# griffithlab/regtools

Measured on AMD Instinct MI355X. Metric: alignments/sec + junctions/sec, junctions extract, 1/2/4/8 MI355X, higher is better.
Workload: dtype u8/u32 integer; 1 GPU; configs[1]: synthetic 50000000-read 101 bp BAM per GPU, ~15% reads with one N-op, junctions extract -s XS; reads_per_gpu=50000000, seed=1, bgzf_members=169426, compressed_bytes_per_gpu=533101619, inflated_bytes_per_gpu=11060000978

## Files before the change

### include/regtools_amd.h

```cpp
#ifndef REGTOOLS_AMD_H
#define REGTOOLS_AMD_H
#include <stddef.h>
#include <stdint.h>

#ifdef __cplusplus
extern "C" {
#endif

#define RGX_OK             0
#define RGX_ERR_OPEN       1
#define RGX_ERR_INDEX      2
#define RGX_ERR_REGION     3
#define RGX_ERR_NO_DEVICE  4
#define RGX_ERR_DEVICE     5
#define RGX_ERR_FORMAT     6
#define RGX_ERR_ARG        7
#define RGX_ERR_FASTA      8
#define RGX_ERR_ABORT      9
#define RGX_ERR_EXIT      10

typedef struct rgx_ctx rgx_ctx;

typedef struct {
    const char *region;
    int32_t     strandness;
    char        strand_tag[2];
    uint32_t    min_anchor;
    uint32_t    min_intron;
    uint32_t    max_intron;
    const char *fasta_path;
    int32_t     shard;
    int32_t     n_shards;
    int32_t     barcodes;
    char        barcode_tag[2];
} rgx_extract_params;

void rgx_extract_params_default(rgx_extract_params *p);

typedef struct {
    int32_t    n_ref;
    char     **ref_name;
    uint32_t  *ref_len;
    uint64_t   n;
    int32_t   *tid;
    uint32_t  *start, *end;
    uint32_t  *thick_start, *thick_end;
    uint32_t  *read_count;
    uint64_t  *name_index;
    char      *strand;
    uint8_t   *left_ok, *right_ok;
    uint64_t   n_records;
    uint64_t   n_events;
    uint64_t   inflated_bytes, compressed_bytes, n_members;
    double     ms_total, ms_inflate, ms_records, ms_scan, ms_reduce;
    uint64_t  *first_seen;
    uint64_t  *last_seen;
    uint64_t   framing_sweeps;
    uint64_t  *bc_row_begin;
    uint32_t  *bc_count;
    uint64_t  *bc_str_begin;
    char      *bc_text;
    uint32_t  *bc_insert_rank;
    double     ms_barcodes;
    uint64_t   stream_ended;
    double     ms_inflate_launch;
} rgx_junction_table;

int  rgx_ctx_create(int device, rgx_ctx **out, char *err, size_t errlen);
void rgx_ctx_destroy(rgx_ctx *ctx);
int  rgx_ctx_arena_trials(const rgx_ctx *ctx, float *ms, int cap);

int  rgx_extract(rgx_ctx *ctx, const char *bam_path, const rgx_extract_params *p,
                 rgx_junction_table **out, char *err, size_t errlen);

void *rgx_host_alloc(size_t bytes);
void  rgx_host_free(void *p);
int  rgx_extract_mem(rgx_ctx *ctx, const void *bam, size_t bam_len, const void *bai, size_t bai_len,
                     const rgx_extract_params *p, rgx_junction_table **out, char *err, size_t errlen);

typedef struct rgx_pipeline rgx_pipeline;
int  rgx_pipeline_create(int device, int depth , rgx_pipeline **out, char *err, size_t errlen);
int  rgx_pipeline_depth(const rgx_pipeline *pl);
rgx_ctx *rgx_pipeline_ctx(const rgx_pipeline *pl, uint64_t ticket);
int  rgx_extract_submit(rgx_pipeline *pl, const void *bam, size_t bam_len, const void *bai, size_t bai_len, const rgx_extract_params *p,
                        uint64_t *ticket, char *err, size_t errlen);
int  rgx_extract_wait(rgx_pipeline *pl, uint64_t ticket, rgx_junction_table **out, char *err, size_t errlen);
void rgx_pipeline_destroy(rgx_pipeline *pl);

int  rgx_extract_device(rgx_ctx *ctx, const void *d_bam, size_t bam_len,
                        const void *bai, size_t bai_len, const rgx_extract_params *p,
                        rgx_junction_table **out, char *err, size_t errlen);

int  rgx_extract_multi(const int *devices, int n_devices, const char *bam_path, const rgx_extract_params *p,
                       rgx_junction_table **out, char *err, size_t errlen);
int  rgx_extract_multi_mem(const int *devices, int n_devices, const void *bam, size_t bam_len, const void *bai, size_t bai_len,
                           const rgx_extract_params *p, rgx_junction_table **out, char *err, size_t errlen);
const char *rgx_multi_exchange_kind(void);

void rgx_table_free(rgx_junction_table *t);

int  rgx_table_merge(const rgx_junction_table *const *parts, int n_parts, uint32_t min_anchor,
                     rgx_junction_table **out, char *err, size_t errlen);

#define RGX_PACKED_ROW_BYTES 48
size_t rgx_table_pack(const rgx_junction_table *t, void *dst, size_t dst_cap);
int    rgx_table_unpack(const void *src, size_t n_rows, const rgx_junction_table *names_from,
                        rgx_junction_table **out);
size_t rgx_table_pack_barcodes(const rgx_junction_table *t, void *dst, size_t dst_cap);
int    rgx_table_unpack_barcodes(rgx_junction_table *t, const void *src, size_t len);
int    rgx_table_merge_barcodes(const rgx_junction_table *const *parts, int n_parts, rgx_junction_table *merged, char *err, size_t errlen);
int    rgx_last_table_pack_device(rgx_ctx *ctx, const rgx_junction_table *t, void *d_dst, uint64_t cap_rows, char *err, size_t errlen);
int    rgx_table_merge_device(rgx_ctx *ctx, const void *d_rows, uint64_t stride_rows, const uint64_t *part_rows, int n_parts,
                              uint32_t min_anchor, const rgx_junction_table *names_from, rgx_junction_table **out,
                              char *err, size_t errlen);

size_t rgx_table_format_bed12(const rgx_junction_table *t, int only_anchored, char *buf, size_t cap);

size_t rgx_table_format_barcodes(const rgx_junction_table *t, int only_anchored, char *buf, size_t cap);

const char *rgx_version(void);

typedef struct { uint64_t cpos, upos; uint32_t clen, isize; } rgx_member;
int  rgx_k_inflate(const void *d_comp, const rgx_member *d_members, uint32_t n_members,
                   void *d_arena, uint32_t *d_status, void *stream);
int  rgx_k_inflate_form(int form, const void *d_comp, const rgx_member *d_members, uint32_t n_members,
                        void *d_arena, uint32_t *d_status, void *stream);

typedef struct {
    const char *vcf_path, *bam_path, *fasta_path, *gtf_path;
    const char *out_tsv;
    const char *out_vcf;
    const char *out_bed;
    uint32_t    window;
    uint32_t    intronic_min;
    uint32_t    exonic_min;
    int32_t     all_intronic;
    int32_t     all_exonic;
    int32_t     skip_single;
    int32_t     strandness;
    char        strand_tag[2];
    uint32_t    min_anchor;
    uint32_t    min_intron;
    uint32_t    max_intron;
    int32_t     override_motif;
    const char *bed_path;
    int32_t     echo;
} rgx_identify_params;

typedef struct {
    uint64_t n_variants, n_relevant, n_windows, n_pairs, n_window_rows, n_junctions;
    uint64_t n_records, n_events;
    uint64_t exon_visits_variants;
    uint64_t exon_visits_junctions;
    double   ms_total, ms_gtf, ms_variants, ms_extract, ms_join, ms_annotate, ms_output;
    double   ms_k_variant_scan, ms_k_junction_scan, ms_k_window_pairs;
} rgx_identify_stats;

void rgx_identify_params_default(rgx_identify_params *p);

int  rgx_identify(rgx_ctx *ctx, const rgx_identify_params *p, rgx_identify_stats *stats, char *err, size_t errlen);
int  rgx_identify_multi(const int *devices, int n_devices, const rgx_identify_params *p, rgx_identify_stats *stats, char *err, size_t errlen);

int  rgx_associate(rgx_ctx *ctx, const rgx_identify_params *p, rgx_identify_stats *stats, char *err, size_t errlen);
int  rgx_variants_annotate(rgx_ctx *ctx, const rgx_identify_params *p, rgx_identify_stats *stats, char *err, size_t errlen);
int  rgx_junctions_annotate(rgx_ctx *ctx, const char *bed_path, const char *fasta_path, const char *gtf_path, const char *out_path,
                            uint64_t *n_rows, char *err, size_t errlen);
#define RGX_ANNOTATE_SINGLE_EXON 1
#define RGX_ANNOTATE_ECHO        2
int  rgx_junctions_annotate_opts(rgx_ctx *ctx, const char *bed_path, const char *fasta_path, const char *gtf_path, const char *out_path,
                                 int options, uint64_t *n_rows, char *err, size_t errlen);

typedef struct rgx_gtf rgx_gtf;
int  rgx_gtf_load(rgx_ctx *ctx, const char *gtf_path, rgx_gtf **out, char *err, size_t errlen);
void rgx_gtf_free(rgx_gtf *g);
int  rgx_gtf_info(const rgx_gtf *g, uint32_t *n_transcripts, uint32_t *n_exons, uint32_t *n_chroms);
int  rgx_gtf_transcript_bin(const rgx_gtf *g, const char *transcript_id, uint32_t *bin);

typedef struct {
    uint64_t n; uint32_t *cis_start, *cis_end; uint32_t *hit_off; uint32_t *hit_transcript, *hit_annotation, *hit_distance;
} rgx_variant_hits;
int  rgx_variant_windows(rgx_ctx *ctx, const rgx_gtf *g, uint64_t n, const char *const *chrom, const uint32_t *pos0, uint32_t intronic_min,
                         uint32_t exonic_min, int all_intronic, int all_exonic, int skip_single, rgx_variant_hits **out, char *err, size_t errlen);
void rgx_variant_hits_free(rgx_variant_hits *h);
const char *rgx_gtf_transcript_id(const rgx_gtf *g, uint32_t t);

typedef struct {
    uint64_t n; uint32_t *flags, *n_acceptors_skipped, *n_exons_skipped, *n_donors_skipped; uint32_t *tx_off, *tx;
} rgx_junction_annot;
int  rgx_annotate_junctions(rgx_ctx *ctx, const rgx_gtf *g, uint64_t n, const char *const *chrom, const uint32_t *start, const uint32_t *end1,
                            const char *strand, rgx_junction_annot **out, char *err, size_t errlen);
void rgx_junction_annot_free(rgx_junction_annot *a);

typedef struct {
    uint64_t n;
    uint32_t *window, *start, *end, *thick_start, *thick_end, *read_count, *name_index;
    char *strand;
} rgx_window_rows;
int  rgx_window_join(rgx_ctx *ctx, const char *bam_path, const rgx_extract_params *p, uint64_t n_windows, const char *const *chrom,
                     const int32_t *beg, const int32_t *end, rgx_window_rows **out, char *err, size_t errlen);
void rgx_window_rows_free(rgx_window_rows *r);

#ifdef __cplusplus
}
#endif
#endif
```

### regtools_amd/_ffi.py

```python
import ctypes as C
import os

_HERE = os.path.dirname(os.path.abspath(__file__))
LIB_PATH = os.path.join(_HERE, "libregtools_amd.so")
SYNTH_PATH = os.path.join(_HERE, "libregtools_synth.so")


class ExtractParams(C.Structure):
    _fields_ = [("region", C.c_char_p), ("strandness", C.c_int32), ("strand_tag", C.c_char * 2),
                ("min_anchor", C.c_uint32), ("min_intron", C.c_uint32), ("max_intron", C.c_uint32),
                ("fasta_path", C.c_char_p), ("shard", C.c_int32), ("n_shards", C.c_int32),
                ("barcodes", C.c_int32), ("barcode_tag", C.c_char * 2)]


class JunctionTable(C.Structure):
    _fields_ = [("n_ref", C.c_int32), ("ref_name", C.POINTER(C.c_char_p)), ("ref_len", C.POINTER(C.c_uint32)),
                ("n", C.c_uint64), ("tid", C.POINTER(C.c_int32)), ("start", C.POINTER(C.c_uint32)),
                ("end", C.POINTER(C.c_uint32)), ("thick_start", C.POINTER(C.c_uint32)),
                ("thick_end", C.POINTER(C.c_uint32)), ("read_count", C.POINTER(C.c_uint32)),
                ("name_index", C.POINTER(C.c_uint64)), ("strand", C.POINTER(C.c_char)),
                ("left_ok", C.POINTER(C.c_uint8)), ("right_ok", C.POINTER(C.c_uint8)),
                ("n_records", C.c_uint64), ("n_events", C.c_uint64), ("inflated_bytes", C.c_uint64),
                ("compressed_bytes", C.c_uint64), ("n_members", C.c_uint64),
                ("ms_total", C.c_double), ("ms_inflate", C.c_double), ("ms_records", C.c_double),
                ("ms_scan", C.c_double), ("ms_reduce", C.c_double),
                ("first_seen", C.POINTER(C.c_uint64)), ("last_seen", C.POINTER(C.c_uint64)), ("framing_sweeps", C.c_uint64),
                ("bc_row_begin", C.POINTER(C.c_uint64)), ("bc_count", C.POINTER(C.c_uint32)), ("bc_str_begin", C.POINTER(C.c_uint64)),
                ("bc_text", C.POINTER(C.c_char)), ("bc_insert_rank", C.POINTER(C.c_uint32)), ("ms_barcodes", C.c_double), ("stream_ended", C.c_uint64),
                ("ms_inflate_launch", C.c_double)]


class Member(C.Structure):
    _fields_ = [("cpos", C.c_uint64), ("upos", C.c_uint64), ("clen", C.c_uint32), ("isize", C.c_uint32)]


EXPORTS = ["rgx_extract_params_default", "rgx_ctx_create", "rgx_ctx_destroy", "rgx_extract", "rgx_extract_mem",
           "rgx_extract_device", "rgx_table_free", "rgx_table_merge", "rgx_table_pack", "rgx_table_unpack",
           "rgx_table_format_bed12", "rgx_table_format_barcodes", "rgx_version", "rgx_k_inflate",
           "rgx_identify_params_default", "rgx_identify", "rgx_gtf_load", "rgx_gtf_free", "rgx_gtf_info", "rgx_gtf_transcript_bin",
           "rgx_gtf_transcript_id", "rgx_variant_windows", "rgx_variant_hits_free", "rgx_annotate_junctions", "rgx_junction_annot_free",
           "rgx_associate", "rgx_variants_annotate", "rgx_junctions_annotate", "rgx_junctions_annotate_opts", "rgx_table_merge_device", "rgx_window_join", "rgx_window_rows_free", "rgx_last_table_pack_device",
           "rgx_host_alloc", "rgx_host_free", "rgx_extract_multi", "rgx_extract_multi_mem", "rgx_multi_exchange_kind", "rgx_k_inflate_form", "rgx_table_merge_barcodes",
           "rgx_table_pack_barcodes", "rgx_table_unpack_barcodes", "rgx_identify_multi", "rgx_ctx_arena_trials",
           "rgx_pipeline_create", "rgx_pipeline_depth", "rgx_pipeline_ctx", "rgx_extract_submit", "rgx_extract_wait", "rgx_pipeline_destroy"]


class IdentifyParams(C.Structure):
    _fields_ = [("vcf_path", C.c_char_p), ("bam_path", C.c_char_p), ("fasta_path", C.c_char_p), ("gtf_path", C.c_char_p),
                ("out_tsv", C.c_char_p), ("out_vcf", C.c_char_p), ("out_bed", C.c_char_p), ("window", C.c_uint32),
                ("intronic_min", C.c_uint32), ("exonic_min", C.c_uint32), ("all_intronic", C.c_int32), ("all_exonic", C.c_int32),
                ("skip_single", C.c_int32), ("strandness", C.c_int32), ("strand_tag", C.c_char * 2), ("min_anchor", C.c_uint32),
                ("min_intron", C.c_uint32), ("max_intron", C.c_uint32), ("override_motif", C.c_int32), ("bed_path", C.c_char_p), ("echo", C.c_int32)]


class IdentifyStats(C.Structure):
    _fields_ = [(n, C.c_uint64) for n in ("n_variants", "n_relevant", "n_windows", "n_pairs", "n_window_rows", "n_junctions", "n_records", "n_events",
                                          "exon_visits_variants", "exon_visits_junctions")] + \
               [(n, C.c_double) for n in ("ms_total", "ms_gtf", "ms_variants", "ms_extract", "ms_join", "ms_annotate", "ms_output",
                                          "ms_k_variant_scan", "ms_k_junction_scan", "ms_k_window_pairs")]


class VariantHits(C.Structure):
    _fields_ = [("n", C.c_uint64), ("cis_start", C.POINTER(C.c_uint32)), ("cis_end", C.POINTER(C.c_uint32)), ("hit_off", C.POINTER(C.c_uint32)),
                ("hit_transcript", C.POINTER(C.c_uint32)), ("hit_annotation", C.POINTER(C.c_uint32)), ("hit_distance", C.POINTER(C.c_uint32))]


class WindowRows(C.Structure):
    _fields_ = [("n", C.c_uint64)] + [(k, C.POINTER(C.c_uint32)) for k in ("window", "start", "end", "thick_start", "thick_end", "read_count", "name_index")] + \
               [("strand", C.POINTER(C.c_char))]


class JunctionAnnot(C.Structure):
    _fields_ = [("n", C.c_uint64), ("flags", C.POINTER(C.c_uint32)), ("n_acceptors_skipped", C.POINTER(C.c_uint32)),
                ("n_exons_skipped", C.POINTER(C.c_uint32)), ("n_donors_skipped", C.POINTER(C.c_uint32)), ("tx_off", C.POINTER(C.c_uint32)),
                ("tx", C.POINTER(C.c_uint32))]

_lib = None


def _preload_torch_hip_runtime():
    try:
        import importlib.util
        spec = importlib.util.find_spec("torch")
        if spec and spec.submodule_search_locations:
            cand = os.path.join(list(spec.submodule_search_locations)[0], "lib", "libamdhip64.so")
            if os.path.exists(cand):
                C.CDLL(cand, mode=C.RTLD_GLOBAL)
    except Exception:
        pass


def lib():
    global _lib
    if _lib is None:
        if not os.path.exists(LIB_PATH):
            raise RuntimeError("regtools_amd: %s is missing -- run `python -c 'import __graft_entry__ as g; g.build()'` "
                               "(hipcc --offload-arch=gfx950). There is no CPU fallback." % LIB_PATH)
        _preload_torch_hip_runtime()
        L = C.CDLL(LIB_PATH)
        P = C.POINTER
        L.rgx_version.restype = C.c_char_p
        L.rgx_extract_params_default.argtypes = [P(ExtractParams)]
        L.rgx_ctx_create.argtypes = [C.c_int, P(C.c_void_p), C.c_char_p, C.c_size_t]
        L.rgx_ctx_destroy.argtypes = [C.c_void_p]
        L.rgx_ctx_arena_trials.argtypes = [C.c_void_p, P(C.c_float), C.c_int]
        L.rgx_extract.argtypes = [C.c_void_p, C.c_char_p, P(ExtractParams), P(P(JunctionTable)), C.c_char_p, C.c_size_t]
        L.rgx_extract_mem.argtypes = [C.c_void_p, C.c_void_p, C.c_size_t, C.c_void_p, C.c_size_t, P(ExtractParams),
                                      P(P(JunctionTable)), C.c_char_p, C.c_size_t]
        L.rgx_extract_device.argtypes = [C.c_void_p, C.c_void_p, C.c_size_t, C.c_void_p, C.c_size_t,
                                         P(ExtractParams), P(P(JunctionTable)), C.c_char_p, C.c_size_t]
        L.rgx_table_free.argtypes = [P(JunctionTable)]
        L.rgx_pipeline_create.argtypes = [C.c_int, C.c_int, P(C.c_void_p), C.c_char_p, C.c_size_t]
        L.rgx_pipeline_depth.argtypes = [C.c_void_p]
        L.rgx_pipeline_ctx.argtypes = [C.c_void_p, C.c_uint64]
        L.rgx_pipeline_ctx.restype = C.c_void_p
        L.rgx_extract_submit.argtypes = [C.c_void_p, C.c_void_p, C.c_size_t, C.c_void_p, C.c_size_t, P(ExtractParams), P(C.c_uint64), C.c_char_p, C.c_size_t]
        L.rgx_extract_wait.argtypes = [C.c_void_p, C.c_uint64, P(P(JunctionTable)), C.c_char_p, C.c_size_t]
        L.rgx_pipeline_destroy.argtypes = [C.c_void_p]
        L.rgx_extract_multi.argtypes = [P(C.c_int), C.c_int, C.c_char_p, P(ExtractParams), P(P(JunctionTable)), C.c_char_p, C.c_size_t]
        L.rgx_multi_exchange_kind.restype = C.c_char_p
        L.rgx_multi_exchange_kind.argtypes = []
        L.rgx_extract_multi_mem.argtypes = [P(C.c_int), C.c_int, C.c_void_p, C.c_size_t, C.c_void_p, C.c_size_t, P(ExtractParams), P(P(JunctionTable)), C.c_char_p, C.c_size_t]
        L.rgx_host_alloc.argtypes = [C.c_size_t]
        L.rgx_host_alloc.restype = C.c_void_p
        L.rgx_host_free.argtypes = [C.c_void_p]
        L.rgx_table_merge.argtypes = [P(P(JunctionTable)), C.c_int, C.c_uint32, P(P(JunctionTable)), C.c_char_p, C.c_size_t]
        L.rgx_table_merge_barcodes.argtypes = [P(P(JunctionTable)), C.c_int, P(JunctionTable), C.c_char_p, C.c_size_t]
        L.rgx_table_pack_barcodes.argtypes = [P(JunctionTable), C.c_void_p, C.c_size_t]
        L.rgx_table_pack_barcodes.restype = C.c_size_t
        L.rgx_table_unpack_barcodes.argtypes = [P(JunctionTable), C.c_void_p, C.c_size_t]
        L.rgx_table_pack.argtypes = [P(JunctionTable), C.c_void_p, C.c_size_t]
        L.rgx_table_pack.restype = C.c_size_t
        L.rgx_table_unpack.argtypes = [C.c_void_p, C.c_size_t, P(JunctionTable), P(P(JunctionTable))]
        L.rgx_last_table_pack_device.argtypes = [C.c_void_p, P(JunctionTable), C.c_void_p, C.c_uint64, C.c_char_p, C.c_size_t]
        L.rgx_table_merge_device.argtypes = [C.c_void_p, C.c_void_p, C.c_uint64, P(C.c_uint64), C.c_int, C.c_uint32, P(JunctionTable), P(P(JunctionTable)), C.c_char_p, C.c_size_t]
        L.rgx_table_format_bed12.argtypes = [P(JunctionTable), C.c_int, C.c_char_p, C.c_size_t]
        L.rgx_table_format_bed12.restype = C.c_size_t
        L.rgx_table_format_barcodes.argtypes = [P(JunctionTable), C.c_int, C.c_char_p, C.c_size_t]
        L.rgx_table_format_barcodes.restype = C.c_size_t
        L.rgx_k_inflate.argtypes = [C.c_void_p, C.c_void_p, C.c_uint32, C.c_void_p, C.c_void_p, C.c_void_p]
        L.rgx_k_inflate_form.argtypes = [C.c_int, C.c_void_p, C.c_void_p, C.c_uint32, C.c_void_p, C.c_void_p, C.c_void_p]
        L.rgx_identify_params_default.argtypes = [P(IdentifyParams)]
        L.rgx_identify.argtypes = [C.c_void_p, P(IdentifyParams), P(IdentifyStats), C.c_char_p, C.c_size_t]
        L.rgx_associate.argtypes = L.rgx_identify.argtypes
        L.rgx_identify_multi.argtypes = [P(C.c_int), C.c_int, P(IdentifyParams), P(IdentifyStats), C.c_char_p, C.c_size_t]
        L.rgx_variants_annotate.argtypes = L.rgx_identify.argtypes
        L.rgx_junctions_annotate_opts.argtypes = [C.c_void_p, C.c_char_p, C.c_char_p, C.c_char_p, C.c_char_p, C.c_int, P(C.c_uint64), C.c_char_p, C.c_size_t]
        L.rgx_junctions_annotate.argtypes = [C.c_void_p, C.c_char_p, C.c_char_p, C.c_char_p, C.c_char_p, P(C.c_uint64), C.c_char_p, C.c_size_t]
        L.rgx_gtf_load.argtypes = [C.c_void_p, C.c_char_p, P(C.c_void_p), C.c_char_p, C.c_size_t]
        L.rgx_gtf_free.argtypes = [C.c_void_p]
        L.rgx_gtf_info.argtypes = [C.c_void_p, P(C.c_uint32), P(C.c_uint32), P(C.c_uint32)]
        L.rgx_gtf_transcript_bin.argtypes = [C.c_void_p, C.c_char_p, P(C.c_uint32)]
        L.rgx_gtf_transcript_id.argtypes = [C.c_void_p, C.c_uint32]
        L.rgx_gtf_transcript_id.restype = C.c_char_p
        L.rgx_variant_windows.argtypes = [C.c_void_p, C.c_void_p, C.c_uint64, P(C.c_char_p), P(C.c_uint32), C.c_uint32, C.c_uint32, C.c_int, C.c_int, C.c_int,
                                          P(P(VariantHits)), C.c_char_p, C.c_size_t]
        L.rgx_variant_hits_free.argtypes = [P(VariantHits)]
        L.rgx_annotate_junctions.argtypes = [C.c_void_p, C.c_void_p, C.c_uint64, P(C.c_char_p), P(C.c_uint32), P(C.c_uint32), C.c_char_p,
                                             P(P(JunctionAnnot)), C.c_char_p, C.c_size_t]
        L.rgx_junction_annot_free.argtypes = [P(JunctionAnnot)]
        L.rgx_window_join.argtypes = [C.c_void_p, C.c_char_p, P(ExtractParams), C.c_uint64, P(C.c_char_p), P(C.c_int32), P(C.c_int32), P(P(WindowRows)), C.c_char_p, C.c_size_t]
        L.rgx_window_rows_free.argtypes = [P(WindowRows)]
        _lib = L
    return _lib


class SynthParams(C.Structure):
    _fields_ = [("shape", C.c_int), ("n_reads", C.c_uint64), ("seed", C.c_uint64), ("level", C.c_int),
                ("threads", C.c_int), ("n_introns", C.c_uint32), ("spliced_frac", C.c_double),
                ("realistic_payload", C.c_int), ("slice_index", C.c_int), ("n_slices", C.c_int), ("n_genes", C.c_uint32)]


class SynthResult(C.Structure):
    _fields_ = [("bam", C.c_void_p), ("bam_len", C.c_size_t), ("bai", C.c_void_p), ("bai_len", C.c_size_t),
                ("n_reads", C.c_uint64), ("n_spliced", C.c_uint64), ("n_blocks", C.c_uint64),
                ("inflated_bytes", C.c_uint64), ("cigar_ops", C.c_uint64)]


_synth = None


def synth():
    global _synth
    if _synth is None:
        if not os.path.exists(SYNTH_PATH):
            raise RuntimeError("regtools_amd: %s is missing -- run __graft_entry__.build()" % SYNTH_PATH)
        L = C.CDLL(SYNTH_PATH)
        P = C.POINTER
        L.rgx_synth_generate.argtypes = [P(SynthParams), P(SynthResult)]
        L.rgx_synth_free.argtypes = [P(SynthResult)]
        L.rgx_synth_write.argtypes = [P(SynthParams), C.c_char_p, P(SynthResult)]
        L.rgx_synth_index.argtypes = [C.c_char_p]
        L.rgx_synth_annotation.argtypes = [P(SynthParams), C.c_uint32, C.c_char_p, C.c_char_p, C.c_char_p]
        _synth = L
    return _synth


def format_bed12(table_ptr, only_anchored=True):
    L = lib()
    t = table_ptr.contents
    longest = max([len(t.ref_name[i]) for i in range(t.n_ref)] or [0])
    cap = int(t.n) * (longest + 160) + 1
    buf = C.create_string_buffer(cap)
    n = L.rgx_table_format_bed12(table_ptr, 1 if only_anchored else 0, buf, cap)
    if n > cap:
        buf = C.create_string_buffer(n + 1)
        L.rgx_table_format_bed12(table_ptr, 1 if only_anchored else 0, buf, n)
    return buf.raw[:n]
```

### regtools_amd/csrc/api_ctx.cpp

```cpp
#include "api_internal.h"

AllocStats g_alloc_stats;

rgx::Fasta *host_fasta(rgx_ctx *c, const char *path) {
    struct stat st;
    if (!path || stat(path, &st) != 0) return nullptr;
    const uint64_t key[4] = {(uint64_t)st.st_dev, (uint64_t)st.st_ino, (uint64_t)st.st_size,
        (uint64_t)st.st_mtim.tv_sec * 1000000000ull + (uint64_t)st.st_mtim.tv_nsec};
    if (c->host_fasta && c->host_fasta_path == path && !memcmp(key, c->host_fasta_key, sizeof key)) return c->host_fasta;
    delete c->host_fasta; c->host_fasta = nullptr;
    rgx::Fasta *f = new rgx::Fasta();
    if (!f->load(path)) { delete f; return nullptr; }
    c->host_fasta = f; c->host_fasta_path = path; memcpy(c->host_fasta_key, key, sizeof key);
    return f;
}

void ktime_begin(rgx_ctx *c, int slot) {
    hipEvent_t e[2];
    for (auto &x : e) { if (!c->kfree.empty()) { x = c->kfree.back(); c->kfree.pop_back(); } else if (hipEventCreate(&x) != hipSuccess) return; }
    (void)hipEventRecord(e[0], c->stream);
    c->kpend.push_back({e[0], e[1], slot});
}
void ktime_end(rgx_ctx *c) { if (!c->kpend.empty()) (void)hipEventRecord(c->kpend.back().b, c->stream); }
void ktime_collect(rgx_ctx *c) {
    for (auto &k : c->kpend) {
        float ms = 0;
        if (hipEventSynchronize(k.b) == hipSuccess && hipEventElapsedTime(&ms, k.a, k.b) == hipSuccess) c->kms[k.slot] += ms;
        c->kfree.push_back(k.a); c->kfree.push_back(k.b);
    }
    c->kpend.clear();
}

extern "C" const char *rgx_version(void) { return "regtools_amd 0.1 gfx950"; }

extern "C" void rgx_extract_params_default(rgx_extract_params *p) {
    memset(p, 0, sizeof *p);
    p->region = "."; p->strandness = -1; p->strand_tag[0] = 'X'; p->strand_tag[1] = 'S';
    p->min_anchor = 8; p->min_intron = 70; p->max_intron = 500000; p->fasta_path = nullptr; p->shard = 0; p->n_shards = 1;
    p->barcodes = 0; p->barcode_tag[0] = 'C'; p->barcode_tag[1] = 'B';
}

extern "C" int rgx_ctx_create(int device, rgx_ctx **out, char *err, size_t errlen) {
    *out = nullptr;
    int n = 0;
    if (hipGetDeviceCount(&n) != hipSuccess || n <= 0)
        return fail(err, errlen, RGX_ERR_NO_DEVICE, "regtools_amd: no HIP device visible; this library has no CPU fallback\n");
    if (device < 0 || device >= n) return fail(err, errlen, RGX_ERR_NO_DEVICE, "regtools_amd: device %d out of range (%d visible)\n", device, n);
    HIP_TRY(hipSetDevice(device));
    hipDeviceProp_t prop;
    HIP_TRY(hipGetDeviceProperties(&prop, device));
    if (!strstr(prop.gcnArchName, "gfx950"))
        return fail(err, errlen, RGX_ERR_NO_DEVICE, "regtools_amd: device %d is %s; the kernels are built for gfx950 only\n", device, prop.gcnArchName);
    rgx_ctx *c = new rgx_ctx();
    c->device = device;
    HIP_TRY(hipStreamCreateWithFlags(&c->stream, hipStreamNonBlocking));
    { const char *e = getenv("REGTOOLS_AMD_ONE_SHOT"); c->one_shot = e && strcmp(e, "0") != 0; }
    c->buf("arena").piece = arena_knobs().piece;
    for (auto &e : c->ev) HIP_TRY(hipEventCreate(&e));
    for (auto &e : c->ev_launch) HIP_TRY(hipEventCreate(&e));
    for (auto &e : c->ev_trial) HIP_TRY(hipEventCreate(&e));
    HIP_TRY(hipHostMalloc(&c->pinned, 4096, hipHostMallocDefault));
    c->pinned_cap = 4096;
    *out = c;
    return RGX_OK;
}

hipError_t ensure_upload_streams(rgx_ctx *c) {
    if (c->copy_stream || c->ev_ready) return hipSuccess;
    if (c->one_shot) return hipEventCreateWithFlags(&c->ev_ready, hipEventDisableTiming);
    hipError_t e = hipStreamCreateWithFlags(&c->copy_stream, hipStreamNonBlocking);
    if (e != hipSuccess) return e;
    for (int k = 0; k < kSideStreams; ++k) {
        if ((e = hipStreamCreateWithPriority(&c->side[k], hipStreamNonBlocking, 0)) != hipSuccess) return e;
        if ((e = hipEventCreateWithFlags(&c->ev_side[k], hipEventDisableTiming)) != hipSuccess) return e;
    }
    return hipEventCreateWithFlags(&c->ev_ready, hipEventDisableTiming);
}

void rgx_ctx_no_arena_trials(rgx_ctx *c) { if (c) c->arena_calibrated_bytes = UINT64_MAX; }
void *rgx_link_turn_create(int depth) {
    LinkTurn *l = new LinkTurn;
    const char *q = getenv("GPU_MAX_HW_QUEUES");
    l->chip.width = q && atoi(q) >= 8 * std::max(2, depth) ? 2 : 1;
    return l;
}
void rgx_link_turn_destroy(void *l) { delete (LinkTurn *)l; }
void rgx_ctx_set_link(rgx_ctx *c, void *l) { if (c) c->link = (LinkTurn *)l; }

extern "C" int rgx_ctx_arena_trials(const rgx_ctx *c, float *ms, int cap) {
    if (!c) return 0;
    for (int k = 0; k < c->arena_trials && k < cap; ++k) ms[k] = c->arena_trial_ms[k];
    return c->arena_trials;
}

extern "C" void rgx_ctx_destroy(rgx_ctx *c) {
    if (!c) return;
    Reaper::get().drain();
    (void)hipSetDevice(c->device);
    for (auto &kv : c->bufs) kv.second.release();
    if (c->arena_retired) { c->arena_retired->release(); delete c->arena_retired; }
    for (auto &e : c->ev) if (e) (void)hipEventDestroy(e);
    for (auto &e : c->ev_launch) if (e) (void)hipEventDestroy(e);
    for (auto &e : c->ev_trial) if (e) (void)hipEventDestroy(e);
    for (auto &e : c->chunk_ev) if (e) (void)hipEventDestroy(e);
    ktime_collect(c);
    for (auto &e : c->kfree) (void)hipEventDestroy(e);
    for (auto &e : c->ev_side) if (e) (void)hipEventDestroy(e);
    if (c->ev_ready) (void)hipEventDestroy(c->ev_ready);
    if (c->ev_packed) (void)hipEventDestroy(c->ev_packed);
    for (auto &q : c->side) if (q) (void)hipStreamDestroy(q);
    if (c->copy_stream) (void)hipStreamDestroy(c->copy_stream);
    delete c->fasta;
    delete c->host_fasta;
    if (c->pinned) (void)hipHostFree(c->pinned);
    if (c->pinned_rows) (void)hipHostFree(c->pinned_rows);
    if (c->pinned_members) (void)hipHostFree(c->pinned_members);
    if (c->stream) (void)hipStreamDestroy(c->stream);
    delete c;
}

static std::mutex g_block_mu;
static std::vector<CachedBlock> g_blocks;
static const size_t kBlockCacheEntries = 6, kBlockCacheBytes = (size_t)1 << 30;

void *block_take(size_t need, size_t &cap, bool pinned) {
    {
        std::lock_guard<std::mutex> lk(g_block_mu);
        size_t best = g_blocks.size();
        for (size_t i = 0; i < g_blocks.size(); ++i)
            if (g_blocks[i].pinned == pinned && g_blocks[i].cap >= need && g_blocks[i].cap <= need * 2 + (1 << 20) &&
                (best == g_blocks.size() || g_blocks[i].cap < g_blocks[best].cap)) best = i;
        if (best != g_blocks.size()) { void *p = g_blocks[best].p; cap = g_blocks[best].cap; g_blocks.erase(g_blocks.begin() + (long)best); return p; }
    }
    cap = need;
    if (!pinned) return malloc(need);
    void *p = nullptr;
    if (hipHostMalloc(&p, need, hipHostMallocDefault) != hipSuccess) return nullptr;
    return p;
}
void block_give(void *p, size_t cap, bool pinned) {
    if (!p) return;
    {
        std::lock_guard<std::mutex> lk(g_block_mu);
        size_t held = 0;
        for (auto &b : g_blocks) held += b.cap;
        if (cap >= (1 << 16) && g_blocks.size() < kBlockCacheEntries && held + cap <= kBlockCacheBytes) { g_blocks.push_back(CachedBlock{p, cap, pinned});
            return; }
    }
    if (pinned) (void)hipHostFree(p); else free(p);
}

rgx_junction_table *table_alloc(const BamHeader &h, uint64_t n, bool zero, bool pinned) {
    TableBox *box = (TableBox *)calloc(1, sizeof *box);
    rgx_junction_table *t = &box->t;
    t->n_ref = (int32_t)h.names.size();
    t->ref_name = (char **)calloc(h.names.size() + 1, sizeof(char *));
    t->ref_len = (uint32_t *)calloc(h.names.size() + 1, sizeof(uint32_t));
    for (size_t i = 0; i < h.names.size(); ++i) { t->ref_name[i] = strdup(h.names[i].c_str()); t->ref_len[i] = h.lens[i]; }
    t->n = n;
    const size_t m = table_block_rows(n);
    const size_t need = table_block_bytes(n);
    box->pinned = pinned;
    box->block = block_take(need, box->block_cap, pinned);
    if (!box->block && pinned) { box->pinned = false; box->block = block_take(need, box->block_cap, false); }
    if (!box->block) {
        for (int32_t i = 0; i < t->n_ref; ++i) free(t->ref_name[i]);
        free(t->ref_name); free(t->ref_len); free(box);
        return nullptr;
    }
    if (zero) memset(box->block, 0, need);
    uint8_t *q = (uint8_t *)box->block;
    t->name_index = (uint64_t *)q; q += m * 8; t->first_seen = (uint64_t *)q; q += m * 8; t->last_seen = (uint64_t *)q; q += m * 8;
    t->tid = (int32_t *)q; q += m * 4; t->start = (uint32_t *)q; q += m * 4; t->end = (uint32_t *)q; q += m * 4;
    t->thick_start = (uint32_t *)q; q += m * 4; t->thick_end = (uint32_t *)q; q += m * 4; t->read_count = (uint32_t *)q; q += m * 4;
    t->strand = (char *)q; q += m; t->left_ok = q; q += m; t->right_ok = q;
    return t;
}

extern "C" void rgx_table_free(rgx_junction_table *t) {
    if (!t) return;
    TableBox *box = (TableBox *)t;
    if (t->ref_name) for (int32_t i = 0; i < t->n_ref; ++i) free(t->ref_name[i]);
    free(t->ref_name); free(t->ref_len);
    block_give(box->block, box->block_cap, box->pinned);
    free(t->bc_row_begin); free(t->bc_count); free(t->bc_str_begin); free(t->bc_text); free(t->bc_insert_rank);
    free(box);
}

void host_sort_rows(rgx_junction_table *t) {
    std::vector<uint32_t> crank((size_t)std::max(t->n_ref, 1), 0);
    {
        std::vector<int32_t> order((size_t)t->n_ref);
        for (int32_t i = 0; i < t->n_ref; ++i) order[(size_t)i] = i;
        std::sort(order.begin(), order.end(), [&](int32_t a, int32_t b) { return strcmp(t->ref_name[a], t->ref_name[b]) < 0; });
        uint32_t rk = 0;
        for (int32_t i = 0; i < t->n_ref; ++i) { if (i > 0 && strcmp(t->ref_name[order[(size_t)i]], t->ref_name[order[(size_t)i - 1]]) != 0) ++rk;
            crank[(size_t)order[(size_t)i]] = rk; }
    }
    auto name_less = [](uint64_t a, uint64_t b) {
        if (a < 100000000ull && b < 100000000ull) return a < b;
        char na[32], nb[32];
        snprintf(na, sizeof na, "%08llu", (unsigned long long)a); snprintf(nb, sizeof nb, "%08llu", (unsigned long long)b);
        return strcmp(na, nb) < 0;
    };
    std::vector<uint64_t> idx(t->n);
    for (uint64_t i = 0; i < t->n; ++i) idx[i] = i;
    std::sort(idx.begin(), idx.end(), [&](uint64_t a, uint64_t b) {
        const uint32_t ca = crank[(size_t)t->tid[a]], cb = crank[(size_t)t->tid[b]];
        if (ca != cb) return ca < cb;
        if (t->thick_start[a] != t->thick_start[b]) return t->thick_start[a] < t->thick_start[b];
        if (t->thick_end[a] != t->thick_end[b]) return t->thick_end[a] < t->thick_end[b];
        return name_less(t->name_index[a], t->name_index[b]);
    });
    auto permute = [&](auto *col) {
        typedef typename std::remove_reference<decltype(col[0])>::type T;
        std::vector<T> tmp(t->n);
        for (uint64_t i = 0; i < t->n; ++i) tmp[i] = col[idx[i]];
        memcpy(col, tmp.data(), sizeof(T) * t->n);
    };
    permute(t->tid); permute(t->start); permute(t->end); permute(t->thick_start); permute(t->thick_end); permute(t->read_count);
    permute(t->name_index); permute(t->strand); permute(t->left_ok); permute(t->right_ok); permute(t->first_seen); permute(t->last_seen);
}

void format_bed12_rows(const rgx_junction_table *t, int only_anchored, uint64_t r0, uint64_t r1, std::string &out) {
    char tail[256];
    for (uint64_t i = r0; i < r1; ++i) {
        if (only_anchored && !(t->left_ok[i] && t->right_ok[i])) continue;
        const char *name = t->ref_name[t->tid[i]];
        const int n = snprintf(tail, sizeof tail, "\t%u\t%u\tJUNC%08llu\t%u\t%c\t%u\t%u\t255,0,0\t2\t%u,%u\t0,%u\n",
                               t->thick_start[i], t->thick_end[i], (unsigned long long)t->name_index[i], t->read_count[i], t->strand[i],
                               t->thick_start[i], t->thick_end[i], (uint32_t)(t->start[i] - t->thick_start[i]),
                               (uint32_t)(t->thick_end[i] - t->end[i]), (uint32_t)(t->end[i] - t->thick_start[i]));
        out.append(name); out.append(tail, (size_t)n);
    }
}

extern "C" size_t rgx_table_format_bed12(const rgx_junction_table *t, int only_anchored, char *buf, size_t cap) {
    const unsigned n_thr = t->n >= 20000 ? std::max(1u, std::min<unsigned>(usable_threads(16), (unsigned)(t->n / 8192))) : 1u;
    std::vector<std::string> part(n_thr);
    if (n_thr == 1) format_bed12_rows(t, only_anchored, 0, t->n, part[0]);
    else {
        std::vector<std::thread> pool;
        for (unsigned w = 0; w < n_thr; ++w)
            pool.emplace_back([&, w] { part[w].reserve((size_t)(t->n / n_thr + 1) * 96); format_bed12_rows(t, only_anchored, t->n * w / n_thr,
                t->n * (w + 1) / n_thr, part[w]); });
        for (auto &th : pool) th.join();
    }
    size_t need = 0;
    for (const std::string &q : part) need += q.size();
    if (buf && need <= cap) { size_t o = 0; for (const std::string &q : part) { memcpy(buf + o, q.data(), q.size()); o += q.size(); } }
    return need;
}

extern "C" size_t rgx_table_format_barcodes(const rgx_junction_table *t, int only_anchored, char *buf, size_t cap) {
    size_t need = 0;
    auto put = [&](const char *s, size_t n) { if (buf && need + n <= cap) memcpy(buf + need, s, n); need += n; };
    char num[32];
    for (uint64_t i = 0; i < t->n; ++i) {
        if (only_anchored && !(t->left_ok[i] && t->right_ok[i])) continue;
        const uint64_t b = t->bc_row_begin ? t->bc_row_begin[i] : 0, e = t->bc_row_begin ? t->bc_row_begin[i + 1] : 0;
// ... 12 lines not shown
```

### regtools_amd/csrc/api_entry.cpp

```cpp
#include "api_internal.h"

extern "C" int rgx_extract_device(rgx_ctx *ctx, const void *d_bam, size_t bam_len, const void *bai, size_t bai_len,
                                  const rgx_extract_params *p, rgx_junction_table **out, char *err, size_t errlen) {
    if (!ctx || !d_bam || !out) return fail(err, errlen, RGX_ERR_ARG, "regtools_amd: bad arguments\n");
    return run_pipeline(ctx, (const uint8_t *)d_bam, nullptr, bam_len, (const uint8_t *)bai, bai_len, p, out, err, errlen);
}

extern "C" int rgx_extract_mem(rgx_ctx *ctx, const void *bam, size_t bam_len, const void *bai, size_t bai_len, const rgx_extract_params *p,
                               rgx_junction_table **out, char *err, size_t errlen) {
    if (!ctx || !bam || !out) return fail(err, errlen, RGX_ERR_ARG, "regtools_amd: bad arguments\n");
    fputs(bam_open_notes((const uint8_t *)bam, bam_len, nullptr, nullptr).c_str(), stderr);
    return run_pipeline(ctx, nullptr, (const uint8_t *)bam, bam_len, (const uint8_t *)bai, bai_len, p, out, err, errlen);
}

int rgx_extract_mem_scanned(rgx_ctx *ctx, const void *bam, size_t bam_len, const void *bai, size_t bai_len, const rgx_extract_params *p,
                            const std::vector<rgx::Member> *members, uint64_t total_inflated, rgx_junction_table **out, char *err, size_t errlen) {
    if (!ctx || !bam || !out) return fail(err, errlen, RGX_ERR_ARG, "regtools_amd: bad arguments\n");
    SharedMembers sm{members, total_inflated};
    return run_pipeline(ctx, nullptr, (const uint8_t *)bam, bam_len, (const uint8_t *)bai, bai_len, p, out, err, errlen, members && !members->empty() ? &sm :
        nullptr);
}

extern "C" void *rgx_host_alloc(size_t bytes) {
    void *p = nullptr;
    return hipHostMalloc(&p, bytes ? bytes : 1, hipHostMallocDefault) == hipSuccess ? p : nullptr;
}
extern "C" void rgx_host_free(void *p) { if (p) (void)hipHostFree(p); }

extern "C" int rgx_extract(rgx_ctx *ctx, const char *bam_path, const rgx_extract_params *p, rgx_junction_table **out, char *err, size_t errlen) {
    if (!ctx || !bam_path || !out) return fail(err, errlen, RGX_ERR_ARG, "regtools_amd: bad arguments\n");
    FileBytes bam; std::vector<uint8_t> bai;
    if (!bam.open(bam_path)) return fail(err, errlen, RGX_ERR_OPEN, "[E::hts_open_format] fail to open file '%s'\n%s", bam_path, kMsgOpen);
    std::string idx;
    int r = find_index(bam_path, idx);
    fputs(bam_open_notes(bam.data(), bam.size(), r == 0 ? bam_path : nullptr, r == 0 ? idx.c_str() : nullptr).c_str(), stderr);
    if (r != 0 || !read_index(idx, bai)) return fail(err, errlen, RGX_ERR_INDEX, "%s", kMsgIndex);
    return run_pipeline(ctx, nullptr, bam.data(), bam.size(), bai.data(), bai.size(), p, out, err, errlen);
}

extern "C" int rgx_k_inflate(const void *d_comp, const rgx_member *d_members, uint32_t n_members, void *d_arena, uint32_t *d_status, void *stream) {
    return rgx_k_inflate_form(0, d_comp, d_members, n_members, d_arena, d_status, stream);
}

extern "C" int rgx_k_inflate_form(int form, const void *d_comp, const rgx_member *d_members, uint32_t n_members, void *d_arena, uint32_t *d_status,
    void *stream) {
    if (form < 0 || form > 5) return RGX_ERR_ARG;
    static_assert(sizeof(rgx_member) == sizeof(Member), "rgx_member layout");
    static void *scratch = nullptr; static size_t scratch_cap = 0;
    const size_t need = inflate_scratch_bytes(n_members);
    if (need > scratch_cap) {
        if (scratch) (void)hipFree(scratch);
        if (hipMalloc(&scratch, need) != hipSuccess) { scratch = nullptr; scratch_cap = 0; return RGX_ERR_DEVICE; }
        scratch_cap = need;
    }
    launch_inflate((const uint8_t *)d_comp, (const Member *)d_members, n_members, (uint8_t *)d_arena, 0, (uint32_t *)scratch, d_status, (hipStream_t)stream,
        0, 0, false, form, nullptr, 1, true);
    return hipGetLastError() == hipSuccess ? RGX_OK : RGX_ERR_DEVICE;
}

extern "C" size_t rgx_table_pack(const rgx_junction_table *t, void *dst, size_t dst_cap) {
    const size_t need = (size_t)t->n * RGX_PACKED_ROW_BYTES;
    if (!dst || dst_cap < need) return need;
    uint8_t *q = (uint8_t *)dst;
    for (uint64_t i = 0; i < t->n; ++i, q += RGX_PACKED_ROW_BYTES) {
        uint32_t w[12] = {(uint32_t)t->tid[i], t->start[i], t->end[i], t->thick_start[i], t->thick_end[i], t->read_count[i],
                          (uint32_t)t->first_seen[i], (uint32_t)(t->first_seen[i] >> 32), (uint32_t)t->last_seen[i], (uint32_t)(t->last_seen[i] >> 32),
                          (uint32_t)(uint8_t)t->strand[i], (uint32_t)t->name_index[i]};
        memcpy(q, w, sizeof w);
    }
    return need;
}

extern "C" int rgx_table_unpack(const void *src, size_t n_rows, const rgx_junction_table *names_from, rgx_junction_table **out) {
    BamHeader h;
    for (int32_t i = 0; i < names_from->n_ref; ++i) { h.names.push_back(names_from->ref_name[i]); h.lens.push_back(names_from->ref_len[i]); }
    rgx_junction_table *t = table_alloc(h, n_rows);
    if (!t) return RGX_ERR_ARG;
    const uint8_t *q = (const uint8_t *)src;
    for (size_t i = 0; i < n_rows; ++i, q += RGX_PACKED_ROW_BYTES) {
        uint32_t w[12]; memcpy(w, q, sizeof w);
        t->tid[i] = (int32_t)w[0]; t->start[i] = w[1]; t->end[i] = w[2]; t->thick_start[i] = w[3]; t->thick_end[i] = w[4]; t->read_count[i] = w[5];
        t->first_seen[i] = (uint64_t)w[6] | (uint64_t)w[7] << 32; t->last_seen[i] = (uint64_t)w[8] | (uint64_t)w[9] << 32; t->strand[i] = (char)w[10];
        t->name_index[i] = w[11];
    }
    *out = t;
    return RGX_OK;
}

extern "C" size_t rgx_table_pack_barcodes(const rgx_junction_table *t, void *dst, size_t dst_cap) {
    if (!t || !t->bc_row_begin) return 0;
    const uint64_t n = t->n, E = t->bc_row_begin[n], T = t->bc_str_begin ? t->bc_str_begin[E] : 0;
    const size_t need = 24 + (size_t)(n + 1) * 8 + (size_t)(E + 1) * 8 + (size_t)E * 8 + (size_t)T;
    if (!dst || dst_cap < need) return need;
    uint8_t *q = (uint8_t *)dst;
    const uint64_t head[3] = {n, E, T};
    memcpy(q, head, 24); q += 24;
    memcpy(q, t->bc_row_begin, (size_t)(n + 1) * 8); q += (size_t)(n + 1) * 8;
    memcpy(q, t->bc_str_begin, (size_t)(E + 1) * 8); q += (size_t)(E + 1) * 8;
    memcpy(q, t->bc_count, (size_t)E * 4); q += (size_t)E * 4;
    memcpy(q, t->bc_insert_rank, (size_t)E * 4); q += (size_t)E * 4;
    memcpy(q, t->bc_text, (size_t)T);
    return need;
}

extern "C" int rgx_table_unpack_barcodes(rgx_junction_table *t, const void *src, size_t len) {
    if (!t || !src || len < 24) return RGX_ERR_ARG;
    const uint8_t *q = (const uint8_t *)src;
    uint64_t head[3]; memcpy(head, q, 24); q += 24;
    const uint64_t n = head[0], E = head[1], T = head[2];
    if (n != t->n || E > (len >> 3) || T > len) return RGX_ERR_ARG;
    const size_t need = 24 + (size_t)(n + 1) * 8 + (size_t)(E + 1) * 8 + (size_t)E * 8 + (size_t)T;
    if (len < need) return RGX_ERR_ARG;
    uint64_t *row_begin = (uint64_t *)calloc((size_t)n + 1, 8), *str_begin = (uint64_t *)calloc((size_t)E + 1, 8);
    uint32_t *count = (uint32_t *)calloc((size_t)E + 1, 4), *rank = (uint32_t *)calloc((size_t)E + 1, 4);
    char *text = (char *)malloc((size_t)T + 1);
    bool ok = row_begin && str_begin && count && rank && text;
    if (ok) {
        memcpy(row_begin, q, (size_t)(n + 1) * 8); q += (size_t)(n + 1) * 8;
        memcpy(str_begin, q, (size_t)(E + 1) * 8); q += (size_t)(E + 1) * 8;
        memcpy(count, q, (size_t)E * 4); q += (size_t)E * 4;
        memcpy(rank, q, (size_t)E * 4); q += (size_t)E * 4;
        memcpy(text, q, (size_t)T);
        ok = row_begin[0] == 0 && row_begin[n] == E && str_begin[0] == 0 && str_begin[E] == T;
        for (uint64_t i = 0; ok && i < n; ++i) ok = row_begin[i] <= row_begin[i + 1];
        for (uint64_t k = 0; ok && k < E; ++k) ok = str_begin[k] <= str_begin[k + 1];
        for (uint64_t i = 0; ok && i < n; ++i) {
            const uint64_t b = row_begin[i], e = row_begin[i + 1];
            std::vector<uint8_t> seen((size_t)(e - b), 0);
            for (uint64_t k = b; ok && k < e; ++k) { ok = rank[k] < e - b && !seen[rank[k]]; if (ok) seen[rank[k]] = 1; }
        }
    }
    if (!ok) { free(row_begin); free(str_begin); free(count); free(rank); free(text); return RGX_ERR_ARG; }
    free(t->bc_row_begin); free(t->bc_count); free(t->bc_str_begin); free(t->bc_text); free(t->bc_insert_rank);
    t->bc_row_begin = row_begin; t->bc_str_begin = str_begin; t->bc_count = count; t->bc_insert_rank = rank; t->bc_text = text;
    return RGX_OK;
}

extern "C" int rgx_table_merge_barcodes(const rgx_junction_table *const *parts, int n_parts, rgx_junction_table *t, char *err, size_t errlen) {
    if (!parts || n_parts <= 0 || !t) return fail(err, errlen, RGX_ERR_ARG, "regtools_amd: nothing to merge\n");
    for (int g = 0; g < n_parts; ++g) if (!parts[g] || !parts[g]->bc_row_begin) return fail(err, errlen, RGX_ERR_ARG,
        "regtools_amd: shard %d carries no barcode counts\n", g);
    auto cls = [](char c) { return c == '+' ? 0u : c == '-' ? 1u : 2u; };
    struct Key { int32_t tid; uint32_t start, end, cls; bool operator==(const Key &o) const { return tid == o.tid && start == o.start && end == o.end &&
        cls == o.cls; } };
    struct KeyHash {
        size_t operator()(const Key &k) const {
            const uint64_t h = (uint64_t)(uint32_t)k.tid * 0x9e3779b97f4a7c15ull ^ ((uint64_t)k.start << 32 | k.end) * 0xc2b2ae3d27d4eb4full ^ k.cls;
            return (size_t)(h ^ h >> 29);
        }
    };
    std::unordered_map<Key, uint64_t, KeyHash> row_of;
    row_of.reserve((size_t)t->n * 2 + 16);
    for (uint64_t i = 0; i < t->n; ++i) row_of[Key{t->tid[i], t->start[i], t->end[i], cls(t->strand[i])}] = i;
    struct Ent { const char *s; uint32_t len; uint32_t count; };
    std::vector<std::vector<Ent>> per_row((size_t)t->n);
    typedef std::pair<const char *, uint32_t> Sv;
    struct SvHash {
        size_t operator()(const Sv &k) const {
            uint64_t h = 1469598103934665603ull;
            for (uint32_t i = 0; i < k.second; ++i) h = (h ^ (uint8_t)k.first[i]) * 1099511628211ull;
            return (size_t)h;
        }
    };
    struct SvEq { bool operator()(const Sv &a, const Sv &b) const { return a.second == b.second && !memcmp(a.first, b.first, a.second); } };
    typedef std::unordered_map<std::pair<const char *, uint32_t>, uint32_t, SvHash, SvEq> RowIndex;
    std::unordered_map<uint64_t, RowIndex> row_index;
    constexpr size_t kScanRows = 16;
    std::vector<uint64_t> order;
    for (int g = 0; g < n_parts; ++g) {
        const rgx_junction_table *p = parts[g];
        for (uint64_t i = 0; i < p->n; ++i) {
            auto it = row_of.find(Key{p->tid[i], p->start[i], p->end[i], cls(p->strand[i])});
            if (it == row_of.end()) return fail(err, errlen, RGX_ERR_ARG,
                "regtools_amd: a shard row is missing from the merged table (shard %d row %llu: tid %d %u-%u '%c'; merged rows %llu)\n", g,
                (unsigned long long)i, p->tid[i], p->start[i], p->end[i], p->strand[i], (unsigned long long)t->n);
            std::vector<Ent> &dst = per_row[(size_t)it->second];
            const uint64_t b = p->bc_row_begin[i], e = p->bc_row_begin[i + 1];
            order.assign(e - b, 0);
            for (uint64_t k = b; k < e; ++k) order[p->bc_insert_rank[k]] = k;
            for (uint64_t k : order) {
                const char *str = p->bc_text + p->bc_str_begin[k];
                const uint32_t len = (uint32_t)(p->bc_str_begin[k + 1] - p->bc_str_begin[k]);
                bool found = false;
                if (dst.size() > kScanRows) {
                    RowIndex &ix = row_index[it->second];
                    if (ix.empty()) for (uint32_t q = 0; q < dst.size(); ++q) ix.emplace(std::make_pair(dst[q].s, dst[q].len), q);
                    auto f = ix.find(std::make_pair(str, len));
                    if (f != ix.end()) { dst[f->second].count += p->bc_count[k]; found = true; }
                    else ix.emplace(std::make_pair(str, len), (uint32_t)dst.size());
                } else for (Ent &x : dst) if (x.len == len && !memcmp(x.s, str, len)) { x.count += p->bc_count[k]; found = true; break; }
                if (!found) dst.push_back(Ent{str, len, p->bc_count[k]});
            }
        }
        if (p->stream_ended) break;
    }
    size_t n_pairs = 0, text_len = 0;
    for (auto &v : per_row) { n_pairs += v.size(); for (auto &x : v) text_len += x.len; }
    free(t->bc_row_begin); free(t->bc_count); free(t->bc_str_begin); free(t->bc_text); free(t->bc_insert_rank);
    t->bc_row_begin = (uint64_t *)calloc((size_t)t->n + 1, 8);
    t->bc_count = (uint32_t *)calloc(n_pairs + 1, 4);
    t->bc_str_begin = (uint64_t *)calloc(n_pairs + 1, 8);
    t->bc_text = (char *)malloc(text_len + 1);
    t->bc_insert_rank = (uint32_t *)calloc(n_pairs + 1, 4);
    uint64_t o = 0, pos = 0;
    for (uint64_t r = 0; r < t->n; ++r) {
        t->bc_row_begin[r] = o;
        const std::vector<Ent> &v = per_row[(size_t)r];
        std::unordered_map<std::string, int> m;
        for (size_t k = 0; k < v.size(); ++k) m.insert(std::pair<std::string, int>(std::string(v[k].s, v[k].len), (int)k));
// ... 216 lines not shown
```

### regtools_amd/csrc/api_front.cpp

```cpp
#include "api_internal.h"

int EventsRun::run() {
    if (!p || p->strandness < 0 || p->strandness > 3) return fail(err, errlen, RGX_ERR_ARG, "Please supply strandness mode with '-s' option!\n\n");
    if (p->strandness == 3 && !p->fasta_path) return fail(err, errlen, RGX_ERR_ARG, "Strandness mode 'intron-motif' requires a fasta file!\n\n");
    HIP_ENTER(c->device);
    st = c->stream;
    copy_q = c->copy_stream ? c->copy_stream : c->stream;
    t_begin = now_ms();
    trace = getenv("REGTOOLS_AMD_TRACE") != nullptr;
    t_last = t_begin;

    if (bam_len < 28) return fail(err, errlen, RGX_ERR_OPEN, "%s", kMsgOpen);
    if (c->arena_retired) { c->arena_retired->release(); delete c->arena_retired; c->arena_retired = nullptr; }
    { const int rc = stage_upload(); if (rc != kGoOn) return rc; }
    { const int rc = stage_members(); if (rc != kGoOn) return rc; }
    { const int rc = stage_range_and_inflate(); if (rc != kGoOn) return rc; }
    { const int rc = stage_footers_and_header(); if (rc != kGoOn) return rc; }
    { const int rc = stage_bounds_and_chains(); if (rc != kGoOn) return rc; }
    { const int rc = stage_framing(); if (rc != kGoOn) return rc; }
    { const int rc = stage_decode(); if (rc != kGoOn) return rc; }
    const int rc_emit = stage_emit();
    if (rc_emit == RGX_OK) { const int rc = calibrate_arena(); if (rc != RGX_OK) return rc; }
    P.d_file = rc_emit == RGX_OK && p->n_shards <= 1 && (!p->region || !strcmp(p->region, ".")) ? d_bam : nullptr;
    return rc_emit;
}

static int arena_challengers() { return arena_knobs().trials; }
int EventsRun::calibrate_arena() {
    if (!arena_challengers() || c->one_shot || d_true_sizes || chunked || split_B || P.stream_ended || !n_range || n_range <= 2048 ||
        total < ((uint64_t)2 << 30)) return RGX_OK;
    if (c->arena_calibrated_bytes == UINT64_MAX || (c->arena_calibrated_bytes &&
        total + 256 <= c->arena_calibrated_bytes + c->arena_calibrated_bytes / 4)) return RGX_OK;
    static std::mutex trial_mu[16];
    std::lock_guard<std::mutex> trial_lock(trial_mu[(unsigned)c->device % 16u]);
    if (!inflate_takes_coop(n_range) || h_sc[0] != 0xffffffffu) return RGX_OK;
    DevBuf &b_arena = c->buf("arena"), &b_lens = c->buf("inflate_scratch");
    if (!b_arena.p || b_arena.cap < total + 256) return RGX_OK;
    auto room_for_one = [&] {
        size_t free_b = 0, total_b = 0;
        return hipMemGetInfo(&free_b, &total_b) == hipSuccess && free_b >= b_arena.cap + b_arena.cap / 8 + ((size_t)16 << 30);
    };
    const int plan = inflate_plan_for(bam_len, total_all);
    uint32_t *d_dummy = d_sc + 100;
    auto time_into = [&](uint8_t *arena_p, float &ms) -> hipError_t {
        float t[3] = {0, 0, 0};
        for (int k = 0; k < 4; ++k) {
            hipError_t e = hipMemsetAsync(d_dummy, 0xff, 8, st);
            if (e != hipSuccess) return e;
            if ((e = hipEventRecord(c->ev_trial[0], st)) != hipSuccess) return e;
            launch_inflate(d_bam, d_members + m_lo, n_range, arena_p, upos_lo, b_lens.as<uint32_t>(), d_dummy, st, 0, 0, false, 0, nullptr, plan);
            if ((e = hipEventRecord(c->ev_trial[1], st)) != hipSuccess) return e;
            if ((e = hipEventSynchronize(c->ev_trial[1])) != hipSuccess) return e;
            if (k && (e = hipEventElapsedTime(&t[k - 1], c->ev_trial[0], c->ev_trial[1])) != hipSuccess) return e;
        }
        std::sort(t, t + 3);
        ms = t[1];
        return hipSuccess;
    };
    c->arena_trials = 0;
    float best_ms = 0;
    if (time_into(b_arena.as<uint8_t>(), best_ms) != hipSuccess) { (void)hipGetLastError(); return RGX_OK; }
    c->arena_trial_ms[c->arena_trials++] = best_ms;
    DevBuf best;
    for (int k = 0; k < arena_challengers(); ++k) {
        if (best.p) break;
        if (!room_for_one()) break;
        static const size_t kLadder[] = {(size_t)1 << 30, (size_t)256 << 20, (size_t)512 << 20, (size_t)128 << 20, (size_t)1 << 30, (size_t)64 << 20,
            (size_t)512 << 20};
        DevBuf cand; cand.piece = b_arena.piece ? kLadder[k % 7] : 0;
        if (cand.ensure(b_arena.cap) != hipSuccess) { (void)hipGetLastError(); break; }
        float ms = 0;
        if (time_into(cand.as<uint8_t>(), ms) != hipSuccess) { (void)hipGetLastError(); cand.release(); break; }
        if (c->arena_trials < 8) c->arena_trial_ms[c->arena_trials++] = ms;
        if (ms < best_ms * 0.985f) { best = cand; best_ms = ms; } else cand.release();
    }
    if (best.p) {
        if (c->arena_retired) { c->arena_retired->release(); delete c->arena_retired; }
        c->arena_retired = new DevBuf(b_arena);
        b_arena = best;
        b_arena.piece = arena_knobs().piece;
    }
    c->arena_calibrated_bytes = b_arena.cap;
    if (trace) {
        fprintf(stderr, "[rgx trace] arena placement: call's arena %.3f ms", c->arena_trial_ms[0]);
        for (int k = 1; k < c->arena_trials; ++k) fprintf(stderr, ", %.3f", c->arena_trial_ms[k]);
        fprintf(stderr, " -> %s\n", best.p ? "a challenger kept" : "kept");
    }
    mark("arena placement trial");
    return RGX_OK;
}

int EventsRun::stage_upload() {
    bai_thread = std::thread([this] {
        bai_ok = bai && normalize_index(bai, bai_len, index_image, bai, bai_len) && parse_bai(bai, bai_len, bi, false);
    });
    d_bam = d_bam_in;
    std::vector<Member> &hm = c->hm_scratch;
    hm.clear();
    if (!d_bam) {
        DevBuf &b = c->buf("bam");
        HIP_TRY(b.ensure(bam_len + 64));
        d_bam = b.as<uint8_t>();
        mark("file buffer in HBM");
        if (c->link) { c->wire_hold.take(&c->link->wire); mark("the link is ours"); }
        const size_t overlap_min = overlap_knobs().min_bytes;
        if (allow_overlap && !d_true_sizes && bam_len >= overlap_min) {
            HIP_TRY(ensure_upload_streams(c));
            if (c->copy_stream) copy_q = c->copy_stream;
            mark("upload streams");
            size_t up_lo = 0, up_hi = bam_len, hdr_hi = 0;
            if (shared && p->n_shards > 1 && p->shard >= 0 && p->shard < p->n_shards) {
                if (bai_thread.joinable()) bai_thread.join();
                BamHeader hh; size_t hb = 0;
                if (bai_ok && host_bam_header(h_bam, std::min<size_t>(bam_len, (size_t)8 << 20), hh, &hb)) {
                    const bool rest0 = p->region && !strcmp(p->region, "*"), whole0 = rest0 || !strcmp(p->region ? p->region : ".", ".");
                    uint64_t sv = 0;
                    if (rest0 && bi.have_nocoor) sv = bi.nocoor_voff; else if (whole0 && !rest0 && bi.have_start) sv = bi.start_voff;
                    uint64_t tgt[2], got[2];
                    for (int k = 0; k < 2; ++k) tgt[k] = std::max<uint64_t>((uint64_t)((double)bam_len * (p->shard + k) / p->n_shards) << 16, sv ? sv : 1);
                    bai_first_anchor_ge(bai, bai_len, tgt, 2, got);
                    if (p->shard > 0 && got[0] != UINT64_MAX) up_lo = std::min<size_t>(bam_len, (size_t)(got[0] >> 16));
                    else if (p->shard > 0) up_lo = bam_len;
                    if (p->shard + 1 < p->n_shards && got[1] != UINT64_MAX) up_hi = std::min<size_t>(bam_len, (size_t)(got[1] >> 16) + 2 * kBgzfMaxBlock + 64);
                    if (up_hi < up_lo) up_hi = up_lo;
                    const std::vector<Member> &sm = *shared->members;
                    if (!sm.empty()) { const Member &m4 = sm[std::min<size_t>(sm.size(), 4) - 1]; hb = std::max<size_t>(hb, (size_t)m4.cpos + m4.clen + 8); }
                    hdr_hi = std::min(up_lo, hb + 64);
                    up_lo &= ~(size_t)4095;
                    if (up_lo < hdr_hi) { up_lo = 0; hdr_hi = 0; }
                }
            }
            const unsigned gate_chunks = overlap_knobs().chunks;
            gated = !c->gate_distrust && !c->one_shot && up_hi - up_lo >= std::min(overlap_min, (size_t)8 << 20) &&
                up_hi - up_lo >= 2 * 4096 * (size_t)gate_chunks;
            if (gated) {
                uint64_t cb = 0, ub = 0; size_t o = 0;
                for (int k = 0; k < 64 && o + 28 <= bam_len; ++k) {
                    if (!(h_bam[o] == 0x1f && h_bam[o + 1] == 0x8b && h_bam[o + 12] == 'B' && h_bam[o + 13] == 'C')) break;
                    const size_t bl = (size_t)(h_bam[o + 16] | h_bam[o + 17] << 8) + 1;
                    if (bl < 26 || o + bl > bam_len) break;
                    uint32_t isz; memcpy(&isz, h_bam + o + bl - 4, 4);
                    cb += bl; ub += isz; o += bl;
                }
                if (cb && !(inflate_plan_for(cb, ub) & 1)) gated = false;
            }
            std::vector<unsigned> cuts = {33, 67};
            if (c->one_shot) cuts.clear();
            if (gated) {
                gate_chunk = (((up_hi - up_lo) + gate_chunks - 1) / gate_chunks + 4095) & ~(size_t)4095;
                for (size_t e = up_lo + gate_chunk; e < up_hi; e += gate_chunk) up.end.push_back(e);
                DevBuf &bg = c->buf("gate_flags");
                if (!bg.p) { HIP_TRY(bg.ensure(4 * 64)); HIP_TRY(hipMemset(bg.p, 0, 4 * 64)); c->gate_epoch = 0; }
                ++c->gate_epoch;
            } else
            for (unsigned pc : cuts) {
                const size_t e = (up_lo + (size_t)((double)(up_hi - up_lo) * pc / 100.0) + 4095) & ~(size_t)4095;
                if (e < up_hi && e > up_lo && (up.end.empty() || e > up.end.back())) up.end.push_back(e);
            }
            up.end.push_back(up_hi);
// ... 354 lines not shown
```

### regtools_amd/csrc/api_internal.h

```cpp
#pragma once
#include "../../include/regtools_amd.h"

#include <hip/hip_runtime.h>
#include <stdarg.h>
#include <stdio.h>
#include <stdlib.h>
#include <string.h>

#include <algorithm>
#include <atomic>
#include <condition_variable>
#include <charconv>
#include <chrono>
#include <map>
#include <memory>
#include <mutex>
#include <string>
#include <thread>
#include <unordered_map>
#include <vector>

#include "cse_host.h"
#include "host_io.h"
#include "worker_pool.h"
// ... 35 lines not shown
inline const ArenaKnobs &arena_knobs() {
    static const ArenaKnobs k = [] {
        ArenaKnobs v;
        if (const char *e = getenv("REGTOOLS_AMD_ARENA")) {
            long long a = -1, b = -1;
            const int n = sscanf(e, "%lld,%lld", &a, &b);
            if (n >= 1 && a >= 0) v.trials = (int)std::min<long long>(a, 7);
            if (n >= 2 && b >= 0) v.piece = b == 0 ? 0 : (size_t)std::min<long long>(std::max<long long>(b, 2), 16384) << 20;
        }
        return v;
    }();
    return k;
}
struct DevBuf {
    static constexpr size_t kFront = 256;
    void *p = nullptr; size_t cap = 0;
    size_t piece = 0;
    size_t mapped = 0;
    std::vector<size_t> piece_len;
    int range_dev = -1;
    struct KeptRange { void *base; size_t len; int dev; };
    struct KeptRanges { std::mutex mu; std::vector<KeptRange> v; };
    static KeptRanges &kept_ranges() { static KeptRanges *k = new KeptRanges(); return *k; }
    static void *take_range(int dev, size_t total, size_t *reserved) {
        KeptRanges &k = kept_ranges();
        std::lock_guard<std::mutex> lock(k.mu);
        size_t best = SIZE_MAX;
        for (size_t i = 0; i < k.v.size(); ++i) if (k.v[i].dev == dev && k.v[i].len >= total && (best == SIZE_MAX || k.v[i].len < k.v[best].len)) best = i;
        if (best == SIZE_MAX) return nullptr;
        void *base = k.v[best].base; *reserved = k.v[best].len;
        k.v.erase(k.v.begin() + (long)best);
        return base;
    }
    static void unmap_range(void *base, const std::vector<size_t> &lens, size_t reserved, int dev) {
        static const bool trace = getenv("REGTOOLS_AMD_TRACE") != nullptr;
        size_t at = 0;
        for (size_t n : lens) {
            const hipError_t e = hipMemUnmap((uint8_t *)base + at, n);
            if (e != hipSuccess && trace) fprintf(stderr, "[rgx trace] hipMemUnmap of %zu bytes at +%zu: %s\n", n, at, hipGetErrorString(e));
            if (e != hipSuccess) (void)hipGetLastError();
            at += n;
        }
        KeptRanges &k = kept_ranges();
        std::lock_guard<std::mutex> lock(k.mu);
        k.v.push_back(KeptRange{base, reserved, dev});
    }
    hipError_t map_pieces(size_t bytes, void **out) {
        int dev = 0;
        hipError_t e = hipGetDevice(&dev);
        if (e != hipSuccess) return e;
        hipMemAllocationProp prop = {}; prop.type = hipMemAllocationTypePinned; prop.location.type = hipMemLocationTypeDevice; prop.location.id = dev;
        size_t gran = 0;
        if (hipMemGetAllocationGranularity(&gran, &prop, hipMemAllocationGranularityRecommended) != hipSuccess || !gran) { (void)hipGetLastError();
            gran = (size_t)2 << 20; }
        const size_t total = (bytes + gran - 1) / gran * gran, each = std::max(gran, piece / gran * gran);
        size_t reserved = total;
        void *base = take_range(dev, total, &reserved);
        if (!base) { reserved = total; if ((e = hipMemAddressReserve(&base, total, 0, nullptr, 0)) != hipSuccess) return e; }
        std::vector<size_t> lens;
        size_t done = 0;
        while (done < total) {
            const size_t n = std::min(each, total - done);
            hipMemGenericAllocationHandle_t h;
            if ((e = hipMemCreate(&h, n, &prop, 0)) != hipSuccess) break;
            e = hipMemMap((uint8_t *)base + done, n, 0, h, 0);
            (void)hipMemRelease(h);
            if (e != hipSuccess) break;
            lens.push_back(n);
            done += n;
        }
        if (e == hipSuccess) {
            hipMemAccessDesc ad = {}; ad.location.type = hipMemLocationTypeDevice; ad.location.id = dev; ad.flags = hipMemAccessFlagsProtReadWrite;
            e = hipMemSetAccess(base, total, &ad, 1);
        }
        if (e != hipSuccess) { unmap_range(base, lens, reserved, dev); return e; }
        *out = base; mapped = reserved; range_dev = dev; piece_len.swap(lens);
        return hipSuccess;
    }
    hipError_t ensure(size_t bytes) {
        if (bytes <= cap) return hipSuccess;
        static const bool trace = getenv("REGTOOLS_AMD_TRACE") != nullptr;
        const auto t0 = std::chrono::steady_clock::now();
        release();
        static const bool no_slack = [] { const char *e = getenv("REGTOOLS_AMD_ONE_SHOT"); return e && strcmp(e, "0") != 0; }();
        size_t want = bytes + (no_slack ? 0 : bytes / 8) + 256;
        void *raw = nullptr;
        hipError_t e = hipErrorNotSupported;
        if (piece && want + kFront >= piece) { e = map_pieces(want + kFront, &raw); if (e != hipSuccess) { (void)hipGetLastError(); raw = nullptr;
            mapped = 0; piece_len.clear(); } }
        if (e != hipSuccess) e = hipMalloc(&raw, want + kFront);
        if (e == hipSuccess) { p = (uint8_t *)raw + kFront; cap = want; }
        if (trace) {
            static std::mutex mu; std::lock_guard<std::mutex> lock(mu);
            g_alloc_stats.ms += std::chrono::duration<double, std::milli>(std::chrono::steady_clock::now() - t0).count(); ++g_alloc_stats.calls;
                g_alloc_stats.bytes += want;
        }
        return e;
    }
    void release() {
        if (p && mapped) { (void)hipDeviceSynchronize();
                           unmap_range((uint8_t *)p - kFront, piece_len, mapped, range_dev); }
        else if (p) (void)hipFree((uint8_t *)p - kFront);
        p = nullptr; cap = 0; mapped = 0; piece_len.clear();
    }
    template <class T> T *as() const { return (T *)p; }
};

constexpr int kSideStreams = 2;
struct OverlapKnobs { size_t min_bytes = (size_t)8 << 20; unsigned chunks = 16; uint32_t early_min = 4096; bool early_small = false; };
inline const OverlapKnobs &overlap_knobs() {
    static const OverlapKnobs k = [] {
        OverlapKnobs v;
        if (const char *e = getenv("REGTOOLS_AMD_OVERLAP")) {
            long long a = -1, b = -1, c2 = -1;
            const int n = sscanf(e, "%lld,%lld,%lld", &a, &b, &c2);
            if (n >= 1 && a >= 0) v.min_bytes = (size_t)a;
            if (n >= 2 && b >= 2) v.chunks = (unsigned)std::min<long long>(b, 64);
            if (n >= 3 && c2 >= 1) { v.early_min = (uint32_t)c2; v.early_small = true; }
        }
        return v;
    }();
    return k;
}
struct Turn {
    std::mutex mu; std::condition_variable cv; uint64_t next = 0, serving = 0;
    uint64_t width = 1;
};
struct LinkTurn { Turn wire, chip; };
struct TurnHold {
    Turn *t = nullptr; std::atomic<bool> held{false};
    void take(Turn *x) {
        if (!x || held.load()) return;
        std::unique_lock<std::mutex> lk(x->mu);
        const uint64_t mine = x->next++;
        x->cv.wait(lk, [&] { return mine < x->serving + x->width; });
        t = x; held.store(true);
    }
    void give() { if (held.exchange(false)) { { std::lock_guard<std::mutex> lk(t->mu); ++t->serving; } t->cv.notify_all(); } }
};

struct rgx_ctx {
    int device = 0;
    LinkTurn *link = nullptr;
    TurnHold wire_hold, chip_hold;
    hipStream_t stream = nullptr;
    hipStream_t copy_stream = nullptr, side[kSideStreams] = {};
    bool gate_distrust = false, early_distrust = false;
    bool walk_strict = false;
    bool one_shot = false;
    std::vector<hipEvent_t> chunk_ev;
    uint32_t gate_epoch = 0;
    hipEvent_t ev_ready = nullptr, ev_side[kSideStreams] = {}, ev_packed = nullptr;
    hipEvent_t ev[8] = {};
    uint64_t arena_calibrated_bytes = 0;
    DevBuf *arena_retired = nullptr;
    hipEvent_t ev_trial[2] = {};
    float arena_trial_ms[8] = {}; int arena_trials = 0;
    hipEvent_t ev_launch[2] = {}; bool launch_timed = false;
    std::map<std::string, DevBuf> bufs;
    void *pinned = nullptr; size_t pinned_cap = 0;
    std::vector<Member> hm_scratch;
    void *pinned_members = nullptr; size_t pinned_members_cap = 0;
    void *pinned_rows = nullptr; size_t pinned_rows_cap = 0;
    uint64_t last_rows = 0, last_records = 0, last_events = 0, last_bytes = 0; bool last_rows_valid = false;
    struct KPend { hipEvent_t a, b; int slot; };
    std::vector<KPend> kpend; std::vector<hipEvent_t> kfree; double kms[3] = {0, 0, 0};
    uint64_t tables_made = 0;
    std::vector<uint32_t> rank_stage;
    std::string fasta_path;
    rgx::Fasta *fasta = nullptr;
    rgx::Fasta *host_fasta = nullptr; std::string host_fasta_path; uint64_t host_fasta_key[4] = {0, 0, 0, 0};
    DevBuf &buf(const char *name) { return bufs[name]; }
};


rgx::Fasta *host_fasta(rgx_ctx *c, const char *path);
void ktime_begin(rgx_ctx *c, int slot);
void ktime_end(rgx_ctx *c);
void ktime_collect(rgx_ctx *c);
hipError_t ensure_upload_streams(rgx_ctx *c);
rgx_junction_table *table_alloc(const BamHeader &h, uint64_t n, bool zero = true, bool pinned = false);
void host_sort_rows(rgx_junction_table *t);
void format_bed12_rows(const rgx_junction_table *t, int only_anchored, uint64_t r0, uint64_t r1, std::string &out);
void *block_take(size_t need, size_t &cap, bool pinned);
void block_give(void *p, size_t cap, bool pinned);
struct TableBox { rgx_junction_table t; void *block; size_t block_cap; bool pinned; };
struct CachedBlock { void *p; size_t cap; bool pinned; };
struct SharedMembers { const std::vector<Member> *members; uint64_t total_inflated; };

struct Prep {
    BamHeader hdr;
    const uint8_t *arena = nullptr;
    ReadSoA soa{};
    EventSoA ev{};
    uint32_t n_rec = 0, n_events = 0, n_range = 0;
    uint64_t n_iterated = 0, total = 0;
    uint32_t framing_sweeps = 0;
    bool stream_ended = false;
    double t_begin = 0;
    struct OddAux { int32_t tid, pos, end; };
    std::vector<OddAux> odd_aux;
    const uint8_t *d_file = nullptr;
};

int prepare_events(rgx_ctx *c, const uint8_t *d_bam_in, const uint8_t *h_bam, size_t bam_len, const uint8_t *bai, size_t bai_len,
                          const rgx_extract_params *p, bool want_read_span, Prep &P, char *err, size_t errlen, const uint32_t *d_true_sizes = nullptr,
                          bool allow_overlap = true, bool region_to_file_end = false, const SharedMembers *shared = nullptr);

constexpr int kGoOn = -1;

struct EventsRun {
    rgx_ctx *c; const uint8_t *d_bam_in; const uint8_t *h_bam; size_t bam_len; const uint8_t *bai; size_t bai_len;
    const rgx_extract_params *p; bool want_read_span; Prep &P; char *err; size_t errlen; const uint32_t *d_true_sizes;
    bool allow_overlap, region_to_file_end; const SharedMembers *shared;
    hipStream_t st = nullptr, copy_q = nullptr;
    double t_begin = 0, t_last = 0; bool trace = false;
    void mark(const char *what) { if (trace) { double t = now_ms(); fprintf(stderr, "[rgx trace] %-28s +%8.3f ms  (at %8.3f)%s\n", what, t - t_last,
        t - t_begin, c->link ? (" clock " + std::to_string(fmod(t, 1e5))).c_str() : ""); t_last = t; } }
    BaiInfo bi; bool bai_ok = false;
    std::vector<uint8_t> index_image;
    std::thread bai_thread;
    const uint8_t *d_bam = nullptr;
    struct Upload {
        std::thread th; std::atomic<uint32_t> recorded{0}; std::atomic<int> err{0};
        std::vector<size_t> end;
        size_t lo = 0, hi = 0, hdr_hi = 0;
        hipStream_t copy_stream = nullptr;
        ~Upload() { if (th.joinable()) th.join(); if (copy_stream) (void)hipStreamSynchronize(copy_stream); }
    } up;
    bool overlap = false, gated = false;
    size_t gate_chunk = 0;
    uint64_t hm_total = 0;
    uint32_t *d_sc = nullptr, *h_sc = nullptr;
    hipError_t complete_upload() {
        if (!h_bam || !(up.lo || (up.hi && up.hi < bam_len))) return hipSuccess;
        if (up.th.joinable()) up.th.join();
        hipError_t e = hipStreamSynchronize(copy_q);
        uint8_t *dst = c->buf("bam").as<uint8_t>();
        if (e == hipSuccess && up.lo > up.hdr_hi) e = hipMemcpy(dst + up.hdr_hi, h_bam + up.hdr_hi, up.lo - up.hdr_hi, hipMemcpyHostToDevice);
        if (e == hipSuccess && up.hi < bam_len) e = hipMemcpy(dst + up.hi, h_bam + up.hi, bam_len - up.hi, hipMemcpyHostToDevice);
        up.lo = 0; up.hi = bam_len; up.hdr_hi = 0;
        return e;
    }
    uint32_t n_cand = 0;
    uint64_t *cand = nullptr;
    uint32_t *nx[2] = {nullptr, nullptr}, *c_isize = nullptr, *c_reach = nullptr, *c_rank = nullptr, *c_isz2 = nullptr, *c_tmp = nullptr;
    Member *d_members = nullptr; hipMemcpyKind from_members = hipMemcpyDeviceToHost;
    void chain(uint64_t root2) {
        launch_member_link(d_bam, bam_len, cand, n_cand, nx[0], c_isize, c_reach, root2, st);
        int cur = 0;
        for (uint32_t span = 1; span < n_cand; span <<= 1) { launch_member_jump(n_cand, nx[cur], nx[cur ^ 1], c_reach, st); cur ^= 1; }
        launch_member_jump(n_cand, nx[cur], nx[cur ^ 1], c_reach, st);
        launch_scan_u32(c_reach, c_rank, n_cand, d_sc + 17, c_tmp, st);
        launch_member_compact(d_bam, bam_len, cand, c_isize, c_reach, c_rank, n_cand, d_members, c_isz2, st);
        if (d_true_sizes) launch_member_fix(d_members, c_isz2, n_cand, d_sc + 17, d_true_sizes, st);
        launch_member_upos(d_members, c_isz2, d_sc + 17, (uint64_t *)(d_sc + 20), st);
    }
    bool whole = false, seek = false, chunked = false, geom_chunked_hint = false, empty_stream = false;
    uint64_t seek_voff = 0, cut_lo = 0, cut_hi = UINT64_MAX, total_all = 0, q_upos[3] = {0, 0, 0};
    std::vector<VChunk> chunks;
    uint32_t n_members_all = 0, first_member = 0, stop = 0;
    uint32_t m_lo = 0, m_hi = 0, n_range = 0;
    uint64_t upos_lo = 0, total = 0;
    uint8_t *d_bad = nullptr;
    hipError_t member_at(uint32_t k, Member &m) {
        if (from_members == hipMemcpyHostToHost) { memcpy(&m, d_members + k, sizeof m); return hipSuccess; }
        hipError_t e = hipMemcpyAsync(&m, d_members + k, sizeof m, from_members, st);
        return e == hipSuccess ? hipStreamSynchronize(st) : e;
    }
    hipError_t upos_of(uint32_t k, uint64_t &out_v) {
        if (k >= n_members_all) { out_v = total_all; return hipSuccess; }
        Member m;
        hipError_t e = member_at(k, m);
        out_v = m.upos;
        return e;
    }
    struct EarlyPart { uint32_t members, waves; uint64_t upos; };
    std::vector<EarlyPart> early_parts;
    bool split_B = false; hipEvent_t split_ev = nullptr;
    hipError_t join_B() {
        if (!split_B) return hipSuccess;
        split_B = false;
        return hipStreamWaitEvent(st, split_ev, 0);
    }
    bool spec = false; uint32_t mean_rec = 0;
    BamHeader hdr; int32_t n_ref = 0;
    uint64_t lim = 0, pos0 = 0; bool chain_ended = false;
    ExtractCfg cfg; SegGeom geom; uint32_t seg_bytes = 0;
    std::vector<SegChunk> seg_chunks;
    const uint8_t *arena = nullptr; uint64_t span = 0; uint32_t n_seg = 0, n_rec = 0; bool lite_walk = false;
    uint64_t *seg_start[2] = {nullptr, nullptr}, *seg_exit[2] = {nullptr, nullptr};
    uint32_t *seg_cnt[2] = {nullptr, nullptr}, *seg_base = nullptr;
    uint32_t *seg_iter_e = nullptr, *seg_long_e = nullptr, *seg_long_base_e = nullptr;
    uint16_t *seg_cp = nullptr;
    int cur = 0;
    int frame(uint32_t n_s, uint32_t walk_from, bool &ended) {
        DevBuf &b_tmp = c->buf("tmp");
        launch_seg_walk(arena, geom, n_s, n_ref, seg_start[cur], seg_exit[cur], seg_cnt[cur], seg_cp, st, walk_from);
        for (int iter = 0;; ++iter) {
            HIP_TRY(hipMemsetAsync(d_sc + 10, 0xff, 8, st));
            launch_seg_verify(arena, geom, n_s, seg_start[cur], seg_exit[cur], seg_cnt[cur], seg_start[cur ^ 1], seg_exit[cur ^ 1],
                              seg_cnt[cur ^ 1], d_sc + 10, seg_cp, st);
            cur ^= 1;
            launch_scan_u32(seg_cnt[cur], seg_base, n_s, d_sc + 3, b_tmp.as<uint32_t>(), st);
            HIP_TRY(hipMemcpyAsync(h_sc + 3, d_sc + 3, 4, hipMemcpyDeviceToHost, st));
            HIP_TRY(hipMemcpyAsync(h_sc + 10, d_sc + 10, 8, hipMemcpyDeviceToHost, st));
            if (spec && iter == 0) {
                HIP_TRY(hipMemcpyAsync(h_sc, d_sc, 8, hipMemcpyDeviceToHost, st));
                HIP_TRY(hipMemcpyAsync(h_sc + kStatusEarly, d_sc + kStatusEarly, 8, hipMemcpyDeviceToHost, st));
            }
            HIP_TRY(hipStreamSynchronize(st));
            if (spec && iter == 0 && (h_sc[0] != 0xffffffffu || h_sc[kStatusEarly] != 0xffffffffu)) {
                mark("inflate verdict: not clean, starting over device-resident");
                if (gated) { c->gate_distrust = true; if (trace) fprintf(stderr,
                    "[rgx trace] arrival gate: verdict not clean, this context no longer uses it\n"); }
                HIP_TRY(join_B());
                HIP_TRY(complete_upload());
                HIP_TRY(hipStreamSynchronize(copy_q));
                HIP_TRY(hipStreamSynchronize(st));
                const int rc2 = prepare_events(c, d_bam, nullptr, bam_len, bai, bai_len, p, want_read_span, P, err, errlen, nullptr, false, region_to_file_end);
                P.t_begin = t_begin;
                return rc2;
            }
            ++P.framing_sweeps;
            if (h_sc[11] != 0xffffffffu) ended = true;
            if (h_sc[11] != 0xffffffffu && (h_sc[11] < h_sc[10] || (h_sc[10] == 0xffffffffu && geom.chunks))) {
                launch_seg_truncate(geom, n_s, h_sc[11], seg_start[cur], seg_exit[cur], seg_cnt[cur], st);
                launch_scan_u32(seg_cnt[cur], seg_base, n_s, d_sc + 3, b_tmp.as<uint32_t>(), st);
                HIP_TRY(hipMemcpyAsync(h_sc + 3, d_sc + 3, 4, hipMemcpyDeviceToHost, st));
                HIP_TRY(hipStreamSynchronize(st));
                break;
            }
            if (h_sc[10] == 0xffffffffu) break;
            if (iter > 1 << 20) return fail(err, errlen, RGX_ERR_FORMAT, "regtools_amd: record framing did not converge\n");
        }
        return -1;
    }
    uint32_t sA = 0;
    bool emit_parts_ok = false; uint32_t emit_parts = 0, emit_rows = 0; size_t ev_lay = 0;
    EventSoA ev_e;
    EventSoA ev_layout(uint8_t *q, size_t E) {
        EventSoA v; memset(&v, 0, sizeof v);
        v.tid = (uint32_t *)q; q += E * 4; v.start = (uint32_t *)q; q += E * 4; v.ilen_cls = (uint32_t *)q; q += E * 4;
        v.ts = (uint32_t *)q; q += E * 4; v.te = (uint32_t *)q; q += E * 4;
        if (want_read_span) { v.rpos = (uint32_t *)q; q += E * 4; v.rend = (uint32_t *)q; q += E * 4; }
        if (p->barcodes) { v.read = (uint32_t *)q; q += E * 4; }
        v.strand = q;
        return v;
    }
    size_t soa_cap = 0;
    ReadSoA soa;
    uint32_t *ev_base = nullptr, *long_list = nullptr;
    hipError_t soa_layout(size_t R) {
        DevBuf &b_soa = c->buf("soa");
        hipError_t e_ = b_soa.ensure(R * (4 + 4 + 4 + 8 + 1 + 4 + 4 + 4 + (p->barcodes ? 8 : 0)) + 256);
        if (e_ != hipSuccess) return e_;
        uint8_t *q = b_soa.as<uint8_t>();
        soa.cig_off = (uint64_t *)q; q += R * 8;
        if (p->barcodes) { soa.rec_off = (uint64_t *)q; q += R * 8; }
        soa.tid = (int32_t *)q; q += R * 4; soa.pos = (int32_t *)q; q += R * 4; soa.flag_nc = (uint32_t *)q; q += R * 4;
        soa.n_ev = (uint32_t *)q; q += R * 4; ev_base = (uint32_t *)q; q += R * 4; long_list = (uint32_t *)q; q += R * 4;
        soa.strand = q;
        soa_cap = R;
        return hipSuccess;
    }
    uint32_t n_events = 0, n_long = 0; uint64_t n_iterated = 0;
    ~EventsRun() {
        if (split_B && split_ev) (void)hipEventSynchronize(split_ev);
        if (bai_thread.joinable()) bai_thread.join();
        if (c->link && !d_bam_in) { c->wire_hold.give(); c->chip_hold.give(); }
    }
    int run();
    int calibrate_arena();
    int stage_upload();
    int stage_members();
    int stage_range_and_inflate();
    int stage_footers_and_header();
    int stage_bounds_and_chains();
    int stage_framing();
    int stage_decode();
    int stage_emit();
};
struct HostRows {
    std::vector<uint32_t> group, start, end, ts, te, count, name_rank, first_seen, last_seen;
    std::vector<uint8_t> strand;
    size_t n = 0;
    const uint32_t *cols = nullptr;
};

struct RowMap { uint32_t *ev_urow = nullptr, *urow_pos = nullptr; };
struct TableSink { const BamHeader *hdr = nullptr; uint32_t min_anchor = 0; rgx_junction_table *table = nullptr; };

int reduce_events(rgx_ctx *c, EventSoA ev, uint32_t n_events, uint32_t group_bits, uint32_t ilen_bits, const uint32_t *rank_of_group_host,
                  uint32_t n_groups, HostRows &R, char *err, size_t errlen, bool view_only = false, RowMap *row_map = nullptr, TableSink *sink = nullptr,
                  bool allow_preagg = true );
int barcode_rows(rgx_ctx *c, const Prep &P, const RowMap &rm, const rgx_extract_params *p, rgx_junction_table *t, char *err, size_t errlen);
void chrom_string_ranks(const BamHeader &hdr, std::vector<uint32_t> &rank_of_tid);
int run_pipeline(rgx_ctx *c, const uint8_t *d_bam_in, const uint8_t *h_bam, size_t bam_len, const uint8_t *bai, size_t bai_len,
                 const rgx_extract_params *p, rgx_junction_table **out, char *err, size_t errlen, const SharedMembers *shared = nullptr);
bool rgx_enable_peer(int a, int b);
int rgx_last_table_pack_async(rgx_ctx *c, const rgx_junction_table *t, void **d_packed, hipEvent_t *done, char *err, size_t errlen);
```

### regtools_amd/csrc/api_records.cpp

```cpp
#include "api_internal.h"

int EventsRun::stage_footers_and_header() {
    DevBuf &b_arena = c->buf("arena"), &b_hdr = c->buf("hdr_arena"), &b_lens = c->buf("inflate_scratch");
    BamHeader hdr_host;
    mean_rec = 0;
    spec = overlap && !d_true_sizes && !geom_chunked_hint && host_bam_header(h_bam, std::min<size_t>(bam_len, (size_t)8 << 20), hdr_host, nullptr, &mean_rec);
    if (spec) { h_sc[0] = h_sc[1] = 0xffffffffu; h_sc[kStatusEarly] = h_sc[kStatusEarly + 1] = 0xffffffffu; }
    else {
        HIP_TRY(join_B());
        HIP_TRY(hipMemcpyAsync(h_sc, d_sc, 8, hipMemcpyDeviceToHost, st));
        HIP_TRY(hipMemcpyAsync(h_sc + kStatusEarly, d_sc + kStatusEarly, 8, hipMemcpyDeviceToHost, st));
        HIP_TRY(hipStreamSynchronize(st));
    }
    if (!d_true_sizes) {
        auto size_trouble = [&](uint32_t k) { return h_sc[k] != 0xffffffffu &&
            (h_sc[k + 1] == 12u  || h_sc[k + 1] == 10u ); };
        bool lies = size_trouble(0) || size_trouble(kStatusEarly);
        if (!lies && stop < n_members_all) {
            Member ms; uint8_t two[2] = {0, 0};
            HIP_TRY(member_at(stop, ms));
            if (ms.isize == 0 && ms.clen >= 2) {
                if (h_bam && ms.cpos + 2 <= bam_len) memcpy(two, h_bam + ms.cpos, 2);
                else { HIP_TRY(hipMemcpyAsync(two, d_bam + ms.cpos, 2, hipMemcpyDeviceToHost, st)); HIP_TRY(hipStreamSynchronize(st)); }
            }
// ... 58 lines not shown
                return fail(err, errlen, RGX_ERR_REGION, "%s", kMsgRegion);
            n_h = std::min(n_members_all, n_h * 4);
        }
    }
    n_ref = (int32_t)hdr.names.size();
    mark("header (sync: inflate done)");

    return kGoOn;
}

int EventsRun::stage_bounds_and_chains() {
    lim = total;
    if (h_sc[0] != 0xffffffffu) {
        uint64_t u = 0;
        HIP_TRY(upos_of(m_lo + h_sc[0], u));
        lim = u - upos_lo;
    }
    auto arena_of = [&](uint64_t voff, uint32_t idx, uint64_t upos) -> uint64_t {
        if (idx >= n_members_all || idx < m_lo || idx >= m_hi) return total;
        return std::min<uint64_t>(total, upos - upos_lo + (voff & 0xffff));
    };
    if (cut_lo) pos0 = arena_of(cut_lo, h_sc[25], q_upos[1]);
    else pos0 = hdr.end;
    chain_ended = false;
    P.stream_ended = empty_stream;
    if (cut_hi != UINT64_MAX) {
        const uint64_t cut_lim = arena_of(cut_hi, h_sc[26], q_upos[2]);
        const uint32_t mh = h_sc[26];
        const uint32_t hi_wanted = (mh < n_members_all && (cut_hi & 0xffff)) ? mh + 1 : mh;
        if (!chunked && h_sc[0] != 0xffffffffu && lim < cut_lim) P.stream_ended = true;
        if (!chunked && stop < std::min(hi_wanted, n_members_all)) P.stream_ended = true;
        lim = std::min(lim, cut_lim);
    } else if (h_sc[0] != 0xffffffffu) P.stream_ended = true;
    if (pos0 > lim) pos0 = lim;
    if (empty_stream) lim = pos0;

    memset(&cfg, 0, sizeof cfg);
    cfg.n_ref = n_ref; cfg.strandness = p->strandness; cfg.tag0 = (uint8_t)p->strand_tag[0]; cfg.tag1 = (uint8_t)p->strand_tag[1];
    if ((p->strandness == 0 || p->barcodes) && !want_read_span) { cfg.abort_out = d_sc + 96; HIP_TRY(hipMemsetAsync(d_sc + 96, 0xff, 4, st)); }
    if (p->barcodes && !want_read_span) { cfg.bc0 = (uint8_t)p->barcode_tag[0]; cfg.bc1 = (uint8_t)p->barcode_tag[1]; }
    if (p->strandness == 0 && want_read_span) { cfg.odd_count = d_sc + 97; HIP_TRY(hipMemsetAsync(d_sc + 97, 0, 4, st)); }
    P.odd_aux.clear();
    cfg.min_anchor = p->min_anchor; cfg.min_intron = p->min_intron; cfg.max_intron = p->max_intron;
    cfg.region_tid = -2; cfg.long_threshold = 16;
    if (!whole) {
        int32_t tid, beg, end;
        if (!parse_region(hdr, p->region, tid, beg, end) || tid >= bi.n_ref || end < beg)
            return fail(err, errlen, RGX_ERR_REGION, "%s", kMsgRegion);
        cfg.region_tid = tid; cfg.region_beg = beg; cfg.region_end = end;
    }

    if (p->fasta_path) {
        if (!c->fasta || c->fasta_path != p->fasta_path) {
            delete c->fasta; c->fasta = new Fasta(); c->fasta_path.clear();
            if (!c->fasta->load(p->fasta_path)) { delete c->fasta; c->fasta = nullptr; return fail(err, errlen, RGX_ERR_FASTA,
                "Unable to open FASTA file.\n\n"); }
            DevBuf &bf = c->buf("fasta");
            HIP_TRY(bf.ensure(c->fasta->size + 256));
            HIP_TRY(hipMemcpy(bf.p, c->fasta->data, c->fasta->size, hipMemcpyHostToDevice));
            c->fasta_path = p->fasta_path;
        }
        std::vector<FaContig> tab((size_t)std::max(n_ref, 1));
        memset(tab.data(), 0, tab.size() * sizeof(FaContig));
        for (int32_t t = 0; t < n_ref; ++t)
            for (const Fasta::Seq &s : c->fasta->seqs)
                if (s.name == hdr.names[(size_t)t]) {
                    const bool sane = s.offset >= 0 && s.len >= 0 && s.line_blen > 0 && s.line_len >= s.line_blen &&
                                      (s.len == 0 ||
                                          (uint64_t)s.offset + (uint64_t)((s.len - 1) / s.line_blen) * (uint64_t)s.line_len +
                                                  (uint64_t)((s.len - 1) % s.line_blen) < (uint64_t)c->fasta->size);
                    if (!sane) continue;
                    tab[(size_t)t].offset = s.offset; tab[(size_t)t].len = s.len; tab[(size_t)t].line_blen = s.line_blen;
                        tab[(size_t)t].line_len = s.line_len; tab[(size_t)t].present = 1;
                }
        DevBuf &bt = c->buf("fasta_tab");
        HIP_TRY(bt.ensure(tab.size() * sizeof(FaContig) + 64));
        HIP_TRY(hipMemcpy(bt.p, tab.data(), tab.size() * sizeof(FaContig), hipMemcpyHostToDevice));
        cfg.fa_data = c->buf("fasta").as<uint8_t>(); cfg.fa_tab = bt.as<FaContig>(); cfg.fa_missing = d_sc + 64;
    }

    memset(&geom, 0, sizeof geom);
    const int env_seg = decode_knobs().seg_bytes;
    seg_bytes = env_seg == (int)kSegBytes || env_seg == (int)kSegBytesLong ? (uint32_t)env_seg : (mean_rec >= kLongRecordBytes ? kSegBytesLong : kSegBytes);
    geom.seg_bytes = seg_bytes;
    if (chunked && chunks.empty()) lim = pos0;
    if (chunked && !chunks.empty() && !empty_stream) {
        std::vector<Member> rm(n_range);
        std::vector<uint8_t> bad(n_range, 0);
        if (n_range) {
            HIP_TRY(hipMemcpyAsync(rm.data(), d_members + m_lo, (size_t)n_range * sizeof(Member), from_members, st));
            HIP_TRY(hipMemcpyAsync(bad.data(), d_bad, n_range, hipMemcpyDeviceToHost, st));
            HIP_TRY(hipStreamSynchronize(st));
        }
        for (uint32_t k = 0; k < n_range; ++k) if (rm[k].isize == 0 || rm[k].isize > kBgzfMaxBlock) bad[k] = 1;
        std::vector<uint32_t> next_bad((size_t)n_range + 1, n_range);
        for (uint32_t k = n_range; k-- > 0;) next_bad[k] = bad[k] ? k : next_bad[k + 1];
        auto usize = [&](uint32_t k) { return rm[k].isize <= kBgzfMaxBlock ? rm[k].isize : 0u; };
        auto lower = [&](uint64_t cfile) {
            uint32_t lo_ = 0, hi_ = n_range;
            while (lo_ < hi_) { const uint32_t mid = lo_ + (hi_ - lo_) / 2; if (rm[mid].cpos - 18 < cfile) lo_ = mid + 1; else hi_ = mid; }
            return lo_;
        };
        uint32_t seg_total = 0;
        for (const VChunk &ch : chunks) {
            const uint32_t k = lower(ch.u >> 16);
            if (k >= n_range || rm[k].cpos - 18 != (ch.u >> 16)) break;
            SegChunk sc; memset(&sc, 0, sizeof sc);
            sc.a = rm[k].upos - upos_lo + std::min<uint64_t>(ch.u & 0xffff, usize(k));
            const uint32_t kv = lower(ch.v >> 16);
            if (kv >= n_range) sc.b = total;
            else sc.b = rm[kv].upos - upos_lo + (rm[kv].cpos - 18 == (ch.v >> 16) ? std::min<uint64_t>(ch.v & 0xffff, usize(kv)) : 0);
            if (sc.b <= sc.a) sc.b = sc.a + 1;
            const uint32_t nb = next_bad[k];
            sc.dlim = nb < n_range ? rm[nb].upos - upos_lo : total;
            sc.seg_base = seg_total;
            const uint64_t ns = (sc.b - sc.a + seg_bytes - 1) / seg_bytes;
            if (seg_total + ns > 0x7fffffffull) return fail(err, errlen, RGX_ERR_FORMAT, "regtools_amd: region too large\n");
            seg_total += (uint32_t)ns;
            seg_chunks.push_back(sc);
        }
        if (seg_chunks.empty()) lim = pos0;
        else {
            DevBuf &b_ch = c->buf("seg_chunks");
            HIP_TRY(b_ch.ensure(seg_chunks.size() * sizeof(SegChunk) + 64));
            HIP_TRY(hipMemcpyAsync(b_ch.p, seg_chunks.data(), seg_chunks.size() * sizeof(SegChunk), hipMemcpyHostToDevice, st));
            geom.chunks = b_ch.as<SegChunk>(); geom.n_chunks = (uint32_t)seg_chunks.size();
        }
        mark("chunk table");
    }

    return kGoOn;
}

int EventsRun::stage_framing() {
    arena = c->buf("arena").as<uint8_t>();
    span = lim - pos0;
    n_seg = (uint32_t)((span + seg_bytes - 1) / seg_bytes);
    geom.pos0 = pos0; geom.lim = lim; geom.data_end = lim; geom.seg_bytes = seg_bytes;
    const int env_lite = 1;
    lite_walk = env_lite && !c->walk_strict;
    geom.lite_walk = lite_walk ? 1u : 0u;
    if (geom.chunks) {
        span = 0;
        for (const SegChunk &sc : seg_chunks) span += sc.b - sc.a;
        const SegChunk &lastc = seg_chunks.back();
        n_seg = lastc.seg_base + (uint32_t)((lastc.b - lastc.a + seg_bytes - 1) / seg_bytes);
        geom.data_end = total;
    }
    n_rec = 0;
    DevBuf &b_seg = c->buf("seg"), &b_tmp = c->buf("tmp");
    HIP_TRY(hipEventRecord(c->ev[2], st));
    sA = 0;
    emit_parts_ok = false; emit_parts = 0; emit_rows = 0; ev_lay = 0;
    memset(&ev_e, 0, sizeof ev_e);
    soa_cap = 0;
    memset(&soa, 0, sizeof soa);
    ev_base = nullptr; long_list = nullptr;
    if (n_seg) {
        const size_t per = (size_t)n_seg;
        HIP_TRY(b_seg.ensure(per * (8 + 8 + 4) * 2 + per * 4 + per * 12 + 64));
        HIP_TRY(c->buf("seg_cp").ensure(per * kSegCpSlots * 2 + 64));
        seg_cp = c->buf("seg_cp").as<uint16_t>();
        uint8_t *q = b_seg.as<uint8_t>();
        for (int k = 0; k < 2; ++k) { seg_start[k] = (uint64_t *)q; q += per * 8; seg_exit[k] = (uint64_t *)q; q += per * 8; }
        for (int k = 0; k < 2; ++k) { seg_cnt[k] = (uint32_t *)q; q += per * 4; }
        seg_base = (uint32_t *)q; q += per * 4;
        seg_iter_e = (uint32_t *)q; q += per * 4; seg_long_e = (uint32_t *)q; q += per * 4; seg_long_base_e = (uint32_t *)q;
        HIP_TRY(b_tmp.ensure(scan_tmp_words(n_seg) * 4 + 64));
        bool early = split_B && spec && !geom.chunks && seg_bytes == kSegBytes && cut_hi == UINT64_MAX && !empty_stream && lim == total;
        const bool env_early_emit = true;
        const bool small_ok = overlap_knobs().early_small;
        uint32_t waves_done = 0;
        for (size_t j = 0; early && j < early_parts.size(); ++j) {
            const EarlyPart &ep = early_parts[j];
            if (ep.upos <= pos0 + 2 * (uint64_t)kBgzfMaxBlock) continue;
            uint32_t sJ = (uint32_t)std::min<uint64_t>(n_seg, (ep.upos - kBgzfMaxBlock - pos0) / seg_bytes);
            if (small_ok ? (sJ < sA + 2 || n_seg - sJ < 1) : (sJ < sA + 1024 || n_seg - sJ < 64)) continue;
            HIP_TRY(hipMemsetAsync(d_sc + 83, 0, 4, st));
            for (size_t i = 0; i <= j; ++i) {
                const uint32_t w_end = early_parts[i].waves, w_beg = i ? early_parts[i - 1].waves : 0u;
                if (w_end > waves_done) { launch_wait_done(c->buf("gate_done").as<uint32_t>() + i, w_end - w_beg, d_sc + 83, st); waves_done = w_end; }
            }
            HIP_TRY(hipMemcpyAsync(h_sc + 83, d_sc + 83, 4, hipMemcpyDeviceToHost, st));
            if (trace) fprintf(stderr, "[rgx trace] early tail: part %zu: members < %u, segments [%u, %u) of %u\n", j, ep.members, sA, sJ, n_seg);
            bool ended_J = false;
            const uint32_t sweeps0 = P.framing_sweeps;
            const int rcJ = frame(sJ, sA, ended_J);
            if (rcJ != -1) return rcJ;
            const uint32_t n_rec_J = h_sc[3];
            uint64_t exit_J = 0;
            HIP_TRY(hipMemcpyAsync(h_sc + 92, seg_exit[cur] + (sJ - 1), 8, hipMemcpyDeviceToHost, st));
            HIP_TRY(hipStreamSynchronize(st));
            memcpy(&exit_J, h_sc + 92, 8);
            const bool reaches_J = exit_J > ep.upos;
            if (reaches_J && trace) fprintf(stderr,
                "[rgx trace] early tail: a record of the prefix ends at %llu, behind the inflated part (%llu): one pass\n", (unsigned long long)exit_J,
                (unsigned long long)ep.upos);
            const bool slow_J = P.framing_sweeps - sweeps0 > 2;
            P.framing_sweeps = sweeps0;
            const uint64_t span_J = (uint64_t)sJ * seg_bytes;
            if (h_sc[83]) { c->early_distrust = true; if (trace) fprintf(stderr,
                "[rgx trace] early tail: a wait for a part's waves timed out, this context no longer uses it\n"); }
            if (h_sc[83] || ended_J || slow_J || reaches_J || !n_rec_J || span_J / n_rec_J > kSparseRecordBytes ||
                (sA && n_rec_J > soa_cap)) { early = false; sA = 0; emit_parts_ok = false; emit_parts = 0; emit_rows = 0; break; }
            if (!sA) {
                HIP_TRY(soa_layout((size_t)((double)n_rec_J * ((double)n_seg / sJ) * 1.125) + 65536));
                cfg.insane_out = nullptr;
                if (lite_walk) { cfg.insane_out = d_sc + 82; HIP_TRY(hipMemsetAsync(d_sc + 82, 0, 4, st)); h_sc[82] = 0; }
            }
            launch_decode_seg(arena, geom, sJ, seg_start[cur], seg_base, seg_cnt[cur], cfg, soa, seg_iter_e, seg_long_e, seg_cp, true, st, sA);
            if (!sA) {
                DevBuf &b_ev0 = c->buf("events");
                ev_lay = b_ev0.cap > 256 ? (b_ev0.cap - 256) / 33 : 0;
                emit_parts_ok = env_early_emit && ev_lay >= 4096;
                if (emit_parts_ok) { HIP_TRY(b_tmp.ensure(scan_tmp_words((uint32_t)std::min<size_t>(soa_cap, 0xffffffffu)) * 4 + 64));
                    ev_e = ev_layout(b_ev0.as<uint8_t>(), ev_lay); }
            }
            if (emit_parts_ok && emit_parts < kGateParts - 1) {
                launch_scan_u32(soa.n_ev + emit_rows, ev_base + emit_rows, n_rec_J - emit_rows, d_sc + 84 + emit_parts, b_tmp.as<uint32_t>(), st);
                launch_emit_short(arena, n_rec_J, cfg, soa, ev_base, ev_e, st, emit_rows, d_sc + 84, emit_parts, (uint32_t)std::min<size_t>(ev_lay,
                    0xffffffffu));
                emit_rows = n_rec_J; ++emit_parts;
            }
            sA = sJ;
            mark("early tail: part framed and decoded");
        }
        HIP_TRY(join_B());
        const int rcF = frame(n_seg, sA, chain_ended);
        if (rcF != -1) return rcF;
        n_rec = h_sc[3];
    } else HIP_TRY(join_B());
    if (spec && !n_seg) {
        HIP_TRY(hipMemcpyAsync(h_sc, d_sc, 8, hipMemcpyDeviceToHost, st));
        HIP_TRY(hipMemcpyAsync(h_sc + kStatusEarly, d_sc + kStatusEarly, 8, hipMemcpyDeviceToHost, st));
        HIP_TRY(hipStreamSynchronize(st));
        if (h_sc[0] != 0xffffffffu || h_sc[kStatusEarly] != 0xffffffffu) {
            HIP_TRY(complete_upload());
            HIP_TRY(hipStreamSynchronize(copy_q));
            const int rc2 = prepare_events(c, d_bam, nullptr, bam_len, bai, bai_len, p, want_read_span, P, err, errlen, nullptr, false, region_to_file_end);
            P.t_begin = t_begin;
            return rc2;
        }
    }
    if (chain_ended) P.stream_ended = true;
    if (chain_ended && geom.chunks && m_hi < n_members_all && !region_to_file_end) {
        mark("region: chain ended, re-reading to the end of the file");
        if (overlap) { HIP_TRY(complete_upload()); HIP_TRY(hipStreamSynchronize(copy_q)); }
        const int rc2 = prepare_events(c, d_bam, nullptr, bam_len, bai, bai_len, p, want_read_span, P, err, errlen, d_true_sizes, false, true);
        P.t_begin = t_begin;
        return rc2;
    }
    HIP_TRY(hipEventRecord(c->ev[3], st));
    mark("framing (sync)");

    return kGoOn;
}

int EventsRun::stage_decode() {
    DevBuf &b_tmp = c->buf("tmp");
    n_events = 0; n_long = 0;
    n_iterated = 0;
    if (n_rec) {
        const size_t R = n_rec;
        uint32_t s_from = sA;
        if (sA && (R > soa_cap || chain_ended)) s_from = 0;
        if (!s_from) { HIP_TRY(soa_layout(R)); emit_parts_ok = false; }
        HIP_TRY(b_tmp.ensure(scan_tmp_words(n_rec) * 4 + 64));
        uint32_t *seg_iter = sA ? seg_iter_e : seg_cnt[cur ^ 1], *seg_long = sA ? seg_long_e : (uint32_t *)seg_start[cur ^ 1], *seg_long_base = sA ?
            seg_long_base_e : (uint32_t *)seg_exit[cur ^ 1];
        if (geom.chunks) {
            cfg.stop_out = d_sc + 80; cfg.stop_index = 0xffffffffu;
            HIP_TRY(hipMemsetAsync(d_sc + 80, 0xff, 4, st));
            HIP_TRY(hipMemsetAsync(d_sc + 81, 0, 4, st));
        }
        if (!s_from) {
            cfg.insane_out = nullptr;
            if (lite_walk) { cfg.insane_out = d_sc + 82; HIP_TRY(hipMemsetAsync(d_sc + 82, 0, 4, st)); h_sc[82] = 0; }
        }
        for (int pass = 0; pass < 2; ++pass) {
            launch_decode_seg(arena, geom, n_seg, seg_start[cur], seg_base, seg_cnt[cur], cfg, soa, seg_iter, seg_long, seg_cp,
                              span / n_rec <= kSparseRecordBytes, st, s_from);
            if (emit_parts_ok && s_from) {
                launch_scan_u32(soa.n_ev + emit_rows, ev_base + emit_rows, n_rec - emit_rows, d_sc + 84 + emit_parts, b_tmp.as<uint32_t>(), st);
                launch_emit_short(arena, n_rec, cfg, soa, ev_base, ev_e, st, emit_rows, d_sc + 84, emit_parts, (uint32_t)std::min<size_t>(ev_lay, 0xffffffffu));
                HIP_TRY(hipMemcpyAsync(h_sc + 84, d_sc + 84, 4 * kGateParts, hipMemcpyDeviceToHost, st));
            } else launch_scan_u32(soa.n_ev, ev_base, n_rec, d_sc + 4, b_tmp.as<uint32_t>(), st);
            launch_scan_u32(seg_iter, seg_iter, n_seg, d_sc + 8, b_tmp.as<uint32_t>(), st);
            launch_scan_u32(seg_long, seg_long_base, n_seg, d_sc + 5, b_tmp.as<uint32_t>(), st);
            HIP_TRY(hipMemcpyAsync(h_sc + 4, d_sc + 4, 24, hipMemcpyDeviceToHost, st));
            if (cfg.stop_out) HIP_TRY(hipMemcpyAsync(h_sc + 80, d_sc + 80, 8, hipMemcpyDeviceToHost, st));
            if (cfg.insane_out) HIP_TRY(hipMemcpyAsync(h_sc + 82, d_sc + 82, 4, hipMemcpyDeviceToHost, st));
            if (cfg.abort_out) HIP_TRY(hipMemcpyAsync(h_sc + 96, d_sc + 96, 4, hipMemcpyDeviceToHost, st));
            if (cfg.odd_count) HIP_TRY(hipMemcpyAsync(h_sc + 97, d_sc + 97, 4, hipMemcpyDeviceToHost, st));
            HIP_TRY(hipStreamSynchronize(st));
            if (cfg.insane_out && h_sc[82]) {
                mark("decode: a record fails bam_read1's test, starting over with the full walk");
                if (overlap) { HIP_TRY(complete_upload()); HIP_TRY(hipStreamSynchronize(copy_q)); }
                c->walk_strict = true;
                const int rc2 = prepare_events(c, d_bam, nullptr, bam_len, bai, bai_len, p, want_read_span, P, err, errlen, d_true_sizes, false,
                    region_to_file_end);
                c->walk_strict = false;
                P.t_begin = t_begin;
                return rc2;
            }
            if (pass || !cfg.stop_out || h_sc[80] == 0xffffffffu || h_sc[81] <= h_sc[80] + 1) break;
            cfg.stop_index = h_sc[80];
        }
        if (cfg.abort_out && h_sc[96] != 0xffffffffu && h_sc[96] < (cfg.stop_out ? cfg.stop_index : 0xffffffffu))
            return fail(err, errlen, RGX_ERR_ABORT,
                "regtools_amd: record %u has an auxiliary field of unknown type in front of its strand or barcode tag: the reference abort()s here\n",
                h_sc[96]);
        n_events = h_sc[4]; n_long = h_sc[5];
        if (emit_parts_ok && s_from) {
            uint64_t tot = 0;
            for (uint32_t k = 0; k <= emit_parts && k < kGateParts; ++k) tot += h_sc[84 + k];
            if (tot > ev_lay || tot > 0xffffffffull || n_long) {
                emit_parts_ok = false;
                launch_scan_u32(soa.n_ev, ev_base, n_rec, d_sc + 4, b_tmp.as<uint32_t>(), st);
                HIP_TRY(hipMemcpyAsync(h_sc + 4, d_sc + 4, 4, hipMemcpyDeviceToHost, st));
                HIP_TRY(hipStreamSynchronize(st));
                n_events = h_sc[4];
            } else n_events = (uint32_t)tot;
        }
        n_iterated = h_sc[8];
        if (cfg.odd_count && h_sc[97]) {
            const uint32_t cap = h_sc[97];
            DevBuf &b_odd = c->buf("odd_aux");
            HIP_TRY(b_odd.ensure((size_t)cap * 12 + 16));
            HIP_TRY(hipMemsetAsync(d_sc + 97, 0, 4, st));
            launch_collect_odd_aux(arena, soa, n_rec, cap, d_sc + 97, b_odd.as<int32_t>(), st);
            HIP_TRY(hipMemcpyAsync(h_sc + 97, d_sc + 97, 4, hipMemcpyDeviceToHost, st));
            HIP_TRY(hipStreamSynchronize(st));
            const uint32_t n_odd = std::min(h_sc[97], cap);
            std::vector<int32_t> rows((size_t)n_odd * 3);
            if (n_odd) { HIP_TRY(hipMemcpyAsync(rows.data(), b_odd.p, (size_t)n_odd * 12, hipMemcpyDeviceToHost, st)); HIP_TRY(hipStreamSynchronize(st)); }
            for (uint32_t k = 0; k < n_odd; ++k) P.odd_aux.push_back(Prep::OddAux{rows[3 * (size_t)k], rows[3 * (size_t)k + 1], rows[3 * (size_t)k + 2]});
        }
        if (geom.chunks && p->n_shards > 1 && h_sc[80] != 0xffffffffu) P.stream_ended = true;
        if (n_long) launch_long_fill(n_seg, seg_base, seg_cnt[cur], seg_long_base, cfg, soa, long_list, st);
    }
    HIP_TRY(hipEventRecord(c->ev[4], st));
    mark("decode+count (sync)");

    return kGoOn;
}

int EventsRun::stage_emit() {
    DevBuf &b_ev = c->buf("events");
    EventSoA ev; memset(&ev, 0, sizeof ev);
    if (n_events) {
        const size_t E = n_events;
        if (emit_parts_ok && n_rec) ev = ev_e;
        else {
            HIP_TRY(b_ev.ensure(E * (4 * 8 + 1) + 256));
            ev = ev_layout(b_ev.as<uint8_t>(), E);
            launch_emit_short(arena, n_rec, cfg, soa, ev_base, ev, st);
            launch_emit_long(arena, long_list, n_long, cfg, soa, ev_base, ev, st);
        }
        if (cfg.fa_data) {
            HIP_TRY(hipMemcpyAsync(h_sc + 64, d_sc + 64, 4, hipMemcpyDeviceToHost, st));
            HIP_TRY(hipStreamSynchronize(st));
            if (h_sc[64]) return fail(err, errlen, RGX_ERR_FASTA, "Unable to extract FASTA sequence for position %s\n\n",
                hdr.names[(size_t)(h_sc[64] - 1)].c_str());
        }
    }
    HIP_TRY(hipEventRecord(c->ev[5], st));

    P.hdr = hdr; P.arena = arena; P.soa = soa; P.ev = ev; P.n_rec = n_rec; P.n_events = n_events; P.n_range = n_range;
    P.n_iterated = n_iterated; P.total = total; P.t_begin = t_begin;
    return RGX_OK;
}

int prepare_events(rgx_ctx *c, const uint8_t *d_bam_in, const uint8_t *h_bam, size_t bam_len, const uint8_t *bai, size_t bai_len,
                          const rgx_extract_params *p, bool want_read_span, Prep &P, char *err, size_t errlen, const uint32_t *d_true_sizes,
                          bool allow_overlap, bool region_to_file_end, const SharedMembers *shared) {
    EventsRun r{c, d_bam_in, h_bam, bam_len, bai, bai_len, p, want_read_span, P, err, errlen, d_true_sizes, allow_overlap, region_to_file_end, shared};
    return r.run();
}
```

### regtools_amd/csrc/api_reduce.cpp

```cpp
#include "api_internal.h"

int reduce_events(rgx_ctx *c, EventSoA ev, uint32_t n_events, uint32_t group_bits, uint32_t ilen_bits, const uint32_t *rank_of_group_host,
                         uint32_t n_groups, HostRows &R, char *err, size_t errlen, bool view_only, RowMap *row_map, TableSink *sink, bool allow_preagg) {
    hipStream_t st = c->stream;
    uint32_t *d_sc = c->buf("scalars").as<uint32_t>();
    uint32_t *h_sc = (uint32_t *)c->pinned;
    DevBuf &b_sort = c->buf("sort"), &b_uni = c->buf("unique");
    c->last_rows_valid = false;
    uint32_t n_unique = 0;
    UniqueSoA u; memset(&u, 0, sizeof u);
    uint32_t *perm[2] = {nullptr, nullptr};
    uint32_t *final_perm = nullptr;
    uint32_t *chrom_rank_rows = nullptr;
    R = HostRows();
    if (n_events) {
        const bool preagg = !row_map && allow_preagg;
        PartialSoA pr; memset(&pr, 0, sizeof pr);
        uint32_t *ev_flag = nullptr;
        EventSoA sev = ev;
        uint32_t n_s = n_events;
        if (preagg) {
            DevBuf &b_par = c->buf("partials");
            const size_t Ev = n_events;
            HIP_TRY(b_par.ensure(Ev * 4 * 9 + scan_tmp_words(n_events) * 4 + 512));
            uint32_t *q = b_par.as<uint32_t>();
            pr.tid = q; q += Ev; pr.start = q; q += Ev; pr.ilen_cls = q; q += Ev; pr.ts = q; q += Ev; pr.te = q; q += Ev;
            pr.count = q; q += Ev; pr.first = q; q += Ev; pr.last = q; q += Ev; ev_flag = q;
            HIP_TRY(hipMemsetAsync(d_sc + 7, 0, 4, st));
            launch_preagg(ev, n_events, pr, d_sc + 7, st);
            HIP_TRY(hipMemcpyAsync(h_sc + 7, d_sc + 7, 4, hipMemcpyDeviceToHost, st));
            HIP_TRY(hipStreamSynchronize(st));
            n_s = h_sc[7];
            memset(&sev, 0, sizeof sev);
            sev.tid = pr.tid; sev.start = pr.start; sev.ilen_cls = pr.ilen_cls; sev.ts = pr.ts; sev.te = pr.te;
        }
        const size_t E = n_s;
        const size_t rtmp = radix_tmp_words(n_s) + scan_tmp_words(n_s) + 64;
        HIP_TRY(b_sort.ensure(E * 4 * 6 + rtmp * 4 + 256));
        uint32_t *q = b_sort.as<uint32_t>();
        perm[0] = q; q += E; perm[1] = q; q += E;
        uint32_t *key[2]; key[0] = q; q += E; key[1] = q; q += E;
        uint32_t *head = q; q += E; uint32_t *seg_excl = q; q += E;
        uint32_t *tmp = q;
        int pc = -1;
        auto sort_word = [&](const uint32_t *word, uint32_t nbits) {
            const uint32_t *kin = word;
            int kc = 0;
            if (pc >= 0) { launch_gather_u32(n_s, word, perm[pc], key[0], st); kin = key[0]; kc = 1; }
            for (uint32_t sh = 0; sh < nbits; sh += 8) {
                const uint32_t bits = std::min<uint32_t>(8, nbits - sh);
                const int nxt = pc < 0 ? 0 : pc ^ 1;
                launch_radix_pass_keyed(kin, key[kc], sh, bits, pc < 0 ? nullptr : perm[pc], perm[nxt], n_s, tmp, st);
                kin = key[kc]; kc ^= 1;
                pc = nxt;
            }
        };
        sort_word(sev.ilen_cls, ilen_bits);
        sort_word(sev.start, 32);
        sort_word(sev.tid, group_bits);
        const uint32_t *sorted = perm[pc];
        launch_heads(sev, sorted, n_s, head, st);
        launch_scan_u32(head, seg_excl, n_s, d_sc + 6, tmp, st);
        HIP_TRY(hipMemcpyAsync(h_sc + 6, d_sc + 6, 4, hipMemcpyDeviceToHost, st));
        HIP_TRY(hipStreamSynchronize(st));
        n_unique = h_sc[6];

        const size_t U = n_unique;
        const size_t utmp = radix_tmp_words(n_unique) + 64;
        HIP_TRY(b_uni.ensure(U * 4 * 13 + U + utmp * 4 + 256));
        uint32_t *w = b_uni.as<uint32_t>();
        u.tid = w; w += U; u.start = w; w += U; u.end = w; w += U; u.ts_min = w; w += U; u.te_max = w; w += U; u.count = w; w += U;
        u.first_seen = w; w += U; u.last_seen = w; w += U; u.name_rank = w; w += U;
        uint32_t *head_pos = w; w += U; chrom_rank_rows = w; w += U;
        uint32_t *uperm[2]; uperm[0] = w; w += U; uperm[1] = w; w += U;
        uint32_t *utmp_p = w; w += utmp;
        u.strand = (uint8_t *)w;
        launch_fill_u32(u.ts_min, 0xffffffffu, U, st);
        launch_fill_u32(u.te_max, 0u, U, st);
        if (preagg) {
            launch_fill_u32(u.count, 0u, U, st);
            launch_fill_u32(u.first_seen, 0xffffffffu, U, st);
            launch_fill_u32(u.last_seen, 0u, U, st);
            launch_reduce_partials(pr, sorted, head, seg_excl, n_s, u, st);
            HIP_TRY(hipMemsetAsync(ev_flag, 0, (size_t)n_events * 4, st));
            launch_reduce_finish_partials(ev.strand, n_unique, u, ev_flag, st);
            launch_scan_u32(ev_flag, ev_flag, n_events, nullptr, ev_flag + n_events, st);
            launch_name_rank(n_unique, ev_flag, u, st);
        } else {
            launch_reduce(ev, sorted, head, seg_excl, n_events, u, head_pos, st);
            if (row_map) {
                DevBuf &b_map = c->buf("row_map");
                HIP_TRY(b_map.ensure((E + U) * 4 + 256));
                row_map->ev_urow = b_map.as<uint32_t>(); row_map->urow_pos = row_map->ev_urow + E;
                launch_event_urow(sorted, head, seg_excl, n_events, row_map->ev_urow, st);
            }
            uint32_t *first_flag = head;
            HIP_TRY(hipMemsetAsync(first_flag, 0, E * 4, st));
            launch_reduce_finish(ev, sorted, n_events, n_unique, head_pos, u, first_flag, st);
            launch_scan_u32(first_flag, seg_excl, n_events, nullptr, tmp, st);
            launch_name_rank(n_unique, seg_excl, u, st);
        }

        uint32_t rk = 0;
        for (uint32_t i = 0; i < n_groups; ++i) rk = std::max(rk, rank_of_group_host[i]);
        DevBuf &b_rank = c->buf("rank");
        HIP_TRY(b_rank.ensure((size_t)n_groups * 4 + 64));
        c->rank_stage.assign(rank_of_group_host, rank_of_group_host + n_groups);
        HIP_TRY(hipMemcpyAsync(b_rank.p, c->rank_stage.data(), (size_t)n_groups * 4, hipMemcpyHostToDevice, st));
        launch_gather_u32(n_unique, b_rank.as<uint32_t>(), u.tid, chrom_rank_rows, st);
        int upc = -1;
        auto usort = [&](const uint32_t *word, uint32_t nbits) {
            for (uint32_t sh = 0; sh < nbits; sh += 8) {
                const uint32_t bits = std::min<uint32_t>(8, nbits - sh);
                const int nxt = upc < 0 ? 0 : upc ^ 1;
                launch_radix_pass(word, sh, bits, upc < 0 ? nullptr : uperm[upc], uperm[nxt], n_unique, utmp_p, st);
                upc = nxt;
            }
        };
        usort(u.name_rank, std::max<uint32_t>(1, bitlen(n_unique)));
        usort(u.te_max, 32);
        usort(u.ts_min, 32);
        usort(chrom_rank_rows, std::max<uint32_t>(1, bitlen(rk)));
        final_perm = uperm[upc];
        if (row_map) launch_inverse_perm(final_perm, n_unique, row_map->urow_pos, st);
        if (!n_unique) HIP_TRY(hipStreamSynchronize(st));
    }

    if (n_unique) {
        const size_t U = n_unique;
        DevBuf &b_out = c->buf("rows_out");
        HIP_TRY(b_out.ensure(U * 40 + 256));
        launch_rows_out(u, final_perm, n_unique, b_out.as<uint32_t>(), st);
        if (sink) {
            DevBuf &b_tab = c->buf("table_dev");
            const size_t bytes = table_block_bytes(U);
            HIP_TRY(b_tab.ensure(bytes + 256));
            launch_rows_table(u, final_perm, n_unique, sink->min_anchor, b_tab.as<uint8_t>(), st);
            rgx_junction_table *t = table_alloc(*sink->hdr, U, false, c->tables_made++ > 0);
            if (!t) { (void)hipStreamSynchronize(st); return fail(err, errlen, RGX_ERR_DEVICE, "regtools_amd: no memory for the result table\n"); }
            hipError_t e_ = hipMemcpyAsync(((TableBox *)t)->block, b_tab.p, bytes, hipMemcpyDeviceToHost, st);
            if (e_ == hipSuccess) e_ = hipStreamSynchronize(st);
            if (e_ != hipSuccess) { rgx_table_free(t); return fail(err, errlen, RGX_ERR_DEVICE, "HIP error %s copying the result table\n",
                hipGetErrorString(e_)); }
            sink->table = t; R.n = U;
            return RGX_OK;
        }
        if (U * 40 > c->pinned_rows_cap) {
            if (c->pinned_rows) (void)hipHostFree(c->pinned_rows);
            c->pinned_rows = nullptr; c->pinned_rows_cap = 0;
            const size_t want = U * 40 + U * 5 + 4096;
            HIP_TRY(hipHostMalloc(&c->pinned_rows, want, hipHostMallocDefault));
            c->pinned_rows_cap = want;
        }
        HIP_TRY(hipMemcpyAsync(c->pinned_rows, b_out.p, U * 40, hipMemcpyDeviceToHost, st));
        HIP_TRY(hipStreamSynchronize(st));
        const uint32_t *hp = (const uint32_t *)c->pinned_rows;
        R.cols = hp; R.n = U;
        if (view_only) return RGX_OK;
        auto col = [&](size_t k, std::vector<uint32_t> &dst) { dst.assign(hp + k * U, hp + (k + 1) * U); };
        col(0, R.group); col(1, R.start); col(2, R.end); col(3, R.ts); col(4, R.te); col(5, R.count); col(6, R.name_rank); col(7, R.first_seen); col(8,
            R.last_seen);
        R.strand.resize(U);
        for (size_t i = 0; i < U; ++i) R.strand[i] = (uint8_t)hp[9 * U + i];
        R.n = U;
    }
    return RGX_OK;
}

int barcode_rows(rgx_ctx *c, const Prep &P, const RowMap &rm, const rgx_extract_params *p, rgx_junction_table *t, char *err, size_t errlen) {
    hipStream_t st = c->stream;
    const double t0 = now_ms();
    const size_t E = P.n_events, U = t->n;
    t->bc_row_begin = (uint64_t *)calloc(U + 1, 8);
    if (!E) { t->bc_count = (uint32_t *)calloc(1, 4); t->bc_str_begin = (uint64_t *)calloc(1, 8); t->bc_text = (char *)calloc(1, 1);
        t->bc_insert_rank = (uint32_t *)calloc(1, 4); return RGX_OK; }
    uint32_t *d_sc = c->buf("scalars").as<uint32_t>();
    uint32_t *h_sc = (uint32_t *)c->pinned;
    DevBuf &b_bc = c->buf("barcodes");
    const size_t rtmp = radix_tmp_words((uint32_t)E) + scan_tmp_words((uint32_t)E) + 64;
    HIP_TRY(b_bc.ensure(E * (8 + 4 * 4 + 4 * 4 + 8 + 4 * 5) + rtmp * 4 + 512));
    uint8_t *q = b_bc.as<uint8_t>();
    BarcodeEv b;
    b.off = (uint64_t *)q; q += E * 8;
    uint64_t *pair_off = (uint64_t *)q; q += E * 8;
    b.len = (uint32_t *)q; q += E * 4; b.h_lo = (uint32_t *)q; q += E * 4; b.h_hi = (uint32_t *)q; q += E * 4; b.row = (uint32_t *)q; q += E * 4;
    uint32_t *perm[2]; perm[0] = (uint32_t *)q; q += E * 4; perm[1] = (uint32_t *)q; q += E * 4;
    uint32_t *head = (uint32_t *)q; q += E * 4; uint32_t *seg_excl = (uint32_t *)q; q += E * 4;
    uint32_t *pair_row = (uint32_t *)q; q += E * 4; uint32_t *pair_first = (uint32_t *)q; q += E * 4; uint32_t *pair_pos = (uint32_t *)q; q += E * 4;
    uint32_t *pair_len = (uint32_t *)q; q += E * 4; uint32_t *pair_count = (uint32_t *)q; q += E * 4;
    uint32_t *tmp = (uint32_t *)q;
    uint32_t *flags = d_sc + 72;
    HIP_TRY(hipMemsetAsync(flags, 0, 8, st));
    launch_bc_event_keys(P.arena, (uint32_t)E, P.ev.read, P.soa.rec_off, rm.ev_urow, rm.urow_pos, (uint8_t)p->barcode_tag[0], (uint8_t)p->barcode_tag[1], b,
        flags, st);
    int pc = -1;
    auto sort_word = [&](const uint32_t *word, uint32_t nbits) {
        for (uint32_t sh = 0; sh < nbits; sh += 8) {
            const int nxt = pc < 0 ? 0 : pc ^ 1;
            launch_radix_pass(word, sh, std::min<uint32_t>(8, nbits - sh), pc < 0 ? nullptr : perm[pc], perm[nxt], (uint32_t)E, tmp, st);
            pc = nxt;
        }
    };
    sort_word(b.h_lo, 32); sort_word(b.h_hi, 32);
    sort_word(b.row, std::max<uint32_t>(1, bitlen((uint32_t)std::max<size_t>(U, 1) - 1)));
    const uint32_t *sorted = perm[pc];
    launch_bc_heads(P.arena, b, sorted, (uint32_t)E, head, flags, st);
    launch_scan_u32(head, seg_excl, (uint32_t)E, d_sc + 74, tmp, st);
    HIP_TRY(hipMemcpyAsync(h_sc + 72, d_sc + 72, 12, hipMemcpyDeviceToHost, st));
    HIP_TRY(hipStreamSynchronize(st));
    if (h_sc[72]) return fail(err, errlen, RGX_ERR_FORMAT,
        "regtools_amd: the %c%c tag of an alignment is not a string (the reference dies on such input)\n\n", p->barcode_tag[0], p->barcode_tag[1]);
    if (h_sc[73]) return fail(err, errlen, RGX_ERR_DEVICE, "regtools_amd: two different barcodes of one junction share a 64-bit hash; not handled\n\n");
    const uint32_t n_pairs = h_sc[74];
    launch_bc_pairs(b, sorted, head, seg_excl, (uint32_t)E, pair_row, pair_first, pair_pos, pair_off, pair_len, st);
    launch_bc_counts(n_pairs, (uint32_t)E, pair_pos, pair_count, st);
    uint32_t *str_begin = head;
    launch_scan_u32(pair_len, str_begin, n_pairs, d_sc + 75, tmp, st);
    HIP_TRY(hipMemcpyAsync(h_sc + 75, d_sc + 75, 4, hipMemcpyDeviceToHost, st));
    HIP_TRY(hipStreamSynchronize(st));
    const size_t text_len = h_sc[75];
    DevBuf &b_txt = c->buf("barcode_text");
    HIP_TRY(b_txt.ensure(text_len + 256));
    launch_bc_gather(P.arena, n_pairs, pair_off, pair_len, str_begin, b_txt.as<uint8_t>(), st);
    std::vector<uint32_t> h_row(n_pairs), h_first(n_pairs), h_count(n_pairs), h_begin(n_pairs), h_len(n_pairs);
    std::vector<char> h_text(text_len + 1);
    HIP_TRY(hipMemcpyAsync(h_row.data(), pair_row, (size_t)n_pairs * 4, hipMemcpyDeviceToHost, st));
    HIP_TRY(hipMemcpyAsync(h_first.data(), pair_first, (size_t)n_pairs * 4, hipMemcpyDeviceToHost, st));
    HIP_TRY(hipMemcpyAsync(h_count.data(), pair_count, (size_t)n_pairs * 4, hipMemcpyDeviceToHost, st));
    HIP_TRY(hipMemcpyAsync(h_begin.data(), str_begin, (size_t)n_pairs * 4, hipMemcpyDeviceToHost, st));
    HIP_TRY(hipMemcpyAsync(h_len.data(), pair_len, (size_t)n_pairs * 4, hipMemcpyDeviceToHost, st));
    if (text_len) HIP_TRY(hipMemcpyAsync(h_text.data(), b_txt.p, text_len, hipMemcpyDeviceToHost, st));
    HIP_TRY(hipStreamSynchronize(st));

    t->bc_count = (uint32_t *)calloc((size_t)n_pairs + 1, 4);
    t->bc_str_begin = (uint64_t *)calloc((size_t)n_pairs + 1, 8);
    t->bc_text = (char *)malloc(text_len + 1);
    t->bc_insert_rank = (uint32_t *)calloc((size_t)n_pairs + 1, 4);
    std::vector<uint32_t> rank_of(n_pairs);
    std::vector<uint32_t> run_begin(U + 1, 0);
    for (uint32_t k = 0; k < n_pairs; ++k) run_begin[h_row[k] + 1]++;
    for (size_t r = 0; r < U; ++r) run_begin[r + 1] += run_begin[r];
    for (size_t r = 0; r <= U; ++r) t->bc_row_begin[r] = run_begin[r];
    const unsigned n_thr = (unsigned)std::max<size_t>(1, std::min<size_t>(16, U / 256));
    std::vector<std::thread> pool;
    auto work = [&](size_t r0, size_t r1) {
        std::vector<uint32_t> idx;
        for (size_t r = r0; r < r1; ++r) {
            const uint32_t k0 = run_begin[r], k1 = run_begin[r + 1];
            idx.resize(k1 - k0);
            for (uint32_t k = k0; k < k1; ++k) idx[k - k0] = k;
            std::sort(idx.begin(), idx.end(), [&](uint32_t x, uint32_t y) { return h_first[x] < h_first[y]; });
            for (uint32_t q = 0; q < idx.size(); ++q) rank_of[idx[q]] = q;
            std::unordered_map<std::string, int> m;
            for (uint32_t k : idx) m.insert(std::pair<std::string, int>(std::string(h_text.data() + h_begin[k], h_len[k]), (int)k));
            uint32_t o = k0;
            for (auto it = m.begin(); it != m.end(); ++it, ++o) { t->bc_count[o] = h_count[(uint32_t)it->second]; t->bc_str_begin[o] = (uint64_t)it->second;
                 t->bc_insert_rank[o] = rank_of[(uint32_t)it->second]; }
        }
    };
    for (unsigned w = 0; w < n_thr; ++w) pool.emplace_back(work, U * w / n_thr, U * (w + 1) / n_thr);
    for (auto &th : pool) th.join();
    uint64_t pos = 0;
    for (uint32_t o = 0; o < n_pairs; ++o) {
        const uint32_t k = (uint32_t)t->bc_str_begin[o];
        t->bc_str_begin[o] = pos;
        memcpy(t->bc_text + pos, h_text.data() + h_begin[k], h_len[k]);
        pos += h_len[k];
    }
    t->bc_str_begin[n_pairs] = pos;
    t->ms_barcodes = now_ms() - t0;
    return RGX_OK;
}

void chrom_string_ranks(const BamHeader &hdr, std::vector<uint32_t> &rank_of_tid) {
    const size_t n = hdr.names.size();
    std::vector<uint32_t> order(n);
    rank_of_tid.assign(n ? n : 1, 0);
    for (size_t i = 0; i < n; ++i) order[i] = (uint32_t)i;
    std::sort(order.begin(), order.end(), [&](uint32_t a, uint32_t b) { return hdr.names[a] < hdr.names[b]; });
    uint32_t rk = 0;
    for (size_t i = 0; i < n; ++i) {
        if (i > 0 && hdr.names[order[i]] != hdr.names[order[i - 1]]) ++rk;
        rank_of_tid[order[i]] = rk;
    }
}

int run_pipeline(rgx_ctx *c, const uint8_t *d_bam_in, const uint8_t *h_bam, size_t bam_len, const uint8_t *bai, size_t bai_len,
                        const rgx_extract_params *p, rgx_junction_table **out, char *err, size_t errlen, const SharedMembers *shared) {
    *out = nullptr;
    c->last_rows_valid = false;
    Prep P;
    int rc = prepare_events(c, d_bam_in, h_bam, bam_len, bai, bai_len, p, false, P, err, errlen, nullptr, true, false, shared);
    if (rc != RGX_OK) return rc;
    hipStream_t st = c->stream;
    const int32_t n_ref = (int32_t)P.hdr.names.size();
    std::vector<uint32_t> rank_of_tid;
    chrom_string_ranks(P.hdr, rank_of_tid);
    HostRows R;
    RowMap rm;
    TableSink sink; sink.hdr = &P.hdr; sink.min_anchor = p->min_anchor;
    rc = reduce_events(c, P.ev, P.n_events, std::max<uint32_t>(1, bitlen((uint32_t)std::max(n_ref - 1, 0))), std::min<uint32_t>(32, bitlen(p->max_intron) + 2),
                       rank_of_tid.data(), (uint32_t)std::max(n_ref, 1), R, err, errlen, true, p->barcodes ? &rm : nullptr, &sink);
    if (rc != RGX_OK) return rc;
    c->last_rows = R.n; c->last_records = P.n_iterated; c->last_events = P.n_events; c->last_bytes = P.total; c->last_rows_valid = true;
    HIP_TRY(hipEventRecord(c->ev[6], st));
    rgx_junction_table *t = sink.table ? sink.table : table_alloc(P.hdr, 0);
    if (!t) return fail(err, errlen, RGX_ERR_DEVICE, "regtools_amd: no memory for the result table\n");
    if (R.n >= 100000000u) host_sort_rows(t);
    if (p->barcodes) {
        if (R.n >= 100000000u) { rgx_table_free(t); return fail(err, errlen, RGX_ERR_ARG, "regtools_amd: -b with 10^8 or more junctions is not supported\n"); }
        rc = barcode_rows(c, P, rm, p, t, err, errlen);
        if (rc != RGX_OK) { rgx_table_free(t); return rc; }
    }
    t->n_records = P.n_iterated;
    t->n_events = P.n_events; t->inflated_bytes = P.total; t->compressed_bytes = bam_len; t->n_members = P.n_range; t->framing_sweeps = P.framing_sweeps;
        t->stream_ended = P.stream_ended ? 1 : 0;
    float ms = 0;
    HIP_TRY(hipEventSynchronize(c->ev[6]));
    (void)hipEventElapsedTime(&ms, c->ev[0], c->ev[1]); t->ms_inflate = ms;
    t->ms_inflate_launch = 0;
    if (c->launch_timed && hipEventSynchronize(c->ev_launch[1]) == hipSuccess && hipEventElapsedTime(&ms, c->ev_launch[0],
        c->ev_launch[1]) == hipSuccess) t->ms_inflate_launch = ms;
    (void)hipEventElapsedTime(&ms, c->ev[2], c->ev[4]); t->ms_records = ms;
    (void)hipEventElapsedTime(&ms, c->ev[4], c->ev[5]); t->ms_scan = ms;
    (void)hipEventElapsedTime(&ms, c->ev[5], c->ev[6]); t->ms_reduce = ms;
    t->ms_total = now_ms() - P.t_begin;
    if (c->arena_retired) { c->arena_retired->release(); delete c->arena_retired; c->arena_retired = nullptr; }
    if (getenv("REGTOOLS_AMD_TRACE")) {
        fprintf(stderr, "[rgx trace] total %.3f ms; device buffers grown so far: %llu allocations, %.1f MB, %.3f ms\n", t->ms_total,
            (unsigned long long)g_alloc_stats.calls,
                (double)g_alloc_stats.bytes / 1e6, g_alloc_stats.ms);
    }
    *out = t;
    return RGX_OK;
}
```

### regtools_amd/csrc/kernels.h

```cpp
#pragma once
#include <hip/hip_runtime.h>

#include "common.h"
#include "bam_core.h"

namespace rgx {

constexpr uint32_t kSegBytes = 16384;
constexpr uint32_t kSparseRecordBytes = 2048;
constexpr uint32_t kSegCpSlots = 64;
constexpr uint64_t kChainEnd = ~0ull;
constexpr uint64_t kChainUnknown = ~0ull - 1;

size_t inflate_scratch_bytes(uint32_t n_members);
hipError_t pending_launch_error();
struct InflateGate {
    const uint32_t *flags = nullptr;
    uint32_t epoch = 0;
    uint32_t n_chunks = 0;
    uint64_t lo = 0, chunk_bytes = 1;
    uint32_t *done = nullptr;
    uint32_t part_start[7] = {0xffffffffu, 0xffffffffu, 0xffffffffu, 0xffffffffu, 0xffffffffu, 0xffffffffu, 0xffffffffu};
};
constexpr uint32_t kGateParts = 8;
constexpr uint32_t kInflateSortGroup = 1024;
void launch_wait_done(const uint32_t *done, uint32_t expected, uint32_t *timed_out, hipStream_t stream);
constexpr uint32_t kStatusEarly = 76;
void launch_inflate(const uint8_t *comp, const Member *members, uint32_t n_members, uint8_t *arena, uint64_t upos_bias, uint32_t *len_scratch,
                    uint32_t *status , hipStream_t stream, uint32_t ignore_below = 0 ,
                    uint32_t index_bias = 0 ,
                    bool piece = false ,
                    int form = 0 ,
                    uint8_t *bad_flags = nullptr ,
                    int plan = 1 ,
                    bool check_layout = false ,
                    InflateGate gate = InflateGate() );
bool inflate_takes_coop(uint32_t n_members);
void launch_gate_set(uint32_t *flag, uint32_t epoch, hipStream_t stream);
inline int inflate_plan_for(uint64_t compressed_bytes, uint64_t inflated_bytes) {
    return compressed_bytes * 32 > inflated_bytes ? 1 : 0;
}

constexpr uint32_t kMagicTile = 4096;
void launch_magic_count(const uint8_t *bam, uint64_t len, uint32_t n_tiles, uint32_t *tile_cnt, hipStream_t stream);
void launch_magic_fill(const uint8_t *bam, uint64_t len, uint32_t n_tiles, const uint32_t *tile_base, uint64_t *cand, hipStream_t stream);
void launch_member_link(const uint8_t *bam, uint64_t len, const uint64_t *cand, uint32_t n, uint32_t *next, uint32_t *isize,
                        uint32_t *reach, uint64_t root2 , hipStream_t stream);
void launch_member_jump(uint32_t n, const uint32_t *next_in, uint32_t *next_out, uint32_t *reach, hipStream_t stream);
void launch_member_compact(const uint8_t *bam, uint64_t len, const uint64_t *cand, const uint32_t *isize, const uint32_t *reach, const uint32_t *rank,
                           uint32_t n, Member *members, uint32_t *isize_compact, hipStream_t stream);
void launch_member_upos(Member *members, const uint32_t *isize_compact, const uint32_t *n_members , uint64_t *total, hipStream_t stream);
void launch_member_query(const Member *members, const uint32_t *n_members , const uint64_t *q_coff, uint32_t n_q, uint32_t *q_index,
                         uint64_t *q_upos, hipStream_t stream);
void launch_inflate_probe(const uint8_t *comp, const Member *members, uint32_t n_members, uint8_t *slots, uint32_t *len_scratch, uint32_t *sizes,
                          hipStream_t stream);
void launch_member_fix(Member *members, uint32_t *isize_compact, uint32_t max_members, const uint32_t *n_members , const uint32_t *fix,
                       hipStream_t stream);
void launch_member_stop(const Member *members, uint32_t max_members, const uint32_t *n_members , const uint32_t *from , uint32_t *stop,
                        hipStream_t stream);

struct SegChunk { uint64_t a, b, dlim; uint32_t seg_base, pad; };
struct DecodeKnobs { bool wave_form = false; int seg_bytes = 0; };
const DecodeKnobs &decode_knobs();
struct SegGeom {
    uint64_t pos0, lim;
    uint64_t data_end;
    const SegChunk *chunks; uint32_t n_chunks;
    uint32_t seg_bytes;
    uint32_t lite_walk;
};
constexpr uint32_t kSegBytesLong = 131072;
constexpr uint32_t kLongRecordBytes = 2048;
void launch_seg_walk(const uint8_t *arena, SegGeom g, uint32_t n_seg, int32_t n_ref,
                     uint64_t *seg_start, uint64_t *seg_exit, uint32_t *seg_cnt, uint16_t *seg_cp , hipStream_t stream,
                     uint32_t s_begin = 0 );
void launch_seg_verify(const uint8_t *arena, SegGeom g, uint32_t n_seg,
                       const uint64_t *seg_start_in, const uint64_t *seg_exit_in, const uint32_t *seg_cnt_in,
                       uint64_t *seg_start_out, uint64_t *seg_exit_out, uint32_t *seg_cnt_out,
                       uint32_t *status , uint16_t *seg_cp, hipStream_t stream);
void launch_seg_truncate(SegGeom g, uint32_t n_seg, uint32_t last, uint64_t *seg_start, uint64_t *seg_exit, uint32_t *seg_cnt, hipStream_t stream);

struct ReadSoA {
    int32_t  *tid, *pos;
    uint32_t *flag_nc;
    uint64_t *cig_off;
    uint8_t  *strand;
    uint32_t *n_ev;
    uint64_t *rec_off;
};
struct ExtractCfg {
    int32_t  n_ref;
    int32_t  strandness;
    uint8_t  tag0, tag1;
    uint32_t min_anchor, min_intron, max_intron;
    int32_t  region_tid;
    int32_t  region_beg, region_end;
    uint32_t long_threshold;
    const uint8_t *fa_data;
    const struct FaContig *fa_tab;
    uint32_t *fa_missing;
    uint32_t *stop_out;
    uint32_t stop_index;
    uint32_t *insane_out;
    uint32_t *abort_out;
    uint8_t  bc0, bc1;
    uint32_t *odd_count;
};
void launch_collect_odd_aux(const uint8_t *arena, ReadSoA soa, uint32_t n_rec, uint32_t cap, uint32_t *count, int32_t *out, hipStream_t stream);

void launch_decode_seg(const uint8_t *arena, SegGeom g, uint32_t n_seg, const uint64_t *seg_start, const uint32_t *seg_base,
                       const uint32_t *seg_cnt, ExtractCfg cfg, ReadSoA soa, uint32_t *seg_iter, uint32_t *seg_long, const uint16_t *seg_cp,
                       bool staged , hipStream_t stream,
                       uint32_t s_begin = 0 );
void launch_long_fill(uint32_t n_seg, const uint32_t *seg_base, const uint32_t *seg_cnt, const uint32_t *seg_long_base, ExtractCfg cfg, ReadSoA soa,
                      uint32_t *long_list, hipStream_t stream);

struct EventSoA {
    uint32_t *tid, *start, *ilen_cls;
    uint32_t *ts, *te;
    uint32_t *rpos, *rend;
    uint8_t  *strand;
    uint32_t *read;
};
void launch_emit_short(const uint8_t *arena, uint32_t n_rec, ExtractCfg cfg, ReadSoA soa, const uint32_t *ev_base,
                       EventSoA ev, hipStream_t stream, uint32_t row_begin = 0 ,
                       const uint32_t *part_totals = nullptr, uint32_t n_parts = 0 ,
                       uint32_t slot_cap = 0xffffffffu );
void launch_emit_long(const uint8_t *arena, const uint32_t *long_list, uint32_t n_long,
                      ExtractCfg cfg, ReadSoA soa, const uint32_t *ev_base, EventSoA ev, hipStream_t stream);

size_t scan_tmp_words(uint32_t n);
void launch_scan_u32(const uint32_t *in, uint32_t *out, uint32_t n, uint32_t *total, uint32_t *tmp, hipStream_t stream);

size_t radix_tmp_words(uint32_t n);
void launch_radix_pass(const uint32_t *word, uint32_t shift, uint32_t bits, const uint32_t *perm_in, uint32_t *perm_out,
                       uint32_t n, uint32_t *tmp, hipStream_t stream);
void launch_radix_pass_keyed(const uint32_t *key_in, uint32_t *key_out, uint32_t shift, uint32_t bits, const uint32_t *perm_in, uint32_t *perm_out,
                             uint32_t n, uint32_t *tmp, hipStream_t stream);

struct UniqueSoA {
    uint32_t *tid, *start, *end, *ts_min, *te_max, *count, *first_seen, *last_seen, *name_rank;
    uint8_t  *strand;
};
struct PartialSoA { uint32_t *tid, *start, *ilen_cls, *ts, *te, *count, *first, *last; };
void launch_preagg(EventSoA ev, uint32_t n, PartialSoA p, uint32_t *p_total , hipStream_t stream);
void launch_reduce_partials(PartialSoA p, const uint32_t *perm, const uint32_t *head, const uint32_t *seg_excl, uint32_t n, UniqueSoA u, hipStream_t stream);
void launch_reduce_finish_partials(const uint8_t *ev_strand, uint32_t n_unique, UniqueSoA u, uint32_t *first_flag , hipStream_t stream);
void launch_heads(EventSoA ev, const uint32_t *perm, uint32_t n, uint32_t *head, hipStream_t stream);
void launch_reduce(EventSoA ev, const uint32_t *perm, const uint32_t *head, const uint32_t *seg_excl, uint32_t n, UniqueSoA u,
                   uint32_t *head_pos, hipStream_t stream);
void launch_reduce_finish(EventSoA ev, const uint32_t *perm, uint32_t n, uint32_t n_unique, const uint32_t *head_pos, UniqueSoA u,
                          uint32_t *first_flag, hipStream_t stream);
void launch_name_rank(uint32_t n_unique, const uint32_t *flag_scan, UniqueSoA u, hipStream_t stream);
void launch_gather_u32(uint32_t n, const uint32_t *table, const uint32_t *idx, uint32_t *out, hipStream_t stream);
void launch_fill_u32(uint32_t *p, uint32_t v, size_t n, hipStream_t stream);
void launch_rows_out(UniqueSoA u, const uint32_t *order, uint32_t n, uint32_t *out, hipStream_t stream);
RGX_HD size_t table_block_rows(uint64_t n) { return ((size_t)n + 1 + 15) & ~(size_t)15; }
RGX_HD size_t table_block_bytes(uint64_t n) { return table_block_rows(n) * (8 * 3 + 4 * 6 + 3); }
void launch_rows_table(UniqueSoA u, const uint32_t *order, uint32_t n, uint32_t min_anchor, uint8_t *out, hipStream_t stream);


struct BarcodeEv { uint64_t *off; uint32_t *len, *h_lo, *h_hi, *row; };
void launch_event_urow(const uint32_t *sorted, const uint32_t *head, const uint32_t *seg_excl, uint32_t n, uint32_t *ev_urow, hipStream_t stream);
void launch_inverse_perm(const uint32_t *perm, uint32_t n, uint32_t *inv, hipStream_t stream);
void launch_bc_event_keys(const uint8_t *arena, uint32_t n_events, const uint32_t *ev_read, const uint64_t *rec_off, const uint32_t *ev_urow,
                          const uint32_t *urow_pos, uint8_t t0, uint8_t t1, BarcodeEv b, uint32_t *flags, hipStream_t stream);
void launch_bc_heads(const uint8_t *arena, BarcodeEv b, const uint32_t *perm, uint32_t n, uint32_t *head, uint32_t *flags, hipStream_t stream);
void launch_bc_pairs(BarcodeEv b, const uint32_t *perm, const uint32_t *head, const uint32_t *seg_excl, uint32_t n, uint32_t *pair_row,
                     uint32_t *pair_first, uint32_t *pair_pos, uint64_t *pair_off, uint32_t *pair_len, hipStream_t stream);
void launch_bc_counts(uint32_t n_pairs, uint32_t n, const uint32_t *pair_pos, uint32_t *pair_count, hipStream_t stream);
void launch_bc_gather(const uint8_t *arena, uint32_t n_pairs, const uint64_t *pair_off, const uint32_t *pair_len, const uint32_t *str_begin,
                      uint8_t *text, hipStream_t stream);

struct GtfView;
struct VariantOpts;
}
#include "cse_core.h"
namespace rgx {
void launch_variant_scan(bool fill, GtfView g, uint32_t n, const int32_t *chrom, const uint32_t *pos0, VariantOpts o, uint32_t *count, const uint32_t *base,
                         uint32_t *ces, uint32_t *cee, uint32_t *hit_tx, uint32_t *hit_ad, unsigned long long *visits ,
                         hipStream_t stream, uint32_t *last_score = nullptr );
void launch_junction_scan(bool fill, GtfView g, uint32_t n, const int32_t *chrom, const uint32_t *js, const uint32_t *je, const uint8_t *strand, uint32_t *count,
                          const uint32_t *base, uint32_t *flags, uint32_t *item_kind, uint32_t *item_a, uint32_t *item_b, unsigned long long *visits,
                          uint32_t *visit_each , hipStream_t stream);
void launch_max_span(EventSoA ev, uint32_t n, uint32_t *out , hipStream_t stream);
constexpr uint32_t kWinSlices = 4;
void launch_window_pairs(bool fill, EventSoA ev, uint32_t n_events, uint32_t n_win, const int32_t *w_tid, const int32_t *w_beg, const int32_t *w_end,
                         const uint32_t *max_span, uint32_t *w_lo, uint32_t *w_hi ,
                         uint32_t *count, const uint32_t *base, uint32_t *pair_ev, uint32_t *pair_win, hipStream_t stream);
void launch_assoc_pairs(bool fill, uint32_t n_win, const int32_t *w_chrom, const uint32_t *w_ces, const uint32_t *w_cee, const uint32_t *chrom_off,
                        const uint32_t *j_start, const uint32_t *j_end, uint32_t *count, const uint32_t *base, uint32_t *pair_j, uint32_t *pair_win, hipStream_t stream);
void launch_pair_gather(EventSoA ev, const uint32_t *pair_ev, const uint32_t *pair_win, uint32_t n, EventSoA out, hipStream_t stream);

struct MergeSoA { uint32_t *tid, *start, *end, *ts, *te, *count, *cls, *first, *shard; uint32_t *strand; };
struct MergeUnique { uint32_t *tid, *start, *end, *ts, *te, *count, *first, *last_shard, *strand; };
void launch_merge_unpack(const uint32_t *rows, uint32_t stride_rows, uint32_t n_parts, const uint32_t *part_rows, const uint32_t *part_base, MergeSoA m, hipStream_t st);
void launch_cols_to_packed(const uint32_t *cols , uint32_t n, uint32_t *out, hipStream_t st);
void launch_merge_heads(MergeSoA m, const uint32_t *sorted, uint32_t n, uint32_t *head, hipStream_t st);
void launch_merge_reduce(MergeSoA m, const uint32_t *sorted, const uint32_t *head, const uint32_t *seg_excl, uint32_t n, MergeUnique u , hipStream_t st);
void launch_merge_rank(const uint32_t *by_first, uint32_t n, uint32_t *name_rank, hipStream_t st);
void launch_merge_pack(MergeUnique u, const uint32_t *order, const uint32_t *name_rank, uint32_t n, uint32_t *out, hipStream_t st);
void launch_merge_table(MergeUnique u, const uint32_t *order, const uint32_t *name_rank, uint32_t n, uint32_t min_anchor, uint8_t *out, hipStream_t st);

}
```

### regtools_amd/csrc/kernels.hip

```cpp
#include "kernels.h"

#include <mutex>
#include <type_traits>

#include "bam_core.h"
#include "inflate_core.h"
#include "inflate_coop.h"
#include "inflate_ring.h"
#include "inflate_wave.h"

namespace rgx {

__device__ __forceinline__ uint32_t lane_id() { return threadIdx.x & 63u; }
__device__ __forceinline__ uint64_t lanemask_lt() { return (1ull << lane_id()) - 1ull; }

__device__ __forceinline__ uint32_t wave_incl_scan(uint32_t v) {
#pragma unroll
    for (int d = 1; d < 64; d <<= 1) {
        uint32_t t = __shfl_up(v, d, 64);
        if ((int)lane_id() >= d) v += t;
    }
    return v;
}

// ... 1293 lines not shown
    uint32_t nx = n, isz = 0xffffffffu;
    if (blen >= 26 && off + blen <= len) {
        isz = ld32(bam + off + blen - 4);
        if (isz == 0xffffffffu) isz = 0xfffffffeu;
        const uint64_t want = off + blen;
        uint32_t lo = i + 1, hi = n;
        while (lo < hi) { const uint32_t mid = (lo + hi) >> 1; if (cand[mid] < want) lo = mid + 1; else hi = mid; }
        if (lo < n && cand[lo] == want) nx = lo;
    } else nx = 0xffffffffu;
    next[i] = nx; isize[i] = isz;
    reach[i] = ((i == 0 && off == 0) || off == root2) ? 1u : 0u;
}

__global__ void k_member_jump(uint32_t n, const uint32_t *__restrict__ next_in, uint32_t *next_out, uint32_t *reach) {
    const uint32_t i = blockIdx.x * blockDim.x + threadIdx.x;
    if (i >= n) return;
    const uint32_t nx = next_in[i];
    if (nx < n) {
        if (reach[i]) reach[nx] = 1u;
        next_out[i] = next_in[nx];
    } else next_out[i] = nx;
}

__global__ void k_member_compact(const uint8_t *__restrict__ bam, uint64_t len, const uint64_t *__restrict__ cand, const uint32_t *__restrict__ isize,
                                 const uint32_t *__restrict__ reach, const uint32_t *__restrict__ rank, uint32_t n, Member *members, uint32_t *isize_compact) {
    const uint32_t i = blockIdx.x * blockDim.x + threadIdx.x;
    if (i >= n || !reach[i]) return;
    const uint64_t off = cand[i];
    const uint32_t blen = (uint32_t)ld16(bam + off + 16) + 1;
    const uint32_t r = rank[i];
    Member m; m.cpos = off + 18; m.upos = 0; m.isize = isize[i];
    m.clen = blen >= 26 ? blen - 18 : 0;
    if (m.cpos + m.clen + 8 > len) m.clen = len > m.cpos + 8 ? (uint32_t)(len - 8 - m.cpos) : 0;
    members[r] = m;
    isize_compact[r] = (isize[i] <= kBgzfMaxBlock) ? isize[i] : 0u;
}

__global__ __launch_bounds__(256) void k_member_upos(Member *members, const uint32_t *__restrict__ isz, const uint32_t *__restrict__ n_ptr, uint64_t *total) {
    __shared__ uint32_t s_wave[4];
    const uint32_t n = *n_ptr;
    uint64_t carry = 0;
    for (uint32_t base = 0; base < n; base += 2048) {
        const uint32_t i0 = base + threadIdx.x * 8;
        uint32_t v[8], sum = 0;
#pragma unroll
        for (int k = 0; k < 8; ++k) { v[k] = i0 + k < n ? isz[i0 + k] : 0u; sum += v[k]; }
        uint32_t tot; uint32_t ex = block_excl_scan_256(sum, s_wave, tot);
#pragma unroll
        for (int k = 0; k < 8; ++k) { if (i0 + k < n) members[i0 + k].upos = carry + ex; ex += v[k]; }
        carry += tot;
    }
    if (threadIdx.x == 0) *total = carry;
}

__global__ void k_member_query(const Member *__restrict__ members, const uint32_t *__restrict__ n_ptr, const uint64_t *__restrict__ q_coff, uint32_t n_q,
                               uint32_t *q_index, uint64_t *q_upos) {
    const uint32_t k = blockIdx.x * blockDim.x + threadIdx.x;
    if (k >= n_q) return;
    const uint32_t n = *n_ptr;
    const uint64_t want = q_coff[k] + 18;
    uint32_t lo = 0, hi = n;
    while (lo < hi) { const uint32_t mid = (lo + hi) >> 1; if (members[mid].cpos < want) lo = mid + 1; else hi = mid; }
    const bool hit = lo < n && members[lo].cpos == want;
    q_index[k] = hit ? lo : n;
    q_upos[k] = hit ? members[lo].upos : ~0ull;
}

__global__ void k_member_fix(Member *members, uint32_t *isize_compact, const uint32_t *__restrict__ n_ptr, const uint32_t *__restrict__ fix) {
    const uint32_t i = blockIdx.x * blockDim.x + threadIdx.x;
    if (i >= *n_ptr) return;
    const uint32_t sz = fix[i];
    members[i].isize = sz;
    isize_compact[i] = sz <= kBgzfMaxBlock ? sz : 0u;
}
__global__ void k_member_stop(const Member *__restrict__ members, const uint32_t *__restrict__ n_ptr, const uint32_t *__restrict__ from_ptr, uint32_t *stop) {
    const uint32_t n = *n_ptr;
    const uint32_t i = blockIdx.x * blockDim.x + threadIdx.x;
    if (i < *from_ptr) return;
    if (i < n && (members[i].isize == 0 || members[i].isize > kBgzfMaxBlock)) atomicMin(stop, i);
}

void launch_magic_count(const uint8_t *bam, uint64_t len, uint32_t n_tiles, uint32_t *tile_cnt, hipStream_t stream) {
    if (n_tiles) hipLaunchKernelGGL(k_magic_count, dim3(n_tiles), dim3(256), 0, stream, bam, len, tile_cnt);
}
void launch_magic_fill(const uint8_t *bam, uint64_t len, uint32_t n_tiles, const uint32_t *tile_base, uint64_t *cand, hipStream_t stream) {
    if (n_tiles) hipLaunchKernelGGL(k_magic_fill, dim3(n_tiles), dim3(256), 0, stream, bam, len, tile_base, cand);
}
void launch_member_link(const uint8_t *bam, uint64_t len, const uint64_t *cand, uint32_t n, uint32_t *next, uint32_t *isize, uint32_t *reach,
                        uint64_t root2, hipStream_t stream) {
    if (n) hipLaunchKernelGGL(k_member_link, dim3((n + 255) / 256), dim3(256), 0, stream, bam, len, cand, n, next, isize, reach, root2);
}
void launch_member_jump(uint32_t n, const uint32_t *next_in, uint32_t *next_out, uint32_t *reach, hipStream_t stream) {
    if (n) hipLaunchKernelGGL(k_member_jump, dim3((n + 255) / 256), dim3(256), 0, stream, n, next_in, next_out, reach);
}
void launch_member_compact(const uint8_t *bam, uint64_t len, const uint64_t *cand, const uint32_t *isize, const uint32_t *reach, const uint32_t *rank, uint32_t n,
                           Member *members, uint32_t *isize_compact, hipStream_t stream) {
    if (n) hipLaunchKernelGGL(k_member_compact, dim3((n + 255) / 256), dim3(256), 0, stream, bam, len, cand, isize, reach, rank, n, members, isize_compact);
}
void launch_member_upos(Member *members, const uint32_t *isize_compact, const uint32_t *n_members, uint64_t *total, hipStream_t stream) {
    hipLaunchKernelGGL(k_member_upos, dim3(1), dim3(256), 0, stream, members, isize_compact, n_members, total);
}
void launch_member_query(const Member *members, const uint32_t *n_members, const uint64_t *q_coff, uint32_t n_q, uint32_t *q_index, uint64_t *q_upos,
                         hipStream_t stream) {
    if (n_q) hipLaunchKernelGGL(k_member_query, dim3((n_q + 63) / 64), dim3(64), 0, stream, members, n_members, q_coff, n_q, q_index, q_upos);
}
void launch_member_fix(Member *members, uint32_t *isize_compact, uint32_t max_members, const uint32_t *n_members, const uint32_t *fix, hipStream_t stream) {
    if (max_members) hipLaunchKernelGGL(k_member_fix, dim3((max_members + 255) / 256), dim3(256), 0, stream, members, isize_compact, n_members, fix);
}
void launch_member_stop(const Member *members, uint32_t max_members, const uint32_t *n_members, const uint32_t *from, uint32_t *stop, hipStream_t stream) {
    if (max_members) hipLaunchKernelGGL(k_member_stop, dim3((max_members + 255) / 256), dim3(256), 0, stream, members, n_members, from, stop);
}

__global__ void k_heads(EventSoA ev, const uint32_t *__restrict__ perm, uint32_t n, uint32_t *head) {
    const uint32_t i = blockIdx.x * blockDim.x + threadIdx.x;
    if (i >= n) return;
    uint32_t h = 1;
    if (i > 0) {
        const uint32_t a = perm[i], b = perm[i - 1];
        h = (ev.tid[a] != ev.tid[b]) || (ev.start[a] != ev.start[b]) || (ev.ilen_cls[a] != ev.ilen_cls[b]);
    }
    head[i] = h;
}

__global__ void k_reduce(EventSoA ev, const uint32_t *__restrict__ perm, const uint32_t *__restrict__ head,
                         const uint32_t *__restrict__ seg_excl, uint32_t n, UniqueSoA u, uint32_t *head_pos) {
    const uint32_t i = blockIdx.x * blockDim.x + threadIdx.x;
    const bool valid = i < n;
    uint32_t row = 0, ts = 0xffffffffu, te = 0, hd = 0;
    if (valid) {
        const uint32_t e = perm[i];
        hd = head[i];
        row = seg_excl[i] + hd - 1;
        ts = ev.ts[e]; te = ev.te[e];
        if (hd) {
            head_pos[row] = i;
            u.tid[row] = ev.tid[e]; u.start[row] = ev.start[e]; u.end[row] = ev.start[e] + (ev.ilen_cls[e] >> 2);
            u.first_seen[row] = e;
        }
    }
    const uint32_t lane = lane_id();
#pragma unroll
    for (int d = 1; d < 64; d <<= 1) {
        const uint32_t r2 = __shfl_down(row, d, 64), ts2 = __shfl_down(ts, d, 64), te2 = __shfl_down(te, d, 64);
        const bool v2 = __shfl_down((uint32_t)valid, d, 64) != 0;
        if (lane + d < 64 && v2 && r2 == row) { ts = min(ts, ts2); te = max(te, te2); }
    }
    const uint32_t prev_row = __shfl_up(row, 1, 64);
    const bool run_head = valid && (lane == 0 || prev_row != row);
    if (run_head) { atomicMin(&u.ts_min[row], ts); atomicMax(&u.te_max[row], te); }
}

constexpr uint32_t kAggEmpty = 0xffffffffu;
template <uint32_t kAggTile>
__global__ __launch_bounds__(256) void k_preagg(EventSoA ev, uint32_t n, PartialSoA p, uint32_t *p_total) {
    constexpr uint32_t kAggSlots = 2 * kAggTile;
    __shared__ uint32_t s_tid[kAggTile], s_start[kAggTile], s_ilen[kAggTile], s_slot[kAggSlots];
    __shared__ uint32_t s_cnt[kAggTile], s_ts[kAggTile], s_te[kAggTile], s_first[kAggTile], s_last[kAggTile];
    __shared__ uint32_t s_wave[4], s_base;
    const uint32_t base = blockIdx.x * kAggTile, t = threadIdx.x;
#pragma unroll
    for (uint32_t k = 0; k < kAggTile / 256; ++k) {
        const uint32_t i = t + 256 * k, e = base + i;
        if (e < n) { s_tid[i] = ev.tid[e]; s_start[i] = ev.start[e]; s_ilen[i] = ev.ilen_cls[e]; }
        s_cnt[i] = 0; s_ts[i] = 0xffffffffu; s_te[i] = 0; s_first[i] = 0xffffffffu; s_last[i] = 0;
        s_slot[i] = kAggEmpty; s_slot[i + kAggTile] = kAggEmpty;
    }
    __syncthreads();
    uint32_t mine = 0;
#pragma unroll
    for (uint32_t k = 0; k < kAggTile / 256; ++k) {
        const uint32_t i = t + 256 * k, e = base + i;
        if (e < n) {
            const uint32_t kt = s_tid[i], ks = s_start[i], kl = s_ilen[i];
            uint32_t h = ks * 0x9E3779B1u ^ kl * 0x85EBCA6Bu ^ kt * 0xC2B2AE35u;
            h = (h ^ h >> 15) & (kAggSlots - 1);
            uint32_t leader;
            for (;;) {
                const uint32_t prev = atomicCAS(&s_slot[h], kAggEmpty, i);
                if (prev == kAggEmpty) { leader = i; mine |= 1u << k; break; }
                if (s_tid[prev] == kt && s_start[prev] == ks && s_ilen[prev] == kl) { leader = prev; break; }
                h = (h + 1) & (kAggSlots - 1);
            }
            atomicAdd(&s_cnt[leader], 1u);
            atomicMin(&s_ts[leader], ev.ts[e]); atomicMax(&s_te[leader], ev.te[e]);
            atomicMin(&s_first[leader], i); atomicMax(&s_last[leader], i);
        }
    }
    __syncthreads();
    uint32_t tot;
    uint32_t at = block_excl_scan_256((uint32_t)__popc(mine), s_wave, tot);
    if (t == 0) s_base = tot ? atomicAdd(p_total, tot) : 0u;
    __syncthreads();
    at += s_base;
#pragma unroll
    for (uint32_t k = 0; k < kAggTile / 256; ++k) {
        if (mine >> k & 1u) {
            const uint32_t i = t + 256 * k;
            p.tid[at] = s_tid[i]; p.start[at] = s_start[i]; p.ilen_cls[at] = s_ilen[i];
            p.count[at] = s_cnt[i]; p.ts[at] = s_ts[i]; p.te[at] = s_te[i]; p.first[at] = base + s_first[i]; p.last[at] = base + s_last[i];
            ++at;
        }
    }
}

__global__ void k_reduce_partials(PartialSoA p, const uint32_t *__restrict__ perm, const uint32_t *__restrict__ head,
                                  const uint32_t *__restrict__ seg_excl, uint32_t n, UniqueSoA u) {
    const uint32_t i = blockIdx.x * blockDim.x + threadIdx.x;
    const bool valid = i < n;
    uint32_t row = 0, ts = 0xffffffffu, te = 0, cnt = 0, first = 0xffffffffu, last = 0;
    if (valid) {
        const uint32_t e = perm[i];
        const uint32_t hd = head[i];
        row = seg_excl[i] + hd - 1;
        ts = p.ts[e]; te = p.te[e]; cnt = p.count[e]; first = p.first[e]; last = p.last[e];
        if (hd) { u.tid[row] = p.tid[e]; u.start[row] = p.start[e]; u.end[row] = p.start[e] + (p.ilen_cls[e] >> 2); }
    }
    const uint32_t lane = lane_id();
#pragma unroll
    for (int d = 1; d < 64; d <<= 1) {
        const uint32_t r2 = __shfl_down(row, d, 64), ts2 = __shfl_down(ts, d, 64), te2 = __shfl_down(te, d, 64), c2 = __shfl_down(cnt, d, 64);
        const uint32_t f2 = __shfl_down(first, d, 64), l2 = __shfl_down(last, d, 64);
        const bool v2 = __shfl_down((uint32_t)valid, d, 64) != 0;
        if (lane + d < 64 && v2 && r2 == row) { ts = min(ts, ts2); te = max(te, te2); cnt += c2; first = min(first, f2); last = max(last, l2); }
    }
    const uint32_t prev_row = __shfl_up(row, 1, 64);
    const bool run_head = valid && (lane == 0 || prev_row != row);
    if (run_head) {
        atomicMin(&u.ts_min[row], ts); atomicMax(&u.te_max[row], te); atomicAdd(&u.count[row], cnt);
        atomicMin(&u.first_seen[row], first); atomicMax(&u.last_seen[row], last);
    }
}
__global__ void k_reduce_finish_partials(const uint8_t *__restrict__ ev_strand, uint32_t n_unique, UniqueSoA u, uint32_t *first_flag) {
    const uint32_t r = blockIdx.x * blockDim.x + threadIdx.x;
    if (r >= n_unique) return;
    u.strand[r] = ev_strand[u.last_seen[r]];
    first_flag[u.first_seen[r]] = 1;
}

__global__ void k_reduce_finish(EventSoA ev, const uint32_t *__restrict__ perm, uint32_t n, uint32_t n_unique,
                                const uint32_t *__restrict__ head_pos, UniqueSoA u, uint32_t *first_flag) {
    const uint32_t r = blockIdx.x * blockDim.x + threadIdx.x;
    if (r >= n_unique) return;
    const uint32_t hp = head_pos[r], nx = (r + 1 < n_unique) ? head_pos[r + 1] : n;
    u.count[r] = nx - hp;
    const uint32_t last = perm[nx - 1];
    u.last_seen[r] = last;
    u.strand[r] = ev.strand[last];
    first_flag[u.first_seen[r]] = 1;
}

__global__ void k_name_rank(uint32_t n_unique, const uint32_t *__restrict__ flag_scan, UniqueSoA u) {
    const uint32_t r = blockIdx.x * blockDim.x + threadIdx.x;
    if (r < n_unique) u.name_rank[r] = flag_scan[u.first_seen[r]] + 1;
}

__global__ void k_gather_u32(uint32_t n, const uint32_t *__restrict__ table, const uint32_t *__restrict__ idx, uint32_t *out) {
    const uint32_t r = blockIdx.x * blockDim.x + threadIdx.x;
    if (r < n) out[r] = table[idx[r]];
}

__global__ void k_rows_out(UniqueSoA u, const uint32_t *__restrict__ order, uint32_t n, uint32_t *out) {
    const uint32_t i = blockIdx.x * blockDim.x + threadIdx.x;
    if (i >= n) return;
    const uint32_t s = order[i];
    const size_t N = n;
    out[i] = u.tid[s]; out[N + i] = u.start[s]; out[2 * N + i] = u.end[s]; out[3 * N + i] = u.ts_min[s]; out[4 * N + i] = u.te_max[s];
    out[5 * N + i] = u.count[s]; out[6 * N + i] = u.name_rank[s]; out[7 * N + i] = u.first_seen[s]; out[8 * N + i] = u.last_seen[s];
    out[9 * N + i] = u.strand[s];
}

__device__ __forceinline__ void table_row(uint8_t *out, size_t m, uint32_t i, uint32_t tid, uint32_t start, uint32_t end, uint32_t ts, uint32_t te, uint32_t count,
                                          uint64_t name_index, uint64_t first, uint64_t last, uint32_t strand, uint32_t min_anchor) {
    uint64_t *q8 = (uint64_t *)out;
    q8[i] = name_index; q8[m + i] = first; q8[2 * m + i] = last;
    uint32_t *q4 = (uint32_t *)(out + m * 24);
    q4[i] = tid; q4[m + i] = start; q4[2 * m + i] = end; q4[3 * m + i] = ts; q4[4 * m + i] = te; q4[5 * m + i] = count;
    uint8_t *q1 = out + m * 48;
    q1[i] = (uint8_t)strand;
    q1[m + i] = (uint32_t)(start - ts) >= min_anchor;
    q1[2 * m + i] = (uint32_t)(te - end) >= min_anchor;
}
__global__ void k_rows_table(UniqueSoA u, const uint32_t *__restrict__ order, uint32_t n, uint32_t min_anchor, uint8_t *out) {
    const uint32_t i = blockIdx.x * blockDim.x + threadIdx.x;
    if (i >= n) return;
    const uint32_t s = order[i];
    table_row(out, table_block_rows(n), i, u.tid[s], u.start[s], u.end[s], u.ts_min[s], u.te_max[s], u.count[s], u.name_rank[s], u.first_seen[s], u.last_seen[s], u.strand[s], min_anchor);
}

__global__ void k_fill_u32(uint32_t *p, uint32_t v, size_t n) {
    const size_t i = (size_t)blockIdx.x * blockDim.x + threadIdx.x;
    if (i < n) p[i] = v;
}

void launch_heads(EventSoA ev, const uint32_t *perm, uint32_t n, uint32_t *head, hipStream_t stream) {
    if (n) hipLaunchKernelGGL(k_heads, dim3((n + 255) / 256), dim3(256), 0, stream, ev, perm, n, head);
}
void launch_reduce(EventSoA ev, const uint32_t *perm, const uint32_t *head, const uint32_t *seg_excl, uint32_t n, UniqueSoA u,
                   uint32_t *head_pos, hipStream_t stream) {
    if (n) hipLaunchKernelGGL(k_reduce, dim3((n + 255) / 256), dim3(256), 0, stream, ev, perm, head, seg_excl, n, u, head_pos);
}
void launch_reduce_finish(EventSoA ev, const uint32_t *perm, uint32_t n, uint32_t n_unique, const uint32_t *head_pos, UniqueSoA u,
                          uint32_t *first_flag, hipStream_t stream) {
    if (n_unique) hipLaunchKernelGGL(k_reduce_finish, dim3((n_unique + 255) / 256), dim3(256), 0, stream, ev, perm, n, n_unique, head_pos, u, first_flag);
}
void launch_name_rank(uint32_t n_unique, const uint32_t *flag_scan, UniqueSoA u, hipStream_t stream) {
    if (n_unique) hipLaunchKernelGGL(k_name_rank, dim3((n_unique + 255) / 256), dim3(256), 0, stream, n_unique, flag_scan, u);
}
void launch_gather_u32(uint32_t n, const uint32_t *table, const uint32_t *idx, uint32_t *out, hipStream_t stream) {
    if (n) hipLaunchKernelGGL(k_gather_u32, dim3((n + 255) / 256), dim3(256), 0, stream, n, table, idx, out);
}
void launch_rows_out(UniqueSoA u, const uint32_t *order, uint32_t n, uint32_t *out, hipStream_t stream) {
    if (n) hipLaunchKernelGGL(k_rows_out, dim3((n + 255) / 256), dim3(256), 0, stream, u, order, n, out);
}
void launch_rows_table(UniqueSoA u, const uint32_t *order, uint32_t n, uint32_t min_anchor, uint8_t *out, hipStream_t stream) {
    if (n) hipLaunchKernelGGL(k_rows_table, dim3((n + 255) / 256), dim3(256), 0, stream, u, order, n, min_anchor, out);
}
void launch_preagg(EventSoA ev, uint32_t n, PartialSoA p, uint32_t *p_total, hipStream_t stream) {
    if (!n) return;
    hipLaunchKernelGGL(k_preagg<1024>, dim3((n + 1023) / 1024), dim3(256), 0, stream, ev, n, p, p_total);
}
void launch_reduce_partials(PartialSoA p, const uint32_t *perm, const uint32_t *head, const uint32_t *seg_excl, uint32_t n, UniqueSoA u, hipStream_t stream) {
    if (n) hipLaunchKernelGGL(k_reduce_partials, dim3((n + 255) / 256), dim3(256), 0, stream, p, perm, head, seg_excl, n, u);
}
void launch_reduce_finish_partials(const uint8_t *ev_strand, uint32_t n_unique, UniqueSoA u, uint32_t *first_flag, hipStream_t stream) {
    if (n_unique) hipLaunchKernelGGL(k_reduce_finish_partials, dim3((n_unique + 255) / 256), dim3(256), 0, stream, ev_strand, n_unique, u, first_flag);
}
void launch_fill_u32(uint32_t *p, uint32_t v, size_t n, hipStream_t stream) {
    if (n) hipLaunchKernelGGL(k_fill_u32, dim3((unsigned)((n + 255) / 256)), dim3(256), 0, stream, p, v, n);
}

}
```

Measured before the change: 2.091 billion alignments/s.

## Overlap per-part pre-aggregation on side stream and replace sort-based grouping with hash table

Runs the per-block hash pre-aggregation of junction events incrementally on a side stream as each early-emitted part is produced, so that reduction overlaps record parsing. The final group-by over partial rows switches from a multi-pass radix sort to a global atomic hash insert plus atomic reduce. Name ranks are then derived from an ordering by first-seen index. This removes the serial post-parse preagg and sort passes, at the cost of extra side-stream events, quiesce synchronisation, and atomic contention in the hash table. It also adds an exported standalone radix-sort entry point.

```diff
diff --git a/include/regtools_amd.h b/include/regtools_amd.h
--- a/include/regtools_amd.h
+++ b/include/regtools_amd.h
@@ -126,6 +126,8 @@
 int  rgx_k_inflate_form(int form, const void *d_comp, const rgx_member *d_members, uint32_t n_members,
                         void *d_arena, uint32_t *d_status, void *stream);
 
+int  rgx_k_radix_sort(const uint32_t *d_keys, uint32_t n, uint32_t key_bits, int keyed, uint32_t *d_perm_out, void *stream);
+
 typedef struct {
     const char *vcf_path, *bam_path, *fasta_path, *gtf_path;
     const char *out_tsv;
diff --git a/regtools_amd/_ffi.py b/regtools_amd/_ffi.py
--- a/regtools_amd/_ffi.py
+++ b/regtools_amd/_ffi.py
@@ -42,7 +42,7 @@
            "rgx_associate", "rgx_variants_annotate", "rgx_junctions_annotate", "rgx_junctions_annotate_opts", "rgx_table_merge_device", "rgx_window_join", "rgx_window_rows_free", "rgx_last_table_pack_device",
            "rgx_host_alloc", "rgx_host_free", "rgx_extract_multi", "rgx_extract_multi_mem", "rgx_multi_exchange_kind", "rgx_k_inflate_form", "rgx_table_merge_barcodes",
            "rgx_table_pack_barcodes", "rgx_table_unpack_barcodes", "rgx_identify_multi", "rgx_ctx_arena_trials",
-           "rgx_pipeline_create", "rgx_pipeline_depth", "rgx_pipeline_ctx", "rgx_extract_submit", "rgx_extract_wait", "rgx_pipeline_destroy"]
+           "rgx_pipeline_create", "rgx_pipeline_depth", "rgx_pipeline_ctx", "rgx_extract_submit", "rgx_extract_wait", "rgx_pipeline_destroy", "rgx_k_radix_sort"]
 
 
 class IdentifyParams(C.Structure):
@@ -140,6 +140,7 @@
         L.rgx_table_format_barcodes.restype = C.c_size_t
         L.rgx_k_inflate.argtypes = [C.c_void_p, C.c_void_p, C.c_uint32, C.c_void_p, C.c_void_p, C.c_void_p]
         L.rgx_k_inflate_form.argtypes = [C.c_int, C.c_void_p, C.c_void_p, C.c_uint32, C.c_void_p, C.c_void_p, C.c_void_p]
+        L.rgx_k_radix_sort.argtypes = [C.c_void_p, C.c_uint32, C.c_uint32, C.c_int, C.c_void_p, C.c_void_p]
         L.rgx_identify_params_default.argtypes = [P(IdentifyParams)]
         L.rgx_identify.argtypes = [C.c_void_p, P(IdentifyParams), P(IdentifyStats), C.c_char_p, C.c_size_t]
         L.rgx_associate.argtypes = L.rgx_identify.argtypes
diff --git a/regtools_amd/csrc/api_ctx.cpp b/regtools_amd/csrc/api_ctx.cpp
--- a/regtools_amd/csrc/api_ctx.cpp
+++ b/regtools_amd/csrc/api_ctx.cpp
@@ -74,6 +74,7 @@
         if ((e = hipStreamCreateWithPriority(&c->side[k], hipStreamNonBlocking, 0)) != hipSuccess) return e;
         if ((e = hipEventCreateWithFlags(&c->ev_side[k], hipEventDisableTiming)) != hipSuccess) return e;
     }
+    for (auto &ev : c->ev_pre) if ((e = hipEventCreateWithFlags(&ev, hipEventDisableTiming)) != hipSuccess) return e;
     return hipEventCreateWithFlags(&c->ev_ready, hipEventDisableTiming);
 }
 
@@ -106,6 +107,7 @@
     ktime_collect(c);
     for (auto &e : c->kfree) (void)hipEventDestroy(e);
     for (auto &e : c->ev_side) if (e) (void)hipEventDestroy(e);
+    for (auto &e : c->ev_pre) if (e) (void)hipEventDestroy(e);
     if (c->ev_ready) (void)hipEventDestroy(c->ev_ready);
     if (c->ev_packed) (void)hipEventDestroy(c->ev_packed);
     for (auto &q : c->side) if (q) (void)hipStreamDestroy(q);
diff --git a/regtools_amd/csrc/api_entry.cpp b/regtools_amd/csrc/api_entry.cpp
--- a/regtools_amd/csrc/api_entry.cpp
+++ b/regtools_amd/csrc/api_entry.cpp
@@ -55,6 +55,34 @@
     }
     launch_inflate((const uint8_t *)d_comp, (const Member *)d_members, n_members, (uint8_t *)d_arena, 0, (uint32_t *)scratch, d_status, (hipStream_t)stream,
         0, 0, false, form, nullptr, 1, true);
+    return hipGetLastError() == hipSuccess ? RGX_OK : RGX_ERR_DEVICE;
+}
+
+extern "C" int rgx_k_radix_sort(const uint32_t *d_keys, uint32_t n, uint32_t key_bits, int keyed, uint32_t *d_perm_out, void *stream) {
+    if (!d_keys || !d_perm_out || !key_bits || key_bits > 32) return RGX_ERR_ARG;
+    if (!n) return RGX_OK;
+    hipStream_t st = (hipStream_t)stream;
+    static void *scratch = nullptr; static size_t scratch_cap = 0;
+    const size_t N = n, need = (N * 4 + radix_tmp_words(n)) * 4 + 256;
+    if (need > scratch_cap) {
+        if (scratch) (void)hipFree(scratch);
+        if (hipMalloc(&scratch, need) != hipSuccess) { scratch = nullptr; scratch_cap = 0; return RGX_ERR_DEVICE; }
+        scratch_cap = need;
+    }
+    uint32_t *q = (uint32_t *)scratch;
+    uint32_t *perm[2], *key[2];
+    perm[0] = q; q += N; perm[1] = q; q += N; key[0] = q; q += N; key[1] = q; q += N;
+    uint32_t *tmp = q;
+    const uint32_t *kin = d_keys;
+    int pc = -1, kc = 0;
+    for (uint32_t sh = 0; sh < key_bits; sh += 8) {
+        const uint32_t bits = std::min<uint32_t>(8, key_bits - sh);
+        const int nxt = pc < 0 ? 0 : pc ^ 1;
+        if (keyed) { launch_radix_pass_keyed(kin, key[kc], sh, bits, pc < 0 ? nullptr : perm[pc], perm[nxt], n, tmp, st); kin = key[kc]; kc ^= 1; }
+        else launch_radix_pass(d_keys, sh, bits, pc < 0 ? nullptr : perm[pc], perm[nxt], n, tmp, st);
+        pc = nxt;
+    }
+    if (hipMemcpyAsync(d_perm_out, perm[pc], N * 4, hipMemcpyDeviceToDevice, st) != hipSuccess) return RGX_ERR_DEVICE;
     return hipGetLastError() == hipSuccess ? RGX_OK : RGX_ERR_DEVICE;
 }
 
diff --git a/regtools_amd/csrc/api_front.cpp b/regtools_amd/csrc/api_front.cpp
--- a/regtools_amd/csrc/api_front.cpp
+++ b/regtools_amd/csrc/api_front.cpp
@@ -5,6 +5,7 @@
     if (p->strandness == 3 && !p->fasta_path) return fail(err, errlen, RGX_ERR_ARG, "Strandness mode 'intron-motif' requires a fasta file!\n\n");
     HIP_ENTER(c->device);
     st = c->stream;
+    HIP_TRY(quiesce_pre(c));
     copy_q = c->copy_stream ? c->copy_stream : c->stream;
     t_begin = now_ms();
     trace = getenv("REGTOOLS_AMD_TRACE") != nullptr;
diff --git a/regtools_amd/csrc/api_internal.h b/regtools_amd/csrc/api_internal.h
--- a/regtools_amd/csrc/api_internal.h
+++ b/regtools_amd/csrc/api_internal.h
@@ -211,6 +211,7 @@
     uint32_t gate_epoch = 0;
     hipEvent_t ev_ready = nullptr, ev_side[kSideStreams] = {}, ev_packed = nullptr;
     hipEvent_t ev[8] = {};
+    hipEvent_t ev_pre[2] = {}; bool pre_busy = false;
     uint64_t arena_calibrated_bytes = 0;
     DevBuf *arena_retired = nullptr;
     hipEvent_t ev_trial[2] = {};
@@ -247,6 +248,18 @@
 struct CachedBlock { void *p; size_t cap; bool pinned; };
 struct SharedMembers { const std::vector<Member> *members; uint64_t total_inflated; };
 
+inline bool groupby_lean() {
+    static const bool lean = [] { const char *e = getenv("REGTOOLS_AMD_GROUPBY_TAIL"); return !(e && !strcmp(e, "0")); }();
+    return lean;
+}
+inline hipError_t quiesce_pre(rgx_ctx *c) {
+    if (!c->pre_busy) return hipSuccess;
+    c->pre_busy = false;
+    hipError_t e_ = hipEventRecord(c->ev_pre[1], c->side[0]);
+    return e_ != hipSuccess ? e_ : hipStreamWaitEvent(c->stream, c->ev_pre[1], 0);
+}
+struct PreAgg { PartialSoA pr{}; uint32_t *total = nullptr; size_t cap = 0; uint32_t rows = 0 ; };
+
 struct Prep {
     BamHeader hdr;
     const uint8_t *arena = nullptr;
@@ -255,6 +268,7 @@
     uint32_t n_rec = 0, n_events = 0, n_range = 0;
     uint64_t n_iterated = 0, total = 0;
     uint32_t framing_sweeps = 0;
+    PreAgg pre;
     bool stream_ended = false;
     double t_begin = 0;
     struct OddAux { int32_t tid, pos, end; };
@@ -398,6 +412,20 @@
     uint32_t sA = 0;
     bool emit_parts_ok = false; uint32_t emit_parts = 0, emit_rows = 0; size_t ev_lay = 0;
     EventSoA ev_e;
+    PreAgg pre;
+    hipError_t pre_layout() {
+        pre = PreAgg();
+        if (!groupby_lean() || p->barcodes || want_read_span || ev_lay > 0xffffffffu || !c->side[0] || !c->ev_pre[0]) return hipSuccess;
+        DevBuf &b_par = c->buf("partials");
+        const hipError_t e_ = b_par.ensure(ev_lay * 4 * 9 + scan_tmp_words((uint32_t)ev_lay) * 4 + 512);
+        if (e_ != hipSuccess) return e_;
+        uint32_t *q = b_par.as<uint32_t>();
+        const size_t Ev = ev_lay;
+        pre.pr.tid = q; q += Ev; pre.pr.start = q; q += Ev; pre.pr.ilen_cls = q; q += Ev; pre.pr.ts = q; q += Ev; pre.pr.te = q; q += Ev;
+        pre.pr.count = q; q += Ev; pre.pr.first = q; q += Ev; pre.pr.last = q;
+        pre.cap = Ev; pre.total = d_sc + 78;
+        return hipMemsetAsync(pre.total, 0, 4, c->stream);
+    }
     EventSoA ev_layout(uint8_t *q, size_t E) {
         EventSoA v; memset(&v, 0, sizeof v);
         v.tid = (uint32_t *)q; q += E * 4; v.start = (uint32_t *)q; q += E * 4; v.ilen_cls = (uint32_t *)q; q += E * 4;
@@ -410,6 +438,14 @@
     size_t soa_cap = 0;
     ReadSoA soa;
     uint32_t *ev_base = nullptr, *long_list = nullptr;
+    hipError_t pre_part(uint32_t part) {
+        hipError_t e_ = hipEventRecord(c->ev_pre[0], c->stream);
+        if (e_ == hipSuccess) e_ = hipStreamWaitEvent(c->side[0], c->ev_pre[0], 0);
+        if (e_ != hipSuccess) return e_;
+        launch_preagg_part(ev_e, (uint32_t)ev_lay, d_sc + 84, part, pre.pr, pre.total, c->side[0]);
+        c->pre_busy = true;
+        return hipSuccess;
+    }
     hipError_t soa_layout(size_t R) {
         DevBuf &b_soa = c->buf("soa");
         hipError_t e_ = b_soa.ensure(R * (4 + 4 + 4 + 8 + 1 + 4 + 4 + 4 + (p->barcodes ? 8 : 0)) + 256);
@@ -452,7 +488,8 @@
 
 int reduce_events(rgx_ctx *c, EventSoA ev, uint32_t n_events, uint32_t group_bits, uint32_t ilen_bits, const uint32_t *rank_of_group_host,
                   uint32_t n_groups, HostRows &R, char *err, size_t errlen, bool view_only = false, RowMap *row_map = nullptr, TableSink *sink = nullptr,
-                  bool allow_preagg = true );
+                  bool allow_preagg = true ,
+                  const PreAgg *pre = nullptr );
 int barcode_rows(rgx_ctx *c, const Prep &P, const RowMap &rm, const rgx_extract_params *p, rgx_junction_table *t, char *err, size_t errlen);
 void chrom_string_ranks(const BamHeader &hdr, std::vector<uint32_t> &rank_of_tid);
 int run_pipeline(rgx_ctx *c, const uint8_t *d_bam_in, const uint8_t *h_bam, size_t bam_len, const uint8_t *bai, size_t bai_len,
diff --git a/regtools_amd/csrc/api_records.cpp b/regtools_amd/csrc/api_records.cpp
--- a/regtools_amd/csrc/api_records.cpp
+++ b/regtools_amd/csrc/api_records.cpp
@@ -234,6 +234,7 @@
     HIP_TRY(hipEventRecord(c->ev[2], st));
     sA = 0;
     emit_parts_ok = false; emit_parts = 0; emit_rows = 0; ev_lay = 0;
+    pre = PreAgg();
     memset(&ev_e, 0, sizeof ev_e);
     soa_cap = 0;
     memset(&soa, 0, sizeof soa);
@@ -296,12 +297,14 @@
                 ev_lay = b_ev0.cap > 256 ? (b_ev0.cap - 256) / 33 : 0;
                 emit_parts_ok = env_early_emit && ev_lay >= 4096;
                 if (emit_parts_ok) { HIP_TRY(b_tmp.ensure(scan_tmp_words((uint32_t)std::min<size_t>(soa_cap, 0xffffffffu)) * 4 + 64));
-                    ev_e = ev_layout(b_ev0.as<uint8_t>(), ev_lay); }
+                    ev_e = ev_layout(b_ev0.as<uint8_t>(), ev_lay);
+                    HIP_TRY(pre_layout()); }
             }
             if (emit_parts_ok && emit_parts < kGateParts - 1) {
                 launch_scan_u32(soa.n_ev + emit_rows, ev_base + emit_rows, n_rec_J - emit_rows, d_sc + 84 + emit_parts, b_tmp.as<uint32_t>(), st);
                 launch_emit_short(arena, n_rec_J, cfg, soa, ev_base, ev_e, st, emit_rows, d_sc + 84, emit_parts, (uint32_t)std::min<size_t>(ev_lay,
                     0xffffffffu));
+                if (pre.total) HIP_TRY(pre_part(emit_parts));
                 emit_rows = n_rec_J; ++emit_parts;
             }
             sA = sJ;
@@ -342,6 +345,7 @@
     DevBuf &b_tmp = c->buf("tmp");
     n_events = 0; n_long = 0;
     n_iterated = 0;
+    if (!(emit_parts_ok && sA)) HIP_TRY(quiesce_pre(c));
     if (n_rec) {
         const size_t R = n_rec;
         uint32_t s_from = sA;
@@ -365,6 +369,11 @@
             if (emit_parts_ok && s_from) {
                 launch_scan_u32(soa.n_ev + emit_rows, ev_base + emit_rows, n_rec - emit_rows, d_sc + 84 + emit_parts, b_tmp.as<uint32_t>(), st);
                 launch_emit_short(arena, n_rec, cfg, soa, ev_base, ev_e, st, emit_rows, d_sc + 84, emit_parts, (uint32_t)std::min<size_t>(ev_lay, 0xffffffffu));
+                if (pre.total) {
+                    launch_preagg_part(ev_e, (uint32_t)ev_lay, d_sc + 84, emit_parts, pre.pr, pre.total, st);
+                    HIP_TRY(quiesce_pre(c));
+                    HIP_TRY(hipMemcpyAsync(h_sc + 78, pre.total, 4, hipMemcpyDeviceToHost, st));
+                }
                 HIP_TRY(hipMemcpyAsync(h_sc + 84, d_sc + 84, 4 * kGateParts, hipMemcpyDeviceToHost, st));
             } else launch_scan_u32(soa.n_ev, ev_base, n_rec, d_sc + 4, b_tmp.as<uint32_t>(), st);
             launch_scan_u32(seg_iter, seg_iter, n_seg, d_sc + 8, b_tmp.as<uint32_t>(), st);
@@ -393,6 +402,7 @@
                 "regtools_amd: record %u has an auxiliary field of unknown type in front of its strand or barcode tag: the reference abort()s here\n",
                 h_sc[96]);
         n_events = h_sc[4]; n_long = h_sc[5];
+        pre.rows = h_sc[78];
         if (emit_parts_ok && s_from) {
             uint64_t tot = 0;
             for (uint32_t k = 0; k <= emit_parts && k < kGateParts; ++k) tot += h_sc[84 + k];
@@ -432,7 +442,7 @@
     EventSoA ev; memset(&ev, 0, sizeof ev);
     if (n_events) {
         const size_t E = n_events;
-        if (emit_parts_ok && n_rec) ev = ev_e;
+        if (emit_parts_ok && n_rec) { ev = ev_e; P.pre = pre; }
         else {
             HIP_TRY(b_ev.ensure(E * (4 * 8 + 1) + 256));
             ev = ev_layout(b_ev.as<uint8_t>(), E);
diff --git a/regtools_amd/csrc/api_reduce.cpp b/regtools_amd/csrc/api_reduce.cpp
--- a/regtools_amd/csrc/api_reduce.cpp
+++ b/regtools_amd/csrc/api_reduce.cpp
@@ -1,7 +1,8 @@
 #include "api_internal.h"
 
 int reduce_events(rgx_ctx *c, EventSoA ev, uint32_t n_events, uint32_t group_bits, uint32_t ilen_bits, const uint32_t *rank_of_group_host,
-                         uint32_t n_groups, HostRows &R, char *err, size_t errlen, bool view_only, RowMap *row_map, TableSink *sink, bool allow_preagg) {
+                         uint32_t n_groups, HostRows &R, char *err, size_t errlen, bool view_only, RowMap *row_map, TableSink *sink, bool allow_preagg,
+                         const PreAgg *pre) {
     hipStream_t st = c->stream;
     uint32_t *d_sc = c->buf("scalars").as<uint32_t>();
     uint32_t *h_sc = (uint32_t *)c->pinned;
@@ -13,13 +14,21 @@
     uint32_t *final_perm = nullptr;
     uint32_t *chrom_rank_rows = nullptr;
     R = HostRows();
+    const bool lean = groupby_lean();
+    HIP_TRY(quiesce_pre(c));
     if (n_events) {
         const bool preagg = !row_map && allow_preagg;
         PartialSoA pr; memset(&pr, 0, sizeof pr);
         uint32_t *ev_flag = nullptr;
         EventSoA sev = ev;
         uint32_t n_s = n_events;
-        if (preagg) {
+        if (preagg && pre && pre->total) {
+            pr = pre->pr; ev_flag = pr.tid + 8 * pre->cap;
+            n_s = pre->rows;
+            if (!n_s || n_s > n_events) return fail(err, errlen, RGX_ERR_DEVICE, "regtools_amd: %u partial rows for %u events\n", n_s, n_events);
+            memset(&sev, 0, sizeof sev);
+            sev.tid = pr.tid; sev.start = pr.start; sev.ilen_cls = pr.ilen_cls; sev.ts = pr.ts; sev.te = pr.te;
+        } else if (preagg) {
             DevBuf &b_par = c->buf("partials");
             const size_t Ev = n_events;
             HIP_TRY(b_par.ensure(Ev * 4 * 9 + scan_tmp_words(n_events) * 4 + 512));
@@ -35,49 +44,74 @@
             sev.tid = pr.tid; sev.start = pr.start; sev.ilen_cls = pr.ilen_cls; sev.ts = pr.ts; sev.te = pr.te;
         }
         const size_t E = n_s;
-        const size_t rtmp = radix_tmp_words(n_s) + scan_tmp_words(n_s) + 64;
-        HIP_TRY(b_sort.ensure(E * 4 * 6 + rtmp * 4 + 256));
-        uint32_t *q = b_sort.as<uint32_t>();
-        perm[0] = q; q += E; perm[1] = q; q += E;
-        uint32_t *key[2]; key[0] = q; q += E; key[1] = q; q += E;
-        uint32_t *head = q; q += E; uint32_t *seg_excl = q; q += E;
-        uint32_t *tmp = q;
-        int pc = -1;
-        auto sort_word = [&](const uint32_t *word, uint32_t nbits) {
-            const uint32_t *kin = word;
-            int kc = 0;
-            if (pc >= 0) { launch_gather_u32(n_s, word, perm[pc], key[0], st); kin = key[0]; kc = 1; }
-            for (uint32_t sh = 0; sh < nbits; sh += 8) {
-                const uint32_t bits = std::min<uint32_t>(8, nbits - sh);
-                const int nxt = pc < 0 ? 0 : pc ^ 1;
-                launch_radix_pass_keyed(kin, key[kc], sh, bits, pc < 0 ? nullptr : perm[pc], perm[nxt], n_s, tmp, st);
-                kin = key[kc]; kc ^= 1;
-                pc = nxt;
-            }
+        uint32_t *head_pos = nullptr, *uperm[2] = {nullptr, nullptr}, *utmp_p = nullptr;
+        auto carve_unique = [&](size_t cap) -> hipError_t {
+            const size_t utmp = radix_tmp_words((uint32_t)cap) + 64;
+            const hipError_t e_ = b_uni.ensure(cap * 4 * 13 + cap + utmp * 4 + 256);
+            if (e_ != hipSuccess) return e_;
+            uint32_t *w = b_uni.as<uint32_t>();
+            u.tid = w; w += cap; u.start = w; w += cap; u.end = w; w += cap; u.ts_min = w; w += cap; u.te_max = w; w += cap; u.count = w; w += cap;
+            u.first_seen = w; w += cap; u.last_seen = w; w += cap; u.name_rank = w; w += cap;
+            head_pos = w; w += cap; chrom_rank_rows = w; w += cap;
+            uperm[0] = w; w += cap; uperm[1] = w; w += cap;
+            utmp_p = w; w += utmp;
+            u.strand = (uint8_t *)w;
+            return hipSuccess;
         };
-        sort_word(sev.ilen_cls, ilen_bits);
-        sort_word(sev.start, 32);
-        sort_word(sev.tid, group_bits);
-        const uint32_t *sorted = perm[pc];
-        launch_heads(sev, sorted, n_s, head, st);
-        launch_scan_u32(head, seg_excl, n_s, d_sc + 6, tmp, st);
-        HIP_TRY(hipMemcpyAsync(h_sc + 6, d_sc + 6, 4, hipMemcpyDeviceToHost, st));
-        HIP_TRY(hipStreamSynchronize(st));
-        n_unique = h_sc[6];
+        constexpr uint32_t kGroupTableMax = 4u << 20;
+        const bool hashed = lean && preagg && n_s <= kGroupTableMax;
+        const uint32_t *sorted = nullptr;
+        uint32_t *head = nullptr, *seg_excl = nullptr, *tmp = nullptr;
+        if (hashed) {
+            uint32_t n_slots = 256;
+            while (n_slots < 2 * n_s) n_slots <<= 1;
+            HIP_TRY(b_sort.ensure(((size_t)n_slots + 2 * E) * 4 + 256));
+            uint32_t *slots = b_sort.as<uint32_t>(), *leader = slots + n_slots, *row_of = leader + E;
+            HIP_TRY(carve_unique(E));
+            launch_group_partials(pr, n_s, slots, n_slots, leader, row_of, d_sc + 6, u, st);
+            HIP_TRY(hipMemcpyAsync(h_sc + 6, d_sc + 6, 8, hipMemcpyDeviceToHost, st));
+            HIP_TRY(hipStreamSynchronize(st));
+            n_unique = h_sc[6];
+            if (h_sc[7] || !n_unique || n_unique > n_s) return fail(err, errlen, RGX_ERR_DEVICE, "regtools_amd: the group-by's table lost %u rows\n", h_sc[7]);
+            launch_reduce_finish_partials(ev.strand, n_unique, u, nullptr, st);
+        } else {
+            const size_t rtmp = radix_tmp_words(n_s) + scan_tmp_words(n_s) + 64;
+            HIP_TRY(b_sort.ensure(E * 4 * 6 + rtmp * 4 + 256));
+            uint32_t *q = b_sort.as<uint32_t>();
+            perm[0] = q; q += E; perm[1] = q; q += E;
+            uint32_t *key[2]; key[0] = q; q += E; key[1] = q; q += E;
+            head = q; q += E; seg_excl = q; q += E;
+            tmp = q;
+            int pc = -1;
+            auto sort_word = [&](const uint32_t *word, uint32_t nbits) {
+                const uint32_t *kin = word;
+                int kc = 0;
+                if (pc >= 0) { launch_gather_u32(n_s, word, perm[pc], key[0], st); kin = key[0]; kc = 1; }
+                for (uint32_t sh = 0; sh < nbits; sh += 8) {
+                    const uint32_t bits = std::min<uint32_t>(8, nbits - sh);
+                    const int nxt = pc < 0 ? 0 : pc ^ 1;
+                    launch_radix_pass_keyed(kin, key[kc], sh, bits, pc < 0 ? nullptr : perm[pc], perm[nxt], n_s, tmp, st);
+                    kin = key[kc]; kc ^= 1;
+                    pc = nxt;
+                }
+            };
+            sort_word(sev.ilen_cls, ilen_bits);
+            sort_word(sev.start, 32);
+            sort_word(sev.tid, group_bits);
+            sorted = perm[pc];
+            launch_heads(sev, sorted, n_s, head, st);
+            launch_scan_u32(head, seg_excl, n_s, d_sc + 6, tmp, st);
+            HIP_TRY(hipMemcpyAsync(h_sc + 6, d_sc + 6, 4, hipMemcpyDeviceToHost, st));
+            HIP_TRY(hipStreamSynchronize(st));
+            n_unique = h_sc[6];
+            HIP_TRY(carve_unique(n_unique));
+        }
 
         const size_t U = n_unique;
-        const size_t utmp = radix_tmp_words(n_unique) + 64;
-        HIP_TRY(b_uni.ensure(U * 4 * 13 + U + utmp * 4 + 256));
-        uint32_t *w = b_uni.as<uint32_t>();
-        u.tid = w; w += U; u.start = w; w += U; u.end = w; w += U; u.ts_min = w; w += U; u.te_max = w; w += U; u.count = w; w += U;
-        u.first_seen = w; w += U; u.last_seen = w; w += U; u.name_rank = w; w += U;
-        uint32_t *head_pos = w; w += U; chrom_rank_rows = w; w += U;
-        uint32_t *uperm[2]; uperm[0] = w; w += U; uperm[1] = w; w += U;
-        uint32_t *utmp_p = w; w += utmp;
-        u.strand = (uint8_t *)w;
-        launch_fill_u32(u.ts_min, 0xffffffffu, U, st);
-        launch_fill_u32(u.te_max, 0u, U, st);
-        if (preagg) {
+        if (hashed) {
+        } else if (preagg) {
+            launch_fill_u32(u.ts_min, 0xffffffffu, U, st);
+            launch_fill_u32(u.te_max, 0u, U, st);
             launch_fill_u32(u.count, 0u, U, st);
             launch_fill_u32(u.first_seen, 0xffffffffu, U, st);
             launch_fill_u32(u.last_seen, 0u, U, st);
@@ -87,6 +121,8 @@
             launch_scan_u32(ev_flag, ev_flag, n_events, nullptr, ev_flag + n_events, st);
             launch_name_rank(n_unique, ev_flag, u, st);
         } else {
+            launch_fill_u32(u.ts_min, 0xffffffffu, U, st);
+            launch_fill_u32(u.te_max, 0u, U, st);
             launch_reduce(ev, sorted, head, seg_excl, n_events, u, head_pos, st);
             if (row_map) {
                 DevBuf &b_map = c->buf("row_map");
@@ -117,7 +153,10 @@
                 upc = nxt;
             }
         };
-        usort(u.name_rank, std::max<uint32_t>(1, bitlen(n_unique)));
+        if (hashed) {
+            usort(u.first_seen, std::max<uint32_t>(1, bitlen(n_events)));
+            launch_name_from_order(uperm[upc], n_unique, u, st);
+        } else usort(u.name_rank, std::max<uint32_t>(1, bitlen(n_unique)));
         usort(u.te_max, 32);
         usort(u.ts_min, 32);
         usort(chrom_rank_rows, std::max<uint32_t>(1, bitlen(rk)));
@@ -300,7 +339,7 @@
     RowMap rm;
     TableSink sink; sink.hdr = &P.hdr; sink.min_anchor = p->min_anchor;
     rc = reduce_events(c, P.ev, P.n_events, std::max<uint32_t>(1, bitlen((uint32_t)std::max(n_ref - 1, 0))), std::min<uint32_t>(32, bitlen(p->max_intron) + 2),
-                       rank_of_tid.data(), (uint32_t)std::max(n_ref, 1), R, err, errlen, true, p->barcodes ? &rm : nullptr, &sink);
+                       rank_of_tid.data(), (uint32_t)std::max(n_ref, 1), R, err, errlen, true, p->barcodes ? &rm : nullptr, &sink, true, &P.pre);
     if (rc != RGX_OK) return rc;
     c->last_rows = R.n; c->last_records = P.n_iterated; c->last_events = P.n_events; c->last_bytes = P.total; c->last_rows_valid = true;
     HIP_TRY(hipEventRecord(c->ev[6], st));
diff --git a/regtools_amd/csrc/kernels.h b/regtools_amd/csrc/kernels.h
--- a/regtools_amd/csrc/kernels.h
+++ b/regtools_amd/csrc/kernels.h
@@ -144,8 +144,12 @@
 };
 struct PartialSoA { uint32_t *tid, *start, *ilen_cls, *ts, *te, *count, *first, *last; };
 void launch_preagg(EventSoA ev, uint32_t n, PartialSoA p, uint32_t *p_total , hipStream_t stream);
+void launch_preagg_part(EventSoA ev, uint32_t cap, const uint32_t *part_totals, uint32_t part, PartialSoA p, uint32_t *p_total, hipStream_t stream);
+void launch_group_partials(PartialSoA p, uint32_t n, uint32_t *slots, uint32_t n_slots, uint32_t *leader, uint32_t *row_of, uint32_t *counters, UniqueSoA u,
+                           hipStream_t stream);
 void launch_reduce_partials(PartialSoA p, const uint32_t *perm, const uint32_t *head, const uint32_t *seg_excl, uint32_t n, UniqueSoA u, hipStream_t stream);
 void launch_reduce_finish_partials(const uint8_t *ev_strand, uint32_t n_unique, UniqueSoA u, uint32_t *first_flag , hipStream_t stream);
+void launch_name_from_order(const uint32_t *by_first, uint32_t n_unique, UniqueSoA u, hipStream_t stream);
 void launch_heads(EventSoA ev, const uint32_t *perm, uint32_t n, uint32_t *head, hipStream_t stream);
 void launch_reduce(EventSoA ev, const uint32_t *perm, const uint32_t *head, const uint32_t *seg_excl, uint32_t n, UniqueSoA u,
                    uint32_t *head_pos, hipStream_t stream);
diff --git a/regtools_amd/csrc/kernels.hip b/regtools_amd/csrc/kernels.hip
--- a/regtools_amd/csrc/kernels.hip
+++ b/regtools_amd/csrc/kernels.hip
@@ -1469,54 +1469,64 @@
 
 constexpr uint32_t kAggEmpty = 0xffffffffu;
 template <uint32_t kAggTile>
-__global__ __launch_bounds__(256) void k_preagg(EventSoA ev, uint32_t n, PartialSoA p, uint32_t *p_total) {
+__global__ __launch_bounds__(256) void k_preagg(EventSoA ev, uint32_t n, PartialSoA p, uint32_t *p_total, const uint32_t *__restrict__ part_totals,
+                                                uint32_t part) {
     constexpr uint32_t kAggSlots = 2 * kAggTile;
     __shared__ uint32_t s_tid[kAggTile], s_start[kAggTile], s_ilen[kAggTile], s_slot[kAggSlots];
     __shared__ uint32_t s_cnt[kAggTile], s_ts[kAggTile], s_te[kAggTile], s_first[kAggTile], s_last[kAggTile];
     __shared__ uint32_t s_wave[4], s_base;
-    const uint32_t base = blockIdx.x * kAggTile, t = threadIdx.x;
-#pragma unroll
-    for (uint32_t k = 0; k < kAggTile / 256; ++k) {
-        const uint32_t i = t + 256 * k, e = base + i;
-        if (e < n) { s_tid[i] = ev.tid[e]; s_start[i] = ev.start[e]; s_ilen[i] = ev.ilen_cls[e]; }
-        s_cnt[i] = 0; s_ts[i] = 0xffffffffu; s_te[i] = 0; s_first[i] = 0xffffffffu; s_last[i] = 0;
-        s_slot[i] = kAggEmpty; s_slot[i + kAggTile] = kAggEmpty;
-    }
-    __syncthreads();
-    uint32_t mine = 0;
-#pragma unroll
-    for (uint32_t k = 0; k < kAggTile / 256; ++k) {
-        const uint32_t i = t + 256 * k, e = base + i;
-        if (e < n) {
-            const uint32_t kt = s_tid[i], ks = s_start[i], kl = s_ilen[i];
-            uint32_t h = ks * 0x9E3779B1u ^ kl * 0x85EBCA6Bu ^ kt * 0xC2B2AE35u;
-            h = (h ^ h >> 15) & (kAggSlots - 1);
-            uint32_t leader;
-            for (;;) {
-                const uint32_t prev = atomicCAS(&s_slot[h], kAggEmpty, i);
-                if (prev == kAggEmpty) { leader = i; mine |= 1u << k; break; }
-                if (s_tid[prev] == kt && s_start[prev] == ks && s_ilen[prev] == kl) { leader = prev; break; }
-                h = (h + 1) & (kAggSlots - 1);
-            }
-            atomicAdd(&s_cnt[leader], 1u);
-            atomicMin(&s_ts[leader], ev.ts[e]); atomicMax(&s_te[leader], ev.te[e]);
-            atomicMin(&s_first[leader], i); atomicMax(&s_last[leader], i);
-        }
-    }
-    __syncthreads();
-    uint32_t tot;
-    uint32_t at = block_excl_scan_256((uint32_t)__popc(mine), s_wave, tot);
-    if (t == 0) s_base = tot ? atomicAdd(p_total, tot) : 0u;
-    __syncthreads();
-    at += s_base;
-#pragma unroll
-    for (uint32_t k = 0; k < kAggTile / 256; ++k) {
-        if (mine >> k & 1u) {
-            const uint32_t i = t + 256 * k;
-            p.tid[at] = s_tid[i]; p.start[at] = s_start[i]; p.ilen_cls[at] = s_ilen[i];
-            p.count[at] = s_cnt[i]; p.ts[at] = s_ts[i]; p.te[at] = s_te[i]; p.first[at] = base + s_first[i]; p.last[at] = base + s_last[i];
-            ++at;
-        }
+    uint32_t first = 0;
+    if (part_totals) {
+        for (uint32_t k = 0; k < part; ++k) first += part_totals[k];
+        n = (uint32_t)min((uint64_t)n, (uint64_t)first + part_totals[part]);
+    }
+    const uint32_t t = threadIdx.x;
+    for (uint64_t tile = blockIdx.x; first + tile * kAggTile < n; tile += gridDim.x) {
+        const uint32_t base = first + (uint32_t)tile * kAggTile;
+#pragma unroll
+        for (uint32_t k = 0; k < kAggTile / 256; ++k) {
+            const uint32_t i = t + 256 * k, e = base + i;
+            if (e < n) { s_tid[i] = ev.tid[e]; s_start[i] = ev.start[e]; s_ilen[i] = ev.ilen_cls[e]; }
+            s_cnt[i] = 0; s_ts[i] = 0xffffffffu; s_te[i] = 0; s_first[i] = 0xffffffffu; s_last[i] = 0;
+            s_slot[i] = kAggEmpty; s_slot[i + kAggTile] = kAggEmpty;
+        }
+        __syncthreads();
+        uint32_t mine = 0;
+#pragma unroll
+        for (uint32_t k = 0; k < kAggTile / 256; ++k) {
+            const uint32_t i = t + 256 * k, e = base + i;
+            if (e < n) {
+                const uint32_t kt = s_tid[i], ks = s_start[i], kl = s_ilen[i];
+                uint32_t h = ks * 0x9E3779B1u ^ kl * 0x85EBCA6Bu ^ kt * 0xC2B2AE35u;
+                h = (h ^ h >> 15) & (kAggSlots - 1);
+                uint32_t leader;
+                for (;;) {
+                    const uint32_t prev = atomicCAS(&s_slot[h], kAggEmpty, i);
+                    if (prev == kAggEmpty) { leader = i; mine |= 1u << k; break; }
+                    if (s_tid[prev] == kt && s_start[prev] == ks && s_ilen[prev] == kl) { leader = prev; break; }
+                    h = (h + 1) & (kAggSlots - 1);
+                }
+                atomicAdd(&s_cnt[leader], 1u);
+                atomicMin(&s_ts[leader], ev.ts[e]); atomicMax(&s_te[leader], ev.te[e]);
+                atomicMin(&s_first[leader], i); atomicMax(&s_last[leader], i);
+            }
+        }
+        __syncthreads();
+        uint32_t tot;
+        uint32_t at = block_excl_scan_256((uint32_t)__popc(mine), s_wave, tot);
+        if (t == 0) s_base = tot ? atomicAdd(p_total, tot) : 0u;
+        __syncthreads();
+        at += s_base;
+#pragma unroll
+        for (uint32_t k = 0; k < kAggTile / 256; ++k) {
+            if (mine >> k & 1u) {
+                const uint32_t i = t + 256 * k;
+                p.tid[at] = s_tid[i]; p.start[at] = s_start[i]; p.ilen_cls[at] = s_ilen[i];
+                p.count[at] = s_cnt[i]; p.ts[at] = s_ts[i]; p.te[at] = s_te[i]; p.first[at] = base + s_first[i]; p.last[at] = base + s_last[i];
+                ++at;
+            }
+        }
+        __syncthreads();
     }
 }
 
@@ -1551,7 +1561,58 @@
     const uint32_t r = blockIdx.x * blockDim.x + threadIdx.x;
     if (r >= n_unique) return;
     u.strand[r] = ev_strand[u.last_seen[r]];
-    first_flag[u.first_seen[r]] = 1;
+    if (first_flag) first_flag[u.first_seen[r]] = 1;
+}
+__global__ void k_name_from_order(const uint32_t *__restrict__ by_first, uint32_t n_unique, UniqueSoA u) {
+    const uint32_t i = blockIdx.x * blockDim.x + threadIdx.x;
+    if (i < n_unique) u.name_rank[by_first[i]] = i + 1;
+}
+
+__global__ void k_group_init(UniqueSoA u, uint32_t n_rows, uint32_t *slots, uint32_t n_slots, uint32_t *counters ) {
+    const uint32_t r = blockIdx.x * blockDim.x + threadIdx.x;
+    if (r < n_rows) { u.ts_min[r] = 0xffffffffu; u.te_max[r] = 0; u.count[r] = 0; u.first_seen[r] = 0xffffffffu; u.last_seen[r] = 0; }
+    if (r < n_slots) slots[r] = kAggEmpty;
+    if (r < 2) counters[r] = 0;
+}
+__global__ __launch_bounds__(256) void k_group_insert(PartialSoA p, uint32_t n, uint32_t *slots, uint32_t slot_mask, uint32_t *leader, uint32_t *row_of,
+                                                      uint32_t *counters, UniqueSoA u) {
+    const uint32_t i = blockIdx.x * blockDim.x + threadIdx.x;
+    bool won = false;
+    uint32_t kt = 0, ks = 0, kl = 0;
+    if (i < n) {
+        kt = p.tid[i]; ks = p.start[i]; kl = p.ilen_cls[i];
+        uint32_t h = ks * 0x9E3779B1u ^ kl * 0x85EBCA6Bu ^ kt * 0xC2B2AE35u;
+        h = (h ^ h >> 15) * 0x2C1B3C6Du;
+        h = (h ^ h >> 13) & slot_mask;
+        uint32_t lead = kAggEmpty;
+        for (uint32_t probe = 0; probe <= slot_mask; ++probe) {
+            const uint32_t prev = atomicCAS(&slots[h], kAggEmpty, i);
+            if (prev == kAggEmpty) { lead = i; won = true; break; }
+            if (p.tid[prev] == kt && p.start[prev] == ks && p.ilen_cls[prev] == kl) { lead = prev; break; }
+            h = (h + 1) & slot_mask;
+        }
+        if (lead == kAggEmpty) { atomicAdd(counters + 1, 1u); lead = i; }
+        leader[i] = lead;
+    }
+    const uint64_t m = __ballot(won);
+    if (m) {
+        const uint32_t first = (uint32_t)__ffsll((unsigned long long)m) - 1;
+        uint32_t b = 0;
+        if (lane_id() == first) b = atomicAdd(counters, (uint32_t)__popcll(m));
+        b = __shfl(b, first, 64);
+        if (won) {
+            const uint32_t row = b + (uint32_t)__popcll(m & lanemask_lt());
+            row_of[i] = row;
+            u.tid[row] = kt; u.start[row] = ks; u.end[row] = ks + (kl >> 2);
+        }
+    }
+}
+__global__ void k_group_reduce(PartialSoA p, uint32_t n, const uint32_t *__restrict__ leader, const uint32_t *__restrict__ row_of, UniqueSoA u) {
+    const uint32_t i = blockIdx.x * blockDim.x + threadIdx.x;
+    if (i >= n) return;
+    const uint32_t row = row_of[leader[i]];
+    atomicMin(&u.ts_min[row], p.ts[i]); atomicMax(&u.te_max[row], p.te[i]); atomicAdd(&u.count[row], p.count[i]);
+    atomicMin(&u.first_seen[row], p.first[i]); atomicMax(&u.last_seen[row], p.last[i]);
 }
 
 __global__ void k_reduce_finish(EventSoA ev, const uint32_t *__restrict__ perm, uint32_t n, uint32_t n_unique,
@@ -1634,7 +1695,10 @@
 }
 void launch_preagg(EventSoA ev, uint32_t n, PartialSoA p, uint32_t *p_total, hipStream_t stream) {
     if (!n) return;
-    hipLaunchKernelGGL(k_preagg<1024>, dim3((n + 1023) / 1024), dim3(256), 0, stream, ev, n, p, p_total);
+    hipLaunchKernelGGL(k_preagg<1024>, dim3((n + 1023) / 1024), dim3(256), 0, stream, ev, n, p, p_total, (const uint32_t *)nullptr, 0u);
+}
+void launch_preagg_part(EventSoA ev, uint32_t cap, const uint32_t *part_totals, uint32_t part, PartialSoA p, uint32_t *p_total, hipStream_t stream) {
+    if (cap) hipLaunchKernelGGL(k_preagg<1024>, dim3(std::min<uint32_t>((cap + 1023) / 1024, 2048)), dim3(256), 0, stream, ev, cap, p, p_total, part_totals, part);
 }
 void launch_reduce_partials(PartialSoA p, const uint32_t *perm, const uint32_t *head, const uint32_t *seg_excl, uint32_t n, UniqueSoA u, hipStream_t stream) {
     if (n) hipLaunchKernelGGL(k_reduce_partials, dim3((n + 255) / 256), dim3(256), 0, stream, p, perm, head, seg_excl, n, u);
@@ -1642,6 +1706,16 @@
 void launch_reduce_finish_partials(const uint8_t *ev_strand, uint32_t n_unique, UniqueSoA u, uint32_t *first_flag, hipStream_t stream) {
     if (n_unique) hipLaunchKernelGGL(k_reduce_finish_partials, dim3((n_unique + 255) / 256), dim3(256), 0, stream, ev_strand, n_unique, u, first_flag);
 }
+void launch_name_from_order(const uint32_t *by_first, uint32_t n_unique, UniqueSoA u, hipStream_t stream) {
+    if (n_unique) hipLaunchKernelGGL(k_name_from_order, dim3((n_unique + 255) / 256), dim3(256), 0, stream, by_first, n_unique, u);
+}
+void launch_group_partials(PartialSoA p, uint32_t n, uint32_t *slots, uint32_t n_slots, uint32_t *leader, uint32_t *row_of, uint32_t *counters, UniqueSoA u,
+                           hipStream_t stream) {
+    if (!n) return;
+    hipLaunchKernelGGL(k_group_init, dim3((std::max(n, n_slots) + 255) / 256), dim3(256), 0, stream, u, n, slots, n_slots, counters);
+    hipLaunchKernelGGL(k_group_insert, dim3((n + 255) / 256), dim3(256), 0, stream, p, n, slots, n_slots - 1, leader, row_of, counters, u);
+    hipLaunchKernelGGL(k_group_reduce, dim3((n + 255) / 256), dim3(256), 0, stream, p, n, leader, row_of, u);
+}
 void launch_fill_u32(uint32_t *p, uint32_t v, size_t n, hipStream_t stream) {
     if (n) hipLaunchKernelGGL(k_fill_u32, dim3((unsigned)((n + 255) / 256)), dim3(256), 0, stream, p, v, n);
 }
```

Measured after the change: 2.107 billion alignments/s (median of 3 runs). About the same (+0.8%).
